# JanEGerken/HEAL-SWIN

Hardware: AMD Instinct MI355X
Metric: images/sec fwd+bwd, HEAL-SWIN nside=256 seg, batch=8 at 1/2/4/8 MI355X (higher is better)
Workload: dtype bf16

## Files before the change

heal_swin_amd/_lib.py:

```python
import ctypes
import os

import numpy as np

_PKG = os.path.dirname(os.path.abspath(__file__))
LIB_PATH = os.path.join(_PKG, "lib", "libhealswin.so")

HS_F32, HS_BF16 = 0, 1
HS_F64 = 3
HS_PRED_LABELS, HS_PRED_ROWS16 = 2, 4
HS_ATTN_COSINE = 1
HS_ATTN_FORCE_VALU = 2
HS_ATTN_RESIDUAL = 4
HS_ATTN_OVERWRITE_GRADS = 8
HS_EPI_BIAS, HS_EPI_GELU, HS_EPI_DGELU, HS_EPI_RESID = 0, 1, 2, 3
HS_ACC_DEFER = 2
HS_MLP_NORM_AFTER = 16
HS_U8, HS_I32, HS_I64 = 8, 9, 10
HS_FLAT_PATCH_ROWS, HS_FLAT_PIXEL_ROWS, HS_FLAT_IMAGE = 0, 1, 2
HS_DEPTH_L1, HS_DEPTH_L2, HS_DEPTH_HUBER, HS_DEPTH_LOGVAR = 0, 1, 2, 3
HS_DT_NONE, HS_DT_LOG, HS_DT_INV = 0, 1, 2
HS_DT_ZERO_BKG, HS_DT_1000_BKG, HS_DT_AFFINE, HS_DT_INVERSE = 1, 2, 4, 8
HS_DEPTH_STATS_WORDS = 15
HS_HISTOGRAM_MAX_BINS = 4096

c_i64 = ctypes.c_int64
c_int = ctypes.c_int
c_uint = ctypes.c_uint
c_ptr = ctypes.c_void_p
c_float = ctypes.c_float


class WgradProblem(ctypes.Structure):
    _fields_ = [("dy", c_ptr), ("x", c_ptr), ("dw", c_ptr), ("dbias", c_ptr), ("n_out", c_int), ("k_in", c_int), ("accumulate", c_int),
                ("gelu_x", c_int)]


def wgrad_problems(members):
    arr = (WgradProblem * len(members))()
    for q, (dy, x, dw, db, n_out, k_in, acc, gelu_x) in zip(arr, members):
        q.dy, q.x, q.dw, q.dbias = dy.data_ptr(), x.data_ptr(), dw.data_ptr(), (None if db is None else db.data_ptr())
        q.n_out, q.k_in, q.accumulate, q.gelu_x = int(n_out), int(k_in), int(acc), int(bool(gelu_x))
    return arr

class AdamGroup(ctypes.Structure):
    _fields_ = [("lr_dev", c_ptr), ("lr", c_float), ("beta1", c_float), ("beta2", c_float), ("eps", c_float), ("weight_decay", c_float),
                ("decoupled", ctypes.c_int32)]


def adam_groups(records):
    arr = (AdamGroup * len(records))()
    for q, (lr, b1, b2, eps, wd, decoupled) in zip(arr, records):
        on_device = hasattr(lr, "data_ptr")
        q.lr_dev, q.lr = (lr.data_ptr() if on_device else None), (0.0 if on_device else float(lr))
        q.beta1, q.beta2, q.eps, q.weight_decay, q.decoupled = float(b1), float(b2), float(eps), float(wd), int(bool(decoupled))
    return arr


class FisheyeCamera(ctypes.Structure):
    _fields_ = [("k", ctypes.c_double * 8), ("cx_offset", ctypes.c_double), ("cy_offset", ctypes.c_double), ("aspect_ratio", ctypes.c_double),
                ("poly_order", c_int), ("width", c_int), ("height", c_int)]


_SIGNATURES = {
    "hs_nest2ring": [c_int, c_ptr, c_ptr, c_i64],
    "hs_ring2nest": [c_int, c_ptr, c_ptr, c_i64],
    "hs_nest_win_idcs": [c_int, c_ptr],
    "hs_rel_pos_index": [c_int, c_ptr],
    "hs_build_nest_roll_shift": [c_i64, c_int, c_int, c_ptr, c_ptr, c_ptr],
    "hs_build_nest_grid_shift": [c_int, c_int, c_int, c_ptr, c_ptr, c_ptr],
    "hs_build_ring_shift": [c_int, c_int, c_int, c_int, c_ptr, c_ptr, c_ptr],
    "hs_attn_mask_from_labels": [c_ptr, c_i64, c_int, c_ptr],
    "hs_flat_zorder": [c_int, c_int, c_int, c_ptr, c_ptr],
    "hs_build_flat_shift": [c_int, c_int, c_int, c_int, c_int, c_ptr, c_ptr, c_ptr],
    "hs_flat_rel_pos_index": [c_int, c_ptr, c_ptr],
    "hs_flat_attn_mask": [c_int, c_int, c_int, c_int, c_ptr],
    "hs_flat_img_to_rows": [c_ptr, c_int, c_ptr, c_int, c_int, c_int, c_int, c_int, c_int, c_int, c_int, c_i64, c_ptr],
    "hs_flat_rows_to_img": [c_ptr, c_int, c_ptr, c_int, c_int, c_int, c_int, c_int, c_int, c_int, c_int, c_i64, c_ptr],
    "hs_flat_resize": [c_ptr, c_int, c_i64, c_int, c_int, c_int, c_int, c_ptr, c_ptr, c_ptr, c_ptr, c_ptr, c_int, c_int, c_int, c_int, c_int,
                       c_int, c_i64, c_int, c_int, c_int, c_int, c_int, c_int, c_float, c_float, c_ptr],
    "hs_rel_bias_gather": [c_ptr, c_ptr, c_ptr, c_int, c_int, c_int, c_ptr],
    "hs_rel_bias_scatter_grad_sorted_add": [c_ptr, c_ptr, c_ptr, c_ptr, c_int, c_int, c_int, c_ptr],
    "hs_cos_head_scale_fwd": [c_ptr, c_ptr, c_int, c_ptr],
    "hs_cos_head_scale_bwd": [c_ptr, c_ptr, c_ptr, c_int, c_int, c_ptr],
    "hs_rel_bias_gather_many": [c_ptr, c_ptr, c_int, c_ptr, c_ptr, c_int, c_int, c_ptr],
    "hs_rel_bias_scatter_grad_sorted_many": [c_ptr, c_ptr, c_ptr, c_ptr, c_int, c_ptr, c_ptr, c_int, c_int, c_ptr],
    "hs_cos_head_scale_many": [c_ptr, c_ptr, c_ptr, c_ptr, c_ptr, c_int, c_ptr],
    "hs_rel_bias_scatter_grad": [c_ptr, c_ptr, c_ptr, c_int, c_int, c_int, c_ptr],
    "hs_rel_bias_scatter_grad_sorted": [c_ptr, c_ptr, c_ptr, c_ptr, c_int, c_int, c_int, c_ptr],
    "hs_window_attn_fwd": [c_ptr, c_ptr, c_ptr, c_ptr, c_ptr, c_ptr, c_i64, c_ptr,
                           c_int, c_i64, c_int, c_int, c_int, c_uint, ctypes.c_float, ctypes.c_uint64, c_int, c_ptr],
    "hs_window_attn_bwd": [c_ptr, c_ptr, c_ptr, c_ptr, c_ptr, c_ptr, c_ptr, c_ptr, c_ptr, c_ptr, c_ptr, c_i64, c_ptr,
                           c_int, c_i64, c_int, c_int, c_int, c_uint, ctypes.c_float, ctypes.c_uint64, c_int, c_ptr],
    "hs_gather_rows": [c_ptr, c_ptr, c_ptr, c_i64, c_int, c_i64, c_i64, c_ptr],
    "hs_pix2ang_nest": [c_int, c_i64, c_i64, c_ptr, c_ptr],
    "hs_ln_head_supported": [c_int, c_int, c_int],
    "hs_expand_ln_head_supported": [c_int, c_int, c_int, c_int],
    "hs_expand_ln_head_fwd": [c_ptr, c_ptr, c_ptr, c_ptr, c_ptr, c_ptr, c_ptr, c_ptr, c_ptr, c_i64, c_int, c_int, c_int, c_ptr],
    "hs_expand_ln_head_ce_fwd": [c_ptr, c_ptr, c_ptr, c_ptr, c_ptr, c_ptr, c_ptr, c_int, c_ptr, c_ptr, c_ptr, c_ptr, c_ptr, c_i64, c_int, c_int,
                                 c_int, c_ptr],
    "hs_expand_ln_head_ce_step_fwd": [c_ptr, c_ptr, c_ptr, c_ptr, c_ptr, c_ptr, c_ptr, c_int, c_ptr, c_ptr, c_ptr, c_ptr, c_ptr, c_ptr, c_ptr,
                                      c_ptr, c_i64, c_int, c_int, c_int, c_ptr],
    "hs_ln_head_ce_bwd": [c_ptr, c_ptr, c_ptr, c_ptr, c_ptr, c_ptr, c_int, c_ptr, c_ptr, c_ptr, c_ptr, c_ptr, c_ptr, c_i64, c_int, c_int, c_ptr],
    "hs_expand_ln_head_depth_fwd": [c_ptr, c_ptr, c_ptr, c_ptr, c_ptr, c_ptr, c_int, c_float, c_int, c_ptr, c_ptr, c_ptr, c_ptr, c_ptr, c_i64,
                                    c_int, c_int, c_int, c_ptr],
    "hs_expand_ln_head_depth_step_fwd": [c_ptr, c_ptr, c_ptr, c_ptr, c_ptr, c_ptr, c_int, c_float, c_int, c_ptr, c_ptr, c_ptr, c_ptr, c_ptr,
                                         c_int, c_int, c_float, c_float, c_int, ctypes.c_double, c_ptr, c_int, c_ptr, c_ptr, c_ptr, c_ptr,
                                         c_i64, c_int, c_int, c_int, c_ptr],
    "hs_ln_head_depth_bwd": [c_ptr, c_ptr, c_ptr, c_ptr, c_int, c_float, c_ptr, c_int, c_ptr, c_ptr, c_ptr, c_ptr, c_ptr, c_ptr, c_i64, c_int,
                             c_int, c_ptr],
    "hs_ln_head_fwd": [c_ptr, c_ptr, c_ptr, c_ptr, c_ptr, c_ptr, c_i64, c_int, c_int, c_int, c_ptr],
    "hs_ln_head_bwd": [c_ptr, c_ptr, c_ptr, c_ptr, c_ptr, c_ptr, c_ptr, c_ptr, c_i64, c_int, c_int, c_int, c_ptr],
    "hs_sample_bilinear_u8": [c_ptr, c_int, c_int, c_int, c_int, c_ptr, c_ptr, c_i64, c_ptr, c_ptr],
    "hs_sample_mask_u8": [c_ptr, c_int, c_int, c_int, c_ptr, c_ptr, c_i64, c_int, c_ptr, c_ptr],
    "hs_hp_rotated_coords": [c_int, c_i64, c_i64, ctypes.POINTER(FisheyeCamera), c_ptr, c_int, c_ptr, c_ptr, c_ptr],
    "hs_sample_bilinear_u8_per_sample": [c_ptr, c_int, c_int, c_int, c_int, c_ptr, c_ptr, c_i64, c_ptr, c_ptr],
    "hs_sample_mask_u8_per_sample": [c_ptr, c_int, c_int, c_int, c_ptr, c_ptr, c_i64, c_int, c_ptr, c_ptr],
    "hs_hp_interp_weights_nest": [c_int, c_ptr, c_ptr, c_i64, c_ptr, c_ptr],
    "hs_backproject_labels": [c_ptr, c_int, c_i64, c_i64, c_int, c_i64, c_i64, c_i64, c_ptr, c_i64, c_int, c_ptr, c_ptr],
    "hs_backproject_image": [c_ptr, c_i64, c_i64, c_ptr, c_ptr, c_i64, c_ptr, c_ptr],
    "hs_seg_confusion": [c_ptr, c_int, c_i64, c_i64, c_int, c_i64, c_i64, c_i64, c_ptr, c_i64, c_ptr, c_int, c_ptr, c_ptr, c_ptr],
    "hs_depth_points": [c_ptr, c_int, c_i64, c_i64, c_i64, c_i64, c_i64, c_i64, c_ptr, c_i64, c_ptr, c_int, c_ptr, c_ptr, c_ptr, c_ptr,
                        c_ptr],
    "hs_chamfer_nn": [c_ptr, c_ptr, c_i64, c_i64, c_ptr, c_ptr, c_i64, c_i64, c_i64, c_int, c_ptr, c_ptr, c_ptr, c_ptr, c_ptr, c_ptr,
                      c_ptr],
    "hs_depth_metrics": [c_ptr, c_int, c_i64, c_i64, c_i64, c_i64, c_i64, c_i64, c_i64, c_ptr, c_int, c_i64, c_i64, c_i64, c_int,
                         ctypes.c_double, c_ptr, c_int, c_ptr, c_ptr, c_ptr],
    "hs_backproject_depth": [c_ptr, c_int, c_i64, c_i64, c_i64, c_i64, c_ptr, c_ptr, c_i64, c_ptr, c_ptr],
    "hs_flat_depth_to_hp": [c_ptr, c_int, c_i64, c_i64, c_i64, c_i64, c_ptr, c_ptr, c_ptr, c_i64, c_ptr, c_ptr],
    "hs_depth_metrics_gather": [c_ptr, c_int, c_i64, c_i64, c_i64, c_i64, c_i64, c_ptr, c_ptr, c_ptr, c_i64, c_ptr, c_int, c_i64, c_i64,
                                c_int, ctypes.c_double, c_ptr, c_int, c_ptr, c_ptr, c_ptr],
    "hs_sample_bilinear_u8_f32": [c_ptr, c_int, c_int, c_int, c_int, c_ptr, c_ptr, c_i64, c_ptr, c_ptr],
    "hs_sample_nearest_f32": [c_ptr, c_int, c_int, c_int, c_ptr, c_ptr, c_i64, c_float, c_ptr, c_ptr],
    "hs_sample_bilinear_u8_f32_per_sample": [c_ptr, c_int, c_int, c_int, c_int, c_ptr, c_ptr, c_i64, c_ptr, c_ptr],
    "hs_sample_nearest_f32_per_sample": [c_ptr, c_int, c_int, c_int, c_ptr, c_ptr, c_i64, c_float, c_ptr, c_ptr],
    "hs_depth_target": [c_ptr, c_i64, c_i64, c_ptr, c_i64, c_i64, c_i64, c_i64, c_int, c_int, c_float, c_float, c_ptr],
    "hs_depth_stats_update": [c_ptr, c_i64, c_int, c_int, c_ptr, c_ptr, c_ptr],
    "hs_depth_stats_merge": [c_ptr, c_int, c_ptr, c_ptr],
    "hs_histogram_update": [c_ptr, c_i64, c_int, c_int, c_ptr, c_int, c_ptr, c_ptr],
    "hs_select_rows": [c_ptr, c_int, c_i64, c_i64, c_i64, c_int, c_int, c_ptr, c_ptr, c_ptr],
    "hs_gelu_fwd": [c_ptr, c_ptr, c_i64, ctypes.c_float, ctypes.c_uint64, c_int, c_ptr],
    "hs_gelu_bwd": [c_ptr, c_ptr, c_ptr, c_i64, ctypes.c_float, ctypes.c_uint64, c_int, c_ptr],
    "hs_residual_drop": [c_ptr, c_ptr, c_ptr, c_ptr, c_i64, c_i64, ctypes.c_float, ctypes.c_uint64, c_int, c_ptr],
    "hs_linear_wgrad": [c_ptr, c_ptr, c_ptr, c_ptr, c_ptr, c_i64, c_int, c_int, c_int, c_int, c_ptr],
    "hs_reduce_flush": [c_ptr],
    "hs_set_seed_epoch": [c_ptr],
    "hs_linear_wgrad_gelu": [c_ptr, c_ptr, c_ptr, c_ptr, c_ptr, c_i64, c_int, c_int, c_int, c_int, c_ptr],
    "hs_linear_wgrad_gelu_supported": [c_i64, c_int, c_int, c_int],
    "hs_linear_wgrad_group_variant": [c_i64, c_int, c_int, c_int],
    "hs_linear_wgrad_group": [c_ptr, c_int, c_ptr, c_i64, c_int, c_ptr],
    "hs_mlp_fused_supported": [c_int, c_int, c_int],
    "hs_mlp_fused_fwd": [c_ptr, c_ptr, c_ptr, c_ptr, c_ptr, c_ptr, c_ptr, c_ptr, c_ptr, c_ptr, c_ptr, c_ptr, c_ptr, c_i64, c_int, c_int, c_uint,
                         c_int, c_ptr],
    "hs_mlp_fused_bwd": [c_ptr, c_ptr, c_ptr, c_ptr, c_ptr, c_ptr, c_ptr, c_i64, c_int, c_int, c_int, c_ptr],
    "hs_mlp_fused_drop_fwd": [c_ptr, c_ptr, c_ptr, c_ptr, c_ptr, c_ptr, c_ptr, c_ptr, c_ptr, c_ptr, c_ptr, c_ptr, c_ptr, c_ptr, c_i64, c_float,
                              ctypes.c_uint64, ctypes.c_uint64, c_i64, c_int, c_int, c_uint, c_int, c_ptr],
    "hs_mlp_fused_drop_bwd": [c_ptr, c_ptr, c_ptr, c_ptr, c_ptr, c_ptr, c_ptr, c_float, ctypes.c_uint64, c_i64, c_int, c_int, c_int, c_ptr],
    "hs_adam_step": [c_ptr, c_ptr, c_ptr, c_ptr, c_ptr, c_i64, c_float, c_ptr, c_float, c_float, c_float, c_float, c_int, c_ptr, c_ptr],
    "hs_adam_advance": [c_ptr, c_ptr],
    "hs_grad_stats": [c_ptr, c_i64, c_ptr, c_int, c_ptr, c_ptr],
    "hs_grad_guard_finalize": [c_ptr, c_i64, c_ptr, c_int, c_int, c_float, c_ptr, c_ptr, c_ptr, c_ptr],
    "hs_adam_step_guarded": [c_ptr, c_ptr, c_ptr, c_ptr, c_ptr, c_i64, c_float, c_ptr, c_float, c_float, c_float, c_float, c_int, c_ptr, c_float,
                             c_ptr, c_int, c_ptr],
    "hs_adam_advance_guarded": [c_ptr, c_ptr, c_int, c_ptr, c_ptr],
    "hs_adam_step_groups": [c_ptr, c_ptr, c_ptr, c_ptr, c_ptr, c_i64, c_ptr, c_int, c_ptr, c_int, c_ptr, c_int, c_i64, c_ptr, c_ptr],
    "hs_adam_step_groups_guarded": [c_ptr, c_ptr, c_ptr, c_ptr, c_ptr, c_i64, c_ptr, c_int, c_ptr, c_int, c_ptr, c_int, c_i64, c_ptr, c_float,
                                    c_ptr, c_int, c_ptr],
    "hs_grad_scale": [c_ptr, c_i64, c_float, c_ptr, c_ptr],
    "hs_weight_avg_update": [c_ptr, c_ptr, c_i64, c_int, c_float, c_ptr, c_ptr, c_int, c_ptr],
    "hs_weight_avg_advance": [c_ptr, c_ptr, c_int, c_ptr],
    "hs_weight_avg_swap": [c_ptr, c_ptr, c_ptr, c_i64, c_ptr],
    "hs_split_bf16x3": [c_ptr, c_ptr, c_i64, c_int, c_int, c_ptr],
    "hs_gelu_split3": [c_ptr, c_ptr, c_ptr, c_i64, c_int, ctypes.c_float, ctypes.c_uint64, c_ptr],
    "hs_linear_wgrad_ld": [c_ptr, c_i64, c_i64, c_ptr, c_i64, c_i64, c_ptr, c_ptr, c_ptr, c_i64, c_int, c_int, c_int, c_ptr],
    "hs_layernorm_fwd": [c_ptr, c_ptr, c_ptr, c_ptr, c_ptr, c_ptr, c_ptr, c_i64, c_int, c_int, c_ptr],
    "hs_add_layernorm_fwd": [c_ptr, c_ptr, c_ptr, c_ptr, c_ptr, c_ptr, c_ptr, c_ptr, c_i64, c_int, c_int, c_ptr],
    "hs_add_layernorm_bwd": [c_ptr, c_ptr, c_ptr, c_ptr, c_ptr, c_ptr, c_ptr, c_ptr, c_ptr, c_ptr, c_int, c_i64, c_int, c_int, c_ptr],
    "hs_layernorm_drop_fwd": [c_ptr, c_ptr, c_ptr, c_ptr, c_ptr, c_ptr, c_ptr, c_ptr, c_i64, ctypes.c_float, ctypes.c_uint64,
                              c_i64, c_int, c_int, c_ptr],
    "hs_layernorm_drop_bwd": [c_ptr, c_ptr, c_ptr, c_ptr, c_ptr, c_ptr, c_ptr, c_ptr, c_ptr, c_int, c_ptr, c_i64, ctypes.c_float,
                              ctypes.c_uint64, c_i64, c_int, c_int, c_ptr],
    "hs_add_layernorm_drop_fwd": [c_ptr, c_ptr, c_ptr, c_ptr, c_ptr, c_ptr, c_ptr, c_ptr, c_ptr, c_i64, ctypes.c_float,
                                  ctypes.c_uint64, c_i64, c_int, c_int, c_ptr],
    "hs_layernorm_fwd_ex": [c_ptr, c_ptr, c_ptr, c_ptr, c_ptr, c_ptr, c_ptr, c_ptr, c_ptr, c_ptr, c_ptr, c_ptr, c_i64, ctypes.c_float,
                            ctypes.c_uint64, c_i64, c_int, c_int, c_ptr],
    "hs_add_layernorm_drop_bwd": [c_ptr, c_ptr, c_ptr, c_ptr, c_ptr, c_ptr, c_ptr, c_ptr, c_ptr, c_ptr, c_ptr, c_int, c_ptr, c_i64,
                                  ctypes.c_float, ctypes.c_uint64, c_i64, c_int, c_int, c_ptr],
    "hs_seg_ce_fwd": [c_ptr, c_ptr, c_ptr, c_ptr, c_i64, c_i64, c_int, c_i64, c_i64, c_i64, c_int, c_i64, c_int, c_ptr],
    "hs_seg_ce_bwd": [c_ptr, c_ptr, c_ptr, c_ptr, c_ptr, c_i64, c_i64, c_int, c_i64, c_i64, c_i64, c_i64, c_i64, c_i64, c_int, c_i64,
                      c_int, c_ptr],
    "hs_depth_loss_fwd": [c_ptr, c_ptr, c_ptr, c_i64, c_i64, c_int, c_i64, c_i64, c_i64, c_int, c_float, c_int, c_ptr],
    "hs_depth_loss_bwd": [c_ptr, c_ptr, c_ptr, c_ptr, c_i64, c_i64, c_int, c_i64, c_i64, c_i64, c_i64, c_i64, c_i64, c_int, c_float, c_int, c_ptr],
    "hs_gemm_nt": [c_ptr, c_i64, c_ptr, c_i64, c_int, c_ptr, c_i64, c_ptr, c_i64, c_int, c_ptr, c_ptr, c_ptr, c_i64, c_int, c_int,
                   ctypes.c_float, ctypes.c_uint64, c_int, c_ptr],
    "hs_gemm_nt_set_tile": [c_int],
    "hs_gemm_nt_tile_variant": [c_i64, c_int, c_int, c_int, c_int],
    "hs_set_reserved_cus": [c_int],
    "hs_transpose_many_16": [c_ptr, c_int, c_int, c_ptr],
    "hs_debug_occupy_cus": [c_int, c_int, c_int, ctypes.c_double, c_ptr],
    "hs_debug_buffer_soffset_probe": [c_ptr, c_int, c_int, c_ptr, c_ptr],
    "hs_window_attn_module_supported": [c_int, c_int, c_int, c_int],
    "hs_window_attn_module_fwd": [c_ptr, c_ptr, c_ptr, c_ptr, c_ptr, c_ptr, c_ptr, c_ptr, c_ptr, c_ptr, c_ptr, c_i64, c_ptr, c_int, c_i64,
                                  c_int, c_int, c_int, c_uint, c_int, c_ptr],
    "hs_window_attn_module_fwd_train": [c_ptr] * 17 + [c_i64] + [c_ptr] * 6 + [c_int, c_i64, c_int, c_int, c_int, c_uint, c_int, c_ptr],
    "hs_window_attn_module_bwd_chain": [c_ptr] * 14 + [c_i64] + [c_ptr] * 11 + [c_int, c_int, c_i64, c_int, c_int, c_int, c_uint, c_int, c_ptr],
    "hs_layernorm_bwd": [c_ptr, c_ptr, c_ptr, c_ptr, c_ptr, c_ptr, c_ptr, c_ptr, c_ptr, c_int, c_i64, c_int, c_int, c_ptr],
    "hs_patch_merge_fwd": [c_ptr, c_ptr, c_ptr, c_ptr, c_ptr, c_ptr, c_ptr, c_ptr, c_i64, c_int, c_int, c_int, c_ptr],
    "hs_patch_merge_bwd": [c_ptr, c_ptr, c_ptr, c_ptr, c_ptr, c_ptr, c_ptr, c_ptr, c_ptr, c_ptr, c_ptr, c_ptr, c_ptr, c_int, c_i64,
                           c_int, c_int, c_int, c_ptr],
    "hs_patch_expand_fwd": [c_ptr, c_ptr, c_ptr, c_ptr, c_ptr, c_ptr, c_ptr, c_ptr, c_i64, c_int, c_int, c_int, c_int, c_ptr],
    "hs_patch_expand_bwd": [c_ptr, c_ptr, c_ptr, c_ptr, c_ptr, c_ptr, c_ptr, c_ptr, c_ptr, c_ptr, c_ptr, c_ptr, c_ptr, c_int, c_i64,
                            c_int, c_int, c_int, c_int, c_ptr],
}
_OTHER = {
    "hs_version": ([], ctypes.c_char_p),
    "hs_last_error": ([], ctypes.c_char_p),
    "hs_status_string": ([c_int], ctypes.c_char_p),
    "hs_device_count": ([], c_int),
    "hs_get_reserved_cus": ([], c_int),
    "hs_grad_guard_piece": ([], c_int),
    "hs_adam_max_groups": ([], c_int),
    "hs_get_seed_epoch": ([], c_ptr),
    "hs_reduce_pending": ([c_ptr], c_int),
    "hs_layernorm_bwd_workspace": ([c_i64, c_int], c_i64),
    "hs_seg_ce_partials": ([c_i64, c_i64], c_i64),
    "hs_depth_loss_partials": ([c_i64, c_i64], c_i64),
    "hs_depth_points_workspace": ([c_i64, c_i64], c_i64),
    "hs_depth_metrics_partials": ([c_i64], c_i64),
    "hs_depth_stats_partials": ([c_i64], c_i64),
    "hs_select_rows_workspace": ([c_int], c_i64),
    "hs_flat_resize_lds_bytes": ([c_int, c_int, c_int, c_int, c_int, c_int], c_i64),
    "hs_ln_head_partials": ([c_i64], c_i64),
    "hs_expand_ln_head_blocks": ([c_i64], c_i64),
    "hs_linear_wgrad_workspace": ([c_i64, c_int, c_int], c_i64),
    "hs_linear_wgrad_group_workspace": ([c_ptr, c_int, c_i64, c_int], c_i64),
    "hs_window_attn_bwd_workspace": ([c_int, c_i64, c_int, c_int, c_int, c_int], c_i64),
    "hs_patch_merge_bwd_workspace": ([c_i64, c_int, c_int], c_i64),
    "hs_window_attn_module_bwd_chain_workspace": ([c_int, c_i64, c_int, c_int, c_int], c_i64),
    "hs_patch_expand_bwd_workspace": ([c_i64, c_int, c_int, c_int], c_i64),
}
EXPORTED_SYMBOLS = sorted(list(_SIGNATURES) + list(_OTHER))


def _load():
    if not os.path.exists(LIB_PATH):
        raise RuntimeError(
            f"libhealswin.so not found at {LIB_PATH}: build it first (python heal_swin_amd/build.py, or "
            "__graft_entry__.build()).  heal_swin_amd has no CPU or PyTorch fallback."
        )
    lib = ctypes.CDLL(LIB_PATH)
    for name, argtypes in _SIGNATURES.items():
        fn = getattr(lib, name)
        fn.argtypes = argtypes
        fn.restype = c_int
    for name, (argtypes, restype) in _OTHER.items():
        fn = getattr(lib, name)
        fn.argtypes = argtypes
        fn.restype = restype
    return lib


lib = _load()


def check(status, what):
    if status != 0:
        msg = lib.hs_last_error().decode()
        kind = lib.hs_status_string(status).decode()
        if status == 1:
            raise AssertionError(f"{what}: {msg}")
        raise RuntimeError(f"{what} failed ({kind}): {msg}")


def version():
    return lib.hs_version().decode()


def device_count():
    return int(lib.hs_device_count())


def np_ptr(a):
    return None if a is None else a.ctypes.data_as(c_ptr)


def ptr(t):
    return None if t is None else ctypes.c_void_p(t.data_ptr())


def stream_ptr(device):
    import torch

    return ctypes.c_void_p(torch.cuda.current_stream(device).cuda_stream)


def dtype_code(dtype):
    import torch

    if dtype == torch.float32:
        return HS_F32
    if dtype == torch.bfloat16:
        return HS_BF16
    raise TypeError(f"heal_swin_amd kernels support float32 and bfloat16 activations, got {dtype}")


def nest2ring(nside, ipix):
    a = np.ascontiguousarray(ipix, dtype=np.int64)
    out = np.empty_like(a)
    check(lib.hs_nest2ring(int(nside), np_ptr(a), np_ptr(out), a.size), "hs_nest2ring")
    return out


def ring2nest(nside, ipix):
    a = np.ascontiguousarray(ipix, dtype=np.int64)
    out = np.empty_like(a)
    check(lib.hs_ring2nest(int(nside), np_ptr(a), np_ptr(out), a.size), "hs_ring2nest")
    return out


def nest_win_idcs(window_size):
    side = int(round(window_size ** 0.5))
    out = np.empty((max(side, 1), max(side, 1)), dtype=np.int64)
    check(lib.hs_nest_win_idcs(int(window_size), np_ptr(out)), "hs_nest_win_idcs")
    return out


def rel_pos_index(window_size):
    out = np.empty((window_size, window_size), dtype=np.int64)
    check(lib.hs_rel_pos_index(int(window_size), np_ptr(out)), "hs_rel_pos_index")
    return out


def _shift_out(n):
    return np.empty(n, np.int32), np.empty(n, np.int32), np.empty(n, np.uint8)


def build_nest_roll_shift(n_pix, window_size, shift_size):
    idx, inv, lab = _shift_out(n_pix)
    check(lib.hs_build_nest_roll_shift(int(n_pix), int(window_size), int(shift_size), np_ptr(idx), np_ptr(inv), np_ptr(lab)),
          "hs_build_nest_roll_shift")
    return idx, inv, lab


def build_nest_grid_shift(nside, base_pix, window_size):
    idx, inv, lab = _shift_out(max(base_pix, 0) * nside * nside)
    check(lib.hs_build_nest_grid_shift(int(nside), int(base_pix), int(window_size), np_ptr(idx), np_ptr(inv), np_ptr(lab)),
          "hs_build_nest_grid_shift")
    return idx, inv, lab


def build_ring_shift(nside, base_pix, window_size, shift_size):
    idx, inv, lab = _shift_out(max(base_pix, 0) * nside * nside)
    check(lib.hs_build_ring_shift(int(nside), int(base_pix), int(window_size), int(shift_size), np_ptr(idx), np_ptr(inv),
                                  np_ptr(lab)), "hs_build_ring_shift")
    return idx, inv, lab


def attn_mask_from_labels(labels, window_size):
    lab = np.ascontiguousarray(labels, dtype=np.uint8)
    out = np.empty((lab.size // window_size, window_size, window_size), dtype=np.float32)
    check(lib.hs_attn_mask_from_labels(np_ptr(lab), lab.size, int(window_size), np_ptr(out)), "hs_attn_mask_from_labels")
    return out


def flat_zorder(Ht, Wt, T):
    z = np.empty(Ht * Wt, np.int32)
    rm = np.empty(Ht * Wt, np.int32)
    check(lib.hs_flat_zorder(int(Ht), int(Wt), int(T), np_ptr(z), np_ptr(rm)), "hs_flat_zorder")
    return z, rm


def build_flat_shift(Ht, Wt, T, window, shift):
    idx, inv, lab = _shift_out(max(Ht * Wt, 0))
    check(lib.hs_build_flat_shift(int(Ht), int(Wt), int(T), int(window), int(shift), np_ptr(idx), np_ptr(inv), np_ptr(lab)),
          "hs_build_flat_shift")
    return idx, inv, lab


def flat_rel_pos_index(window):
    n = window * window
    rm = np.empty((n, n), np.int64)
    z = np.empty((n, n), np.int64)
    check(lib.hs_flat_rel_pos_index(int(window), np_ptr(rm), np_ptr(z)), "hs_flat_rel_pos_index")
    return rm, z


def flat_attn_mask(Ht, Wt, window, shift):
    out = np.empty(((Ht // window) * (Wt // window), window * window, window * window), np.float32)
    check(lib.hs_flat_attn_mask(int(Ht), int(Wt), int(window), int(shift), np_ptr(out)), "hs_flat_attn_mask")
    return out
```

heal_swin_amd/csrc/linear_wgrad.hip:

```cpp
#include <cstdlib>
#include <type_traits>
#include <utility>

#include "hs_gelu.h"

namespace hs {
namespace {

typedef __attribute__((ext_vector_type(4))) short s16x4;
typedef __attribute__((ext_vector_type(8))) short s16x8;
typedef __attribute__((address_space(3))) s16x4 lds_s16x4;

constexpr int kTileK = 128;
constexpr int kTok = 32;
constexpr int kMaxSlices = 2048;
constexpr int kReduceChunks = 32;
__host__ __device__ constexpr int row_stride(int cols) { return cols * 2 + 64; }

template <int LD>
__device__ __forceinline__ bf16x8 tr_frag(const unsigned char* tile, int tok0, int col0, int lane) {
    const int L = lane & 15, nblk = (lane >> 4) & 1;
    const unsigned char* a = tile + (tok0 + (L >> 2)) * LD + (col0 + nblk * 16 + (L & 3) * 4) * 2;
    const s16x4 lo = __builtin_amdgcn_ds_read_tr16_b64_v4i16((lds_s16x4*)a);
    const s16x4 hi = __builtin_amdgcn_ds_read_tr16_b64_v4i16((lds_s16x4*)(a + 4 * LD));
    const s16x8 v = {lo[0], lo[1], lo[2], lo[3], hi[0], hi[1], hi[2], hi[3]};
    return __builtin_bit_cast(bf16x8, v);
}

struct Geometry {
    int tile_n, tile_k, tiles_n, tiles_k, tiles, slices, chunks, per_xcd, dma, reads_first;
    int64_t rows_per_slice;
};

__host__ __device__ constexpr int64_t record_floats(int n_out, int k_in) { return (int64_t)n_out * k_in + n_out; }

inline void plan_slices(Geometry& g, int64_t rows, int wgs_per_cu) {
    int64_t want = ((int64_t)usable_cus() * wgs_per_cu) / g.tiles;
    const int64_t max_by_rows = (rows + 511) / 512;
    if (want > max_by_rows) want = max_by_rows;
    if (want > kMaxSlices) want = kMaxSlices;
    if (want < 1) want = 1;
    g.slices = (int)want;
    const int64_t rps = (rows + g.slices - 1) / g.slices;
    g.rows_per_slice = ((rps + kTok - 1) / kTok) * kTok;
    g.per_xcd = (g.slices * g.tiles + 7) / 8;
}

inline bool slice_fits_dma(const Geometry& g, int64_t width, int elt) { return g.rows_per_slice * width * elt < ((int64_t)1 << 31); }

inline Geometry geometry_for(int64_t rows, int n_out, int k_in, int tile_k, int wgs_per_cu, int tile_n = 0, int elt = 2) {
    Geometry g;
    g.tile_n = tile_n ? tile_n : ((n_out % 256 == 0 || n_out >= 512) ? 256 : 128);
    g.tile_k = tile_k;
    g.tiles_n = (n_out + g.tile_n - 1) / g.tile_n;
    g.tiles_k = (k_in + tile_k - 1) / tile_k;
    g.tiles = g.tiles_n * g.tiles_k;
    plan_slices(g, rows, wgs_per_cu);
    g.chunks = g.slices > 2 * kReduceChunks ? kReduceChunks : 1;
    g.dma = slice_fits_dma(g, n_out > k_in ? n_out : k_in, elt);
    g.reads_first = 3;
    return g;
}

inline Geometry make_geometry(int64_t rows, int n_out, int k_in) {
    static const int variant = getenv("HS_WGRAD_VARIANT") ? atoi(getenv("HS_WGRAD_VARIANT")) : 1;
    if (variant == 1 && k_in % 256 == 0 && (n_out % 256 == 0 || n_out >= 512)) {
        const Geometry g = geometry_for(rows, n_out, k_in, 256, 1);
        if (g.dma) return g;
    }
    Geometry g = geometry_for(rows, n_out, k_in, kTileK, 2);
    if (variant != 1) g.dma = 0;
    return g;
}

inline Geometry make_geometry_f32(int64_t rows, int n_out, int k_in) { return geometry_for(rows, n_out, k_in, kTileK, 3, 128, 4); }

__device__ __forceinline__ bool block_to_work(const Geometry& g, int b, int& slice, int& tile) {
    const int v = (b & 7) * g.per_xcd + (b >> 3);
    slice = v / g.tiles;
    tile = v % g.tiles;
    return (b >> 3) < g.per_xcd && v < g.slices * g.tiles;
}

struct SliceRows {
    int64_t m_begin;
    int m_len;
};
__device__ __forceinline__ SliceRows slice_rows(const Geometry& g, int slice, int64_t rows) {
    const int64_t m_begin = (int64_t)slice * g.rows_per_slice;
    int64_t m_end = m_begin + g.rows_per_slice;
    if (m_end > rows) m_end = rows;
    return {m_begin, m_end > m_begin ? (int)(m_end - m_begin) : 0};
}

template <int NB>
__device__ __forceinline__ void store_partial(const f32x16 (&acc)[NB][2], float* dst, int n_wave, int k_wave, int n_out, int k_in,
                                              int lane) {
#pragma unroll
    for (int i = 0; i < NB; ++i)
#pragma unroll
        for (int j = 0; j < 2; ++j) {
            const int kk = k_wave + j * 32 + (lane & 31);
#pragma unroll
            for (int r = 0; r < 16; ++r) {
                const int nn = n_wave + i * 32 + (r & 3) + 8 * (r >> 2) + 4 * (lane >> 5);
                if (nn < n_out && kk < k_in) dst[(int64_t)nn * k_in + kk] = acc[i][j][r];
            }
        }
}

template <int TN, int GROUPS, int PER_THREAD>
__device__ __forceinline__ void fold_bias(float* bred, const float (&bsum)[PER_THREAD], int tid, int n0, int n_out, float* dst) {
    constexpr int CH = TN / PER_THREAD;
#pragma unroll
    for (int i = 0; i < PER_THREAD; ++i) bred[(tid / CH) * TN + (tid % CH) * PER_THREAD + i] = bsum[i];
    __syncthreads();
    if (tid < TN) {
        float t = 0.f;
#pragma unroll
        for (int rg = 0; rg < GROUPS; ++rg) t += bred[rg * TN + tid];
        if (n0 + tid < n_out) dst[n0 + tid] = t;
    }
}

__device__ __forceinline__ void add_bf16x8(float (&bsum)[8], uint32_t w0, uint32_t w1, uint32_t w2, uint32_t w3) {
    const uint32_t w[4] = {w0, w1, w2, w3};
#pragma unroll
    for (int i = 0; i < 4; ++i) {
        bsum[2 * i] += bf_lo(w[i]);
        bsum[2 * i + 1] += bf_hi(w[i]);
    }
}

template <int NB>
__global__ void __launch_bounds__(256, 2) wgrad_kernel(const uint16_t* __restrict__ dy, const uint16_t* __restrict__ x,
                                                       float* __restrict__ part_w, float* __restrict__ part_b, int64_t rows,
                                                       int n_out, int k_in, Geometry g) {
    constexpr int TN = 64 * NB;
    constexpr int LDY = row_stride(TN), LDX = row_stride(kTileK);
    constexpr int YB = kTok * LDY, XB = kTok * LDX;
    constexpr int YCH = TN / 8;
    constexpr int YPASS = (kTok * YCH) / 256;
    __shared__ __attribute__((aligned(16))) unsigned char smem[2 * (YB + XB)];
    auto ytile = [&](int b) { return smem + b * (YB + XB); };
    auto xtile = [&](int b) { return smem + b * (YB + XB) + YB; };
    float* bred = (float*)smem;

    const int tid = threadIdx.x, lane = tid & 63, wave = tid >> 6, half = lane >> 5;
    const int wn = wave >> 1, wk = wave & 1;

    int slice, tile;
    if (!block_to_work(g, blockIdx.x, slice, tile)) return;
    const int tn = tile / g.tiles_k, tk = tile % g.tiles_k;
    const int n0 = tn * TN, k0 = tk * kTileK;
    const SliceRows sr = slice_rows(g, slice, rows);
    const int64_t m_begin = sr.m_begin, m_end = sr.m_begin + sr.m_len;

    const int xr = tid >> 4, xc = tid & 15;
    const int yr = tid / YCH, yc = tid % YCH;
    const bool ycol_ok = n0 + yc * 8 < n_out, xcol_ok = k0 + xc * 8 < k_in;
    const uint16_t* yptr = dy + n0 + yc * 8;
    const uint16_t* xptr = x + k0 + xc * 8;
    const bool do_bias = part_b != nullptr && tk == 0;
    float bsum[8] = {0.f, 0.f, 0.f, 0.f, 0.f, 0.f, 0.f, 0.f};

    f32x16 acc[NB][2];
    zero(acc);

    uint4 ry[YPASS], rx[2];
    auto load_regs = [&](int64_t m0) {
#pragma unroll
        for (int ps = 0; ps < YPASS; ++ps) {
            const int64_t m = m0 + yr + (256 / YCH) * ps;
            ry[ps] = (m < m_end && ycol_ok) ? *(const uint4*)(yptr + m * n_out) : make_uint4(0, 0, 0, 0);
        }
#pragma unroll
        for (int ps = 0; ps < 2; ++ps) {
            const int64_t m = m0 + xr + 16 * ps;
            rx[ps] = (m < m_end && xcol_ok) ? *(const uint4*)(xptr + m * k_in) : make_uint4(0, 0, 0, 0);
        }
    };
    auto store_lds = [&](int buf) {
#pragma unroll
        for (int ps = 0; ps < YPASS; ++ps) {
            *(uint4*)(ytile(buf) + (yr + (256 / YCH) * ps) * LDY + yc * 16) = ry[ps];
            if (do_bias) add_bf16x8(bsum, ry[ps].x, ry[ps].y, ry[ps].z, ry[ps].w);
        }
#pragma unroll
        for (int ps = 0; ps < 2; ++ps) *(uint4*)(xtile(buf) + (xr + 16 * ps) * LDX + xc * 16) = rx[ps];
    };

    if (m_begin < m_end) {
        load_regs(m_begin);
        store_lds(0);
    }
    __syncthreads();
    int buf = 0;
    for (int64_t m0 = m_begin; m0 < m_end; m0 += kTok) {
        const bool more = m0 + kTok < m_end;
        if (more) load_regs(m0 + kTok);
        bf16x8 af[2][NB], bf[2][2];
#pragma unroll
        for (int ks = 0; ks < 2; ++ks) {
            const int tok0 = ks * 16 + 8 * half;
#pragma unroll
            for (int j = 0; j < 2; ++j) bf[ks][j] = tr_frag<LDX>(xtile(buf), tok0, wk * 64 + j * 32, lane);
#pragma unroll
            for (int i = 0; i < NB; ++i) af[ks][i] = tr_frag<LDY>(ytile(buf), tok0, wn * 32 * NB + i * 32, lane);
        }
#pragma unroll
        for (int ks = 0; ks < 2; ++ks)
#pragma unroll
            for (int i = 0; i < NB; ++i)
#pragma unroll
                for (int j = 0; j < 2; ++j)
                    acc[i][j] = __builtin_amdgcn_mfma_f32_32x32x16_bf16(af[ks][i], bf[ks][j], acc[i][j], 0, 0, 0);
        if (more) store_lds(buf ^ 1);
        __syncthreads();
        buf ^= 1;
    }

    const int64_t rec = slice * record_floats(n_out, k_in);
    store_partial(acc, part_w + rec, n0 + wn * 32 * NB, k0 + wk * 64, n_out, k_in, lane);
    if (do_bias) fold_bias<TN, 256 / YCH>(bred, bsum, tid, n0, n_out, part_b + rec);
}

#if defined(__HIP_DEVICE_COMPILE__)
template <int YI, int XI>
__device__ __forceinline__ void issue_stage(__amdgpu_buffer_rsrc_t rs_y, __amdgpu_buffer_rsrc_t rs_x, unsigned char* ylds,
                                            unsigned char* xlds, int (&voff_y)[YI], int (&voff_x)[XI], int ystep, int xstep) {
#pragma unroll
    for (int j = 0; j < YI; ++j) {
        __builtin_amdgcn_raw_ptr_buffer_load_lds(rs_y, (lds_void*)(ylds + j * 1024), 16, voff_y[j], 0, 0, 0);
        voff_y[j] += ystep;
    }
#pragma unroll
    for (int j = 0; j < XI; ++j) {
        __builtin_amdgcn_raw_ptr_buffer_load_lds(rs_x, (lds_void*)(xlds + j * 1024), 16, voff_x[j], 0, 0, 0);
        voff_x[j] += xstep;
    }
}

template <int PIECES, int AH>
__device__ __forceinline__ void wait_stage(int younger) {
    if (AH - 1 >= 2 && younger >= 2)
        asm volatile("s_waitcnt vmcnt(%0)" ::"n"(2 * PIECES) : "memory");
    else if (younger >= 1)
        asm volatile("s_waitcnt vmcnt(%0)" ::"n"(PIECES) : "memory");
    else
        asm volatile("s_waitcnt vmcnt(0)" ::: "memory");
}
#endif

template <int NSTAGE, typename Issue, typename Stage>
__device__ __forceinline__ void run_stages(int nst, Issue&& issue, Stage&& stage) {
    static_for<NSTAGE - 1>([&](auto bc) {
        constexpr int b = decltype(bc)::value;
        if (nst > b) issue(b);
    });
    for (int t = 0; t < nst; t += NSTAGE)
        static_for<NSTAGE>([&](auto bc) {
            constexpr int b = decltype(bc)::value;
            if (t + b < nst) stage(t + b, bc, std::integral_constant<int, (b + NSTAGE - 1) % NSTAGE>{});
        });
}

template <int RB>
__device__ __forceinline__ s16x8 tr_frag_asm(uint32_t a, int ks) {
    s16x4 lo, hi;
    if (ks == 0) {
        asm volatile("ds_read_b64_tr_b16 %0, %1" : "=v"(lo) : "v"(a));
        asm volatile("ds_read_b64_tr_b16 %0, %1 offset:%2" : "=v"(hi) : "v"(a), "n"(4 * RB));
    } else {
        asm volatile("ds_read_b64_tr_b16 %0, %1 offset:%2" : "=v"(lo) : "v"(a), "n"(16 * RB));
        asm volatile("ds_read_b64_tr_b16 %0, %1 offset:%2" : "=v"(hi) : "v"(a), "n"(20 * RB));
    }
    return s16x8{lo[0], lo[1], lo[2], lo[3], hi[0], hi[1], hi[2], hi[3]};
}

constexpr int kMaxGroup = 4;
struct Member {
    const uint16_t* dy;
    const uint16_t* x;
    float* part_w;
    float* part_b;
    int n_out, k_in, ldy, ldx, yc0, xc0, tiles_k, first_tile, gelu;
};
struct MemberTable {
    int count;
    Member m[kMaxGroup];
};

template <int NB, int TK, bool GX = false>
__global__ void __launch_bounds__(TK * 2, 2) wgrad_dma_kernel(const MemberTable tb, int64_t rows, Geometry g) {
#if defined(__HIP_DEVICE_COMPILE__)
    constexpr int TN = 64 * NB;
    constexpr int WK = TK / 64, NW = 2 * WK, NT = 64 * NW;
    constexpr int YRB = TN * 2, XRB = TK * 2;
    constexpr int YB = kTok * YRB, XB = kTok * XRB;
    constexpr int STAGE = YB + XB, NSTAGE = TK == 256 ? 4 : 3, AH = NSTAGE - 1;
    constexpr int YI = YB / 1024 / NW, XI = XB / 1024 / NW;
    constexpr int YCH = YRB / 16, XCH = XRB / 16;
    __shared__ __attribute__((aligned(16))) unsigned char smem[NSTAGE * STAGE];
    float* bred = (float*)smem;

    const int tid = threadIdx.x, lane = tid & 63, wave = tid >> 6, half = lane >> 5;
    const int wn = wave / WK, wk = wave % WK;
    int slice, tile;
    if (!block_to_work(g, blockIdx.x, slice, tile)) return;
    int mi = 0;
#pragma unroll
    for (int i = 1; i < kMaxGroup; ++i)
        if (i < tb.count && tile >= tb.m[i].first_tile) mi = i;
    const Member& mb = tb.m[__builtin_amdgcn_readfirstlane(mi)];
    const uint16_t* __restrict__ dy = mb.dy;
    const uint16_t* __restrict__ x = mb.x;
    float* __restrict__ part_w = mb.part_w;
    float* __restrict__ part_b = mb.part_b;
    const int n_out = mb.n_out, k_in = mb.k_in, ldy = mb.ldy, ldx = mb.ldx, yc0 = mb.yc0, xc0 = mb.xc0;
    [[maybe_unused]] const bool gelu = mb.gelu != 0;
    tile -= mb.first_tile;
    const int tn = tile / mb.tiles_k, tk = tile % mb.tiles_k;
    const int n0 = tn * TN, k0 = tk * TK;
    const SliceRows sr = slice_rows(g, slice, rows);
    const int64_t m_begin = sr.m_begin;
    const int m_len = sr.m_len, nst = (m_len + kTok - 1) / kTok;
    const bool do_bias = part_b != nullptr && tk == 0;

    const __amdgpu_buffer_rsrc_t rs_y = __builtin_amdgcn_make_buffer_rsrc((void*)(dy + m_begin * ldy), 0, m_len * ldy * 2, 0x00020000);
    const __amdgpu_buffer_rsrc_t rs_x = __builtin_amdgcn_make_buffer_rsrc((void*)(x + m_begin * ldx), 0, m_len * ldx * 2, 0x00020000);
    int voff_y[YI], voff_x[XI];
#pragma unroll
    for (int j = 0; j < YI; ++j) {
        const int p = (wave * YI + j) * 64 + lane, row = p / YCH, pc = p % YCH;
        voff_y[j] = row * ldy * 2 + (yc0 + n0) * 2 + ((pc ^ ((row & 3) << 2)) << 4);
    }
#pragma unroll
    for (int j = 0; j < XI; ++j) {
        const int p = (wave * XI + j) * 64 + lane, row = p / XCH, pc = p % XCH;
        voff_x[j] = row * ldx * 2 + (xc0 + k0) * 2 + ((pc ^ ((row & 3) << 2)) << 4);
    }
    const int ystep = kTok * ldy * 2, xstep = kTok * ldx * 2;
    auto issue = [&](int b) {
        unsigned char* base = smem + b * STAGE;
        issue_stage(rs_y, rs_x, base + wave * YI * 1024, base + YB + wave * XI * 1024, voff_y, voff_x, ystep, xstep);
    };

    const int L = lane & 15, nblk = (lane >> 4) & 1, row_in = L >> 2;
    const int lane_lo = (nblk * 2 + ((L & 3) >> 1)) * 16 + (L & 1) * 8;
    int yoff[NB], xoff[2];
#pragma unroll
    for (int i = 0; i < NB; ++i) yoff[i] = (8 * half + row_in) * YRB + ((((wn * NB + i) ^ row_in) << 2) << 4) + lane_lo;
#pragma unroll
    for (int j = 0; j < 2; ++j) xoff[j] = YB + (8 * half + row_in) * XRB + ((((wk * 2 + j) ^ row_in) << 2) << 4) + lane_lo;
    const uint32_t lds0 = (uint32_t)(uintptr_t)(__attribute__((address_space(3))) unsigned char*)smem;
    const int yr = tid / YCH, yc = tid % YCH;
    const int boff = yr * YRB + ((yc ^ ((yr & 3) << 2)) << 4);
    float bsum[8] = {0.f, 0.f, 0.f, 0.f, 0.f, 0.f, 0.f, 0.f};

    f32x16 acc[NB][2];
    zero(acc);

    s16x8 af[2][NB], bf[2][2];
    auto read_frags = [&](auto buf_c) {
        constexpr int buf = decltype(buf_c)::value;
#pragma unroll
        for (int ks = 0; ks < 2; ++ks) {
#pragma unroll
            for (int j = 0; j < 2; ++j) bf[ks][j] = tr_frag_asm<XRB>(lds0 + buf * STAGE + xoff[j], ks);
#pragma unroll
            for (int i = 0; i < NB; ++i) af[ks][i] = tr_frag_asm<YRB>(lds0 + buf * STAGE + yoff[i], ks);
        }
    };
    auto wait_half = [&](int ks) {
        if constexpr (NB == 4) {
            if (ks == 0) asm volatile("s_waitcnt lgkmcnt(12)" : "+v"(bf[0][0]), "+v"(bf[0][1]), "+v"(af[0][0]), "+v"(af[0][1]), "+v"(af[0][2]), "+v"(af[0][3]));
            else asm volatile("s_waitcnt lgkmcnt(0)" : "+v"(bf[1][0]), "+v"(bf[1][1]), "+v"(af[1][0]), "+v"(af[1][1]), "+v"(af[1][2]), "+v"(af[1][3]));
        } else {
            if (ks == 0) asm volatile("s_waitcnt lgkmcnt(8)" : "+v"(bf[0][0]), "+v"(bf[0][1]), "+v"(af[0][0]), "+v"(af[0][1]));
            else asm volatile("s_waitcnt lgkmcnt(0)" : "+v"(bf[1][0]), "+v"(bf[1][1]), "+v"(af[1][0]), "+v"(af[1][1]));
        }
    };
    auto mma_half = [&](int ks) {
        if constexpr (GX) {
            if (gelu) {
#pragma unroll
                for (int j = 0; j < 2; ++j) {
                    u32x4 w = __builtin_bit_cast(u32x4, bf[ks][j]);
#pragma unroll
                    for (int e = 0; e < 4; ++e) {
                        const f32x2 v = gelu2(f32x2{bf_lo(w[e]), bf_hi(w[e])});
                        w[e] = pack_bf16x2(v.x, v.y);
                    }
                    bf[ks][j] = __builtin_bit_cast(s16x8, w);
                }
            }
        }
#pragma unroll
        for (int i = 0; i < NB; ++i)
#pragma unroll
            for (int j = 0; j < 2; ++j)
                acc[i][j] = __builtin_amdgcn_mfma_f32_32x32x16_bf16(__builtin_bit_cast(bf16x8, af[ks][i]), __builtin_bit_cast(bf16x8, bf[ks][j]), acc[i][j], 0, 0, 0);
    };
    auto bias_sums = [&](auto buf_c) {
        constexpr int buf = decltype(buf_c)::value;
        constexpr int PS = kTok / (NT / YCH);
        u32x4 v[PS];
        const uint32_t ba = lds0 + buf * STAGE + boff;
        asm volatile("ds_read_b128 %0, %1" : "=v"(v[0]) : "v"(ba));
        asm volatile("ds_read_b128 %0, %1 offset:%2" : "=v"(v[1]) : "v"(ba), "n"((NT / YCH) * YRB));
        if constexpr (PS == 4) {
            asm volatile("ds_read_b128 %0, %1 offset:%2" : "=v"(v[2]) : "v"(ba), "n"(2 * (NT / YCH) * YRB));
            asm volatile("ds_read_b128 %0, %1 offset:%2" : "=v"(v[3]) : "v"(ba), "n"(3 * (NT / YCH) * YRB));
            asm volatile("s_waitcnt lgkmcnt(0)" : "+v"(v[0]), "+v"(v[1]), "+v"(v[2]), "+v"(v[3]));
        } else {
            asm volatile("s_waitcnt lgkmcnt(0)" : "+v"(v[0]), "+v"(v[1]));
        }
#pragma unroll
        for (int ps = 0; ps < PS; ++ps) add_bf16x8(bsum, v[ps][0], v[ps][1], v[ps][2], v[ps][3]);
    };
    const bool late_group = NW == 8 && g.reads_first == 3 && wave >= NW / 2;
    auto stage = [&](int t, auto buf_c, auto nbuf_c) {
        constexpr int nbuf = decltype(nbuf_c)::value;
        wait_stage<YI + XI, AH>(nst - 1 - t);
        __builtin_amdgcn_s_barrier();
        if (late_group) {
            if (t > 0) {
                mma_half(0);
                mma_half(1);
            }
            __builtin_amdgcn_sched_barrier(0);
            if (t + AH < nst) issue(nbuf);
            read_frags(buf_c);
            if (do_bias) bias_sums(buf_c);
            wait_half(0);
            wait_half(1);
            return;
        }
        if (g.reads_first == 0 && t + AH < nst) issue(nbuf);
        read_frags(buf_c);
        if (g.reads_first != 0 && g.reads_first != 2 && t + AH < nst) issue(nbuf);
        wait_half(0);
        mma_half(0);
        __builtin_amdgcn_sched_barrier(0);
        if (g.reads_first == 2 && t + AH < nst) issue(nbuf);
        wait_half(1);
        mma_half(1);
        if (do_bias) bias_sums(buf_c);
    };
    run_stages<NSTAGE>(nst, issue, stage);

    if (late_group && nst > 0) {
        mma_half(0);
        mma_half(1);
    }

    const int64_t rec = slice * record_floats(n_out, k_in);
    store_partial(acc, part_w + rec, n0 + wn * 32 * NB, k0 + wk * 64, n_out, k_in, lane);
    if (do_bias) {
        __syncthreads();
        fold_bias<TN, NT / YCH>(bred, bsum, tid, n0, n_out, part_b + rec);
    }
#endif
}

constexpr int kTokF = 16;

template <int OFF>
__device__ __forceinline__ float lds_b32(uint32_t a) {
    float v;
    asm volatile("ds_read_b32 %0, %1 offset:%2" : "=v"(v) : "v"(a), "n"(OFF));
    return v;
}
template <int OFF>
__device__ __forceinline__ u32x4 lds_b128(uint32_t a) {
    u32x4 v;
    asm volatile("ds_read_b128 %0, %1 offset:%2" : "=v"(v) : "v"(a), "n"(OFF));
    return v;
}

__global__ void __launch_bounds__(256, 3) wgrad_dma_f32_kernel(const float* __restrict__ dy, const float* __restrict__ x,
                                                               float* __restrict__ part_w, float* __restrict__ part_b, int64_t rows,
                                                               int n_out, int k_in, Geometry g) {
#if defined(__HIP_DEVICE_COMPILE__)
    constexpr int TN = 128, TK = 128;
    constexpr int RB = TN * 4;
    constexpr int YB = kTokF * RB, XB = kTokF * RB;
    constexpr int STAGE = YB + XB, NSTAGE = 3, AH = NSTAGE - 1;
    constexpr int YI = YB / 1024 / 4, XI = XB / 1024 / 4;
    __shared__ __attribute__((aligned(16))) unsigned char smem[NSTAGE * STAGE];
    float* bred = (float*)smem;
    const int tid = threadIdx.x, lane = tid & 63, wave = tid >> 6, half = lane >> 5, l31 = lane & 31;
    const int wn = wave >> 1, wk = wave & 1;
    int slice, tile;
    if (!block_to_work(g, blockIdx.x, slice, tile)) return;
    const int tn = tile / g.tiles_k, tk = tile % g.tiles_k;
    const int n0 = tn * TN, k0 = tk * TK;
    const SliceRows sr = slice_rows(g, slice, rows);
    const int64_t m_begin = sr.m_begin;
    const int m_len = sr.m_len, nst = (m_len + kTokF - 1) / kTokF;
    const bool do_bias = part_b != nullptr && tk == 0;

    const __amdgpu_buffer_rsrc_t rs_y = __builtin_amdgcn_make_buffer_rsrc((void*)(dy + m_begin * n_out), 0, m_len * n_out * 4, 0x00020000);
    const __amdgpu_buffer_rsrc_t rs_x = __builtin_amdgcn_make_buffer_rsrc((void*)(x + m_begin * k_in), 0, m_len * k_in * 4, 0x00020000);
    int voff_y[YI], voff_x[XI];
#pragma unroll
    for (int j = 0; j < YI; ++j) {
        const int p = (wave * YI + j) * 64 + lane, row = p >> 5, ch = p & 31;
        voff_y[j] = row * n_out * 4 + n0 * 4 + (ch << 4);
    }
#pragma unroll
    for (int j = 0; j < XI; ++j) {
        const int p = (wave * XI + j) * 64 + lane, row = p >> 5, ch = p & 31;
        voff_x[j] = row * k_in * 4 + k0 * 4 + (ch << 4);
    }
    const int ystep = kTokF * n_out * 4, xstep = kTokF * k_in * 4;
    auto issue = [&](int b) {
        unsigned char* base = smem + b * STAGE;
        issue_stage(rs_y, rs_x, base + wave * YI * 1024, base + YB + wave * XI * 1024, voff_y, voff_x, ystep, xstep);
    };
    const uint32_t lds0 = (uint32_t)(uintptr_t)(__attribute__((address_space(3))) unsigned char*)smem;
    const uint32_t ya = lds0 + half * RB + (wn * 64 + l31) * 4;
    const uint32_t xa = lds0 + YB + half * RB + (wk * 64 + l31) * 4;
    const uint32_t ba = lds0 + (tid >> 5) * RB + (tid & 31) * 16;
    float bsum[4] = {0.f, 0.f, 0.f, 0.f};

    f32x16 acc[2][2];
    zero(acc);

    auto stage = [&](int t, auto buf_c, auto nbuf_c) {
        constexpr int buf = decltype(buf_c)::value, nbuf = decltype(nbuf_c)::value;
        wait_stage<YI + XI, AH>(nst - 1 - t);
        __builtin_amdgcn_s_barrier();
        if (t + AH < nst) issue(nbuf);
        const uint32_t yb = ya + buf * STAGE, xb = xa + buf * STAGE;
        float fa[8][2], fb[8][2];
        static_for<8>([&](auto jc) {
            constexpr int j = decltype(jc)::value;
            fa[j][0] = lds_b32<2 * j * RB>(yb);
            fa[j][1] = lds_b32<2 * j * RB + 128>(yb);
            fb[j][0] = lds_b32<2 * j * RB>(xb);
            fb[j][1] = lds_b32<2 * j * RB + 128>(xb);
        });
        asm volatile("s_waitcnt lgkmcnt(15)"
                     : "+v"(fa[0][0]), "+v"(fa[0][1]), "+v"(fb[0][0]), "+v"(fb[0][1]), "+v"(fa[1][0]), "+v"(fa[1][1]), "+v"(fb[1][0]),
                       "+v"(fb[1][1]), "+v"(fa[2][0]), "+v"(fa[2][1]), "+v"(fb[2][0]), "+v"(fb[2][1]), "+v"(fa[3][0]), "+v"(fa[3][1]),
                       "+v"(fb[3][0]), "+v"(fb[3][1]));
#pragma unroll
        for (int j = 0; j < 4; ++j)
#pragma unroll
            for (int a = 0; a < 2; ++a)
#pragma unroll
                for (int b2 = 0; b2 < 2; ++b2)
                    acc[a][b2] = __builtin_amdgcn_mfma_f32_32x32x2f32(fa[j][a], fb[j][b2], acc[a][b2], 0, 0, 0);
        __builtin_amdgcn_sched_barrier(0);
        asm volatile("s_waitcnt lgkmcnt(0)"
                     : "+v"(fa[4][0]), "+v"(fa[4][1]), "+v"(fb[4][0]), "+v"(fb[4][1]), "+v"(fa[5][0]), "+v"(fa[5][1]), "+v"(fb[5][0]),
                       "+v"(fb[5][1]), "+v"(fa[6][0]), "+v"(fa[6][1]), "+v"(fb[6][0]), "+v"(fb[6][1]), "+v"(fa[7][0]), "+v"(fa[7][1]),
                       "+v"(fb[7][0]), "+v"(fb[7][1]));
#pragma unroll
        for (int j = 4; j < 8; ++j)
#pragma unroll
            for (int a = 0; a < 2; ++a)
#pragma unroll
                for (int b2 = 0; b2 < 2; ++b2)
                    acc[a][b2] = __builtin_amdgcn_mfma_f32_32x32x2f32(fa[j][a], fb[j][b2], acc[a][b2], 0, 0, 0);
        if (do_bias) {
            u32x4 v0 = lds_b128<0>(ba + buf * STAGE), v1 = lds_b128<8 * RB>(ba + buf * STAGE);
            asm volatile("s_waitcnt lgkmcnt(0)" : "+v"(v0), "+v"(v1));
#pragma unroll
            for (int i = 0; i < 4; ++i) bsum[i] += __uint_as_float(v0[i]) + __uint_as_float(v1[i]);
        }
    };
    run_stages<NSTAGE>(nst, issue, stage);

    const int64_t rec = slice * record_floats(n_out, k_in);
    store_partial(acc, part_w + rec, n0 + wn * 64, k0 + wk * 64, n_out, k_in, lane);
    if (do_bias) {
        __syncthreads();
        fold_bias<TN, 8>(bred, bsum, tid, n0, n_out, part_b + rec);
    }
#endif
}

inline int dma_variant(const Geometry& g) { return !g.dma ? 0 : (g.tile_k == 256 ? 1 : (g.tile_n == 256 ? 2 : 3)); }
inline bool on_gelu_tile(const Geometry& g) { return dma_variant(g) == 3; }
inline bool bf16_shape_ok(int64_t rows, int n_out, int k_in) {
    return rows > 0 && n_out > 0 && k_in > 0 && n_out % 4 == 0 && k_in % 8 == 0;
}

inline void launch_dma(int variant, bool any_gelu, dim3 grid, hipStream_t s, const MemberTable& tb, int64_t rows, const Geometry& g) {
    if (variant == 1)
        hipLaunchKernelGGL((wgrad_dma_kernel<4, 256>), grid, dim3(512), 0, s, tb, rows, g);
    else if (variant == 2)
        hipLaunchKernelGGL((wgrad_dma_kernel<4, 128>), grid, dim3(256), 0, s, tb, rows, g);
    else if (any_gelu)
        hipLaunchKernelGGL((wgrad_dma_kernel<2, 128, true>), grid, dim3(256), 0, s, tb, rows, g);
    else
        hipLaunchKernelGGL((wgrad_dma_kernel<2, 128>), grid, dim3(256), 0, s, tb, rows, g);
}

inline int sum_slices(const float* part_w, int slices, int n_out, int k_in, float* dw, float* dbias, int accumulate, hipStream_t s) {
    const int64_t n = (int64_t)n_out * k_in, rec = record_floats(n_out, k_in), count = dbias ? rec : n;
    if (accumulate & HS_ACC_DEFER) return reduce_defer(part_w, rec, slices, n, count, dw, dbias, accumulate & 1, s);
    return reduce_now(part_w, rec, slices, n, count, dw, dbias, accumulate & 1, s);
}

struct GroupPlan {
    bool grouped;
    int variant, any_gelu;
    Geometry g;
    int first_tile[kMaxGroup], tiles_k[kMaxGroup];
    int64_t offset[kMaxGroup], total;
};

inline GroupPlan plan_group(const hs_wgrad_problem* p, int count, int64_t rows, int dtype) {
    GroupPlan pl{};
    pl.grouped = dtype == HS_BF16 && count > 1;
    int tiles = 0;
    for (int i = 0; i < count && pl.grouped; ++i) {
        if (!bf16_shape_ok(rows, p[i].n_out, p[i].k_in)) pl.grouped = false;
        if (!pl.grouped) break;
        const Geometry gi = make_geometry(rows, p[i].n_out, p[i].k_in);
        const int v = dma_variant(gi);
        if (i == 0) {
            pl.variant = v;
            pl.g = gi;
        }
        if (v == 0 || v != pl.variant || (p[i].gelu_x && !on_gelu_tile(gi))) pl.grouped = false;
        pl.first_tile[i] = tiles;
        pl.tiles_k[i] = gi.tiles_k;
        pl.any_gelu |= p[i].gelu_x ? 1 : 0;
        tiles += gi.tiles;
    }
    if (pl.grouped) {
        pl.g.tiles = tiles;
        plan_slices(pl.g, rows, pl.variant == 1 ? 1 : 2);
        for (int i = 0; i < count; ++i)
            if (!slice_fits_dma(pl.g, p[i].n_out > p[i].k_in ? p[i].n_out : p[i].k_in, 2)) pl.grouped = false;
    }
    int64_t off = 0;
    for (int i = 0; i < count; ++i) {
        pl.offset[i] = off;
        off += pl.grouped ? pl.g.slices * record_floats(p[i].n_out, p[i].k_in) : hs_linear_wgrad_workspace(rows, p[i].n_out, p[i].k_in);
    }
    pl.total = off;
    return pl;
}

struct ColumnBlock {
    int ld, col0;
};

int linear_wgrad_impl(const void* dy, const void* x, float* dw, float* dbias, float* workspace, int64_t rows, int n_out, int k_in,
                      int accumulate, int dtype, void* stream, ColumnBlock yb, ColumnBlock xb, bool gelu_x) {
    HS_CHECK_ARG(dy && x && dw && workspace, "null pointer");
    HS_CHECK_ALIGNED("hs_linear_wgrad", 16, dy, x, dw, dbias, workspace);
    if (int st = linear_wgrad_check_shape("hs_linear_wgrad", rows, n_out, k_in, dtype)) return st;
    const Geometry g = dtype == HS_F32 ? make_geometry_f32(rows, n_out, k_in) : make_geometry(rows, n_out, k_in);
    if (gelu_x && !(dtype == HS_BF16 && on_gelu_tile(g)))
        return fail(HS_ERR_UNSUPPORTED, "hs_linear_wgrad_gelu: bf16 and the 128 x 128 LDS-DMA tile only (n_out <= 128-class shapes)");
    const bool strided = yb.ld != n_out || xb.ld != k_in || yb.col0 || xb.col0;
    if (strided) {
        if (!g.dma || !slice_fits_dma(g, yb.ld > xb.ld ? yb.ld : xb.ld, 2))
            return fail(HS_ERR_UNSUPPORTED, "hs_linear_wgrad_ld: a token slice exceeds the 2 GiB buffer-offset range");
    }
    float* part_w = workspace;
    float* part_b = dbias ? workspace + (int64_t)n_out * k_in : nullptr;
    hipStream_t s = (hipStream_t)stream;
    const dim3 grid((unsigned)(8 * g.per_xcd));
    const uint16_t* dyp = (const uint16_t*)dy;
    const uint16_t* xp = (const uint16_t*)x;
    if (dtype == HS_F32)
        hipLaunchKernelGGL(wgrad_dma_f32_kernel, grid, dim3(256), 0, s, (const float*)dy, (const float*)x, part_w, part_b, rows, n_out,
                           k_in, g);
    else if (g.dma) {
        MemberTable tb{};
        tb.count = 1;
        tb.m[0] = Member{dyp, xp, part_w, part_b, n_out, k_in, yb.ld, xb.ld, yb.col0, xb.col0, g.tiles_k, 0, gelu_x ? 1 : 0};
        launch_dma(dma_variant(g), gelu_x, grid, s, tb, rows, g);
    } else if (g.tile_n == 256)
        hipLaunchKernelGGL(wgrad_kernel<4>, grid, dim3(256), 0, s, dyp, xp, part_w, part_b, rows, n_out, k_in, g);
    else
        hipLaunchKernelGGL(wgrad_kernel<2>, grid, dim3(256), 0, s, dyp, xp, part_w, part_b, rows, n_out, k_in, g);
    HS_LAUNCH_CHECK("linear_wgrad");
    return sum_slices(part_w, g.slices, n_out, k_in, dw, dbias, accumulate, s);
}

}

int linear_wgrad_check_shape(const char* who, int64_t rows, int n_out, int k_in, int dtype) {
    HS_CHECK_ARG(rows > 0 && n_out > 0 && k_in > 0, "%s: bad shape", who);
    HS_CHECK_ARG(dtype == HS_BF16 || dtype == HS_F32, "%s: dtype must be HS_F32 or HS_BF16", who);
    if (dtype == HS_BF16 && (n_out % 4 || k_in % 8))
        return fail(HS_ERR_UNSUPPORTED, "%s: bf16: n_out must be a multiple of 4 and k_in a multiple of 8", who);
    if (dtype == HS_F32 && (n_out % 4 || k_in % 4)) return fail(HS_ERR_UNSUPPORTED, "%s: fp32: n_out and k_in must be multiples of 4", who);
    const Geometry g = dtype == HS_F32 ? make_geometry_f32(rows, n_out, k_in) : make_geometry(rows, n_out, k_in);
    if (dtype == HS_BF16 && n_out % 8 && !g.dma)
        return fail(HS_ERR_UNSUPPORTED, "%s: n_out must be a multiple of 8 for slices beyond 2 GiB", who);
    if (dtype == HS_F32 && !g.dma) return fail(HS_ERR_UNSUPPORTED, "%s: fp32: a token slice exceeds the 2 GiB buffer-offset range", who);
    return HS_OK;
}

}

extern "C" {

int64_t hs_linear_wgrad_workspace(int64_t rows, int n_out, int k_in) {
    if (rows <= 0 || n_out <= 0 || k_in <= 0) return 0;
    const hs::Geometry g = hs::make_geometry(rows, n_out, k_in), f = hs::make_geometry_f32(rows, n_out, k_in);
    const int64_t a = g.slices + (g.chunks > 1 ? g.chunks : 0), b = f.slices + (f.chunks > 1 ? f.chunks : 0);
    return (a > b ? a : b) * hs::record_floats(n_out, k_in);
}

int hs_linear_wgrad(const void* dy, const void* x, float* dw, float* dbias, float* workspace, int64_t rows, int n_out,
                    int k_in, int accumulate, int dtype, void* stream) {
    return hs::linear_wgrad_impl(dy, x, dw, dbias, workspace, rows, n_out, k_in, accumulate, dtype, stream, {n_out, 0}, {k_in, 0}, false);
}

int hs_linear_wgrad_gelu_supported(int64_t rows, int n_out, int k_in, int dtype) {
    if (dtype != HS_BF16 || !hs::bf16_shape_ok(rows, n_out, k_in)) return 0;
    return hs::on_gelu_tile(hs::make_geometry(rows, n_out, k_in));
}

int hs_linear_wgrad_gelu(const void* dy, const void* h, float* dw, float* dbias, float* workspace, int64_t rows, int n_out, int k_in,
                         int accumulate, int dtype, void* stream) {
    return hs::linear_wgrad_impl(dy, h, dw, dbias, workspace, rows, n_out, k_in, accumulate, dtype, stream, {n_out, 0}, {k_in, 0}, true);
}

int hs_linear_wgrad_ld(const void* dy, int64_t ldy, int64_t ycol0, const void* x, int64_t ldx, int64_t xcol0, float* dw, float* dbias,
                       float* workspace, int64_t rows, int n_out, int k_in, int accumulate, void* stream) {
    HS_CHECK_ARG(ycol0 >= 0 && xcol0 >= 0 && ycol0 + n_out <= ldy && xcol0 + k_in <= ldx && ldy % 8 == 0 && ldx % 8 == 0 &&
                 ycol0 % 8 == 0 && xcol0 % 8 == 0 && ldy < (1 << 20) && ldx < (1 << 20),
                 "hs_linear_wgrad_ld: column blocks must lie inside the rows; strides and offsets are multiples of 8 elements");
    return hs::linear_wgrad_impl(dy, x, dw, dbias, workspace, rows, n_out, k_in, accumulate, HS_BF16, stream, {(int)ldy, (int)ycol0},
                                 {(int)ldx, (int)xcol0}, false);
}

int hs_linear_wgrad_group_variant(int64_t rows, int n_out, int k_in, int dtype) {
    if (dtype != HS_BF16 || !hs::bf16_shape_ok(rows, n_out, k_in)) return 0;
    return hs::dma_variant(hs::make_geometry(rows, n_out, k_in));
}

int64_t hs_linear_wgrad_group_workspace(const hs_wgrad_problem* problems, int count, int64_t rows, int dtype) {
    if (!problems || count < 1 || count > hs::kMaxGroup || rows <= 0) return 0;
    return hs::plan_group(problems, count, rows, dtype).total;
}

int hs_linear_wgrad_group(const hs_wgrad_problem* problems, int count, float* workspace, int64_t rows, int dtype, void* stream) {
    using namespace hs;
    HS_CHECK_ARG(problems && workspace, "null pointer");
    HS_CHECK_ARG(count >= 1 && count <= kMaxGroup, "hs_linear_wgrad_group: 1 to 4 problems");
    HS_CHECK_ARG(rows > 0, "bad shape");
    HS_CHECK_ARG(dtype == HS_BF16 || dtype == HS_F32, "dtype must be HS_F32 or HS_BF16");
    HS_CHECK_ALIGNED("hs_linear_wgrad_group", 16, workspace);
    for (int i = 0; i < count; ++i)
        HS_CHECK_ALIGNED("hs_linear_wgrad_group", 16, problems[i].dy, problems[i].x, problems[i].dw, problems[i].dbias);
    const GroupPlan pl = plan_group(problems, count, rows, dtype);
    if (!pl.grouped) {
        for (int i = 0; i < count; ++i) {
            const hs_wgrad_problem& p = problems[i];
            if (int st = linear_wgrad_impl(p.dy, p.x, p.dw, p.dbias, workspace + pl.offset[i], rows, p.n_out, p.k_in, p.accumulate, dtype,
                                           stream, {p.n_out, 0}, {p.k_in, 0}, p.gelu_x != 0))
                return st;
        }
        return HS_OK;
    }
    MemberTable tb{};
    tb.count = count;
    for (int i = 0; i < count; ++i) {
        const hs_wgrad_problem& p = problems[i];
        HS_CHECK_ARG(p.dy && p.x && p.dw, "null pointer");
        float* part = workspace + pl.offset[i];
        tb.m[i] = Member{(const uint16_t*)p.dy, (const uint16_t*)p.x, part, p.dbias ? part + (int64_t)p.n_out * p.k_in : nullptr,
                         p.n_out, p.k_in, p.n_out, p.k_in, 0, 0, pl.tiles_k[i], pl.first_tile[i], p.gelu_x ? 1 : 0};
    }
    hipStream_t s = (hipStream_t)stream;
    launch_dma(pl.variant, pl.any_gelu != 0, dim3((unsigned)(8 * pl.g.per_xcd)), s, tb, rows, pl.g);
    HS_LAUNCH_CHECK("linear_wgrad_group");
    for (int i = 0; i < count; ++i) {
        const hs_wgrad_problem& p = problems[i];
        if (int st = sum_slices(tb.m[i].part_w, pl.g.slices, p.n_out, p.k_in, p.dw, p.dbias, p.accumulate, s)) return st;
    }
    return HS_OK;
}

}
```

heal_swin_amd/csrc/mlp_fused.hip:

```cpp
#include <algorithm>

#include "hs_gelu.h"

namespace hs {
HS_DEFINE_SEED_EPOCH_SETTER(set_seed_epoch_mlp_fused)
namespace {

typedef __attribute__((ext_vector_type(4))) float f32x4;
typedef unsigned int u32x2v __attribute__((__vector_size__(8)));

constexpr int kT = 32;
constexpr float kLnEps = 1e-5f;

struct MlpParams {
    const uint16_t* x;
    const uint16_t* wa;
    const uint16_t* wb;
    const float* ba;
    const float* bb;
    const float* ln_g;
    const float* ln_b;
    const uint16_t* hin;
    uint16_t* n_out;
    float* mean_out;
    float* rstd_out;
    uint16_t* h_out;
    uint16_t* act_out;
    uint16_t* out;
    int64_t tiles;
    int residual;
    int ln_after;
    uint16_t* m_out;
    const uint16_t* res_in;
    float drop_p;
    uint64_t seed_h, seed_o;
    const float* row_scale;
    int tiles_per_sample;
    int64_t row0;
};

__device__ __forceinline__ u32x4 ld128(uint32_t addr) {
    u32x4 v;
    asm volatile("ds_read_b128 %0, %1" : "=v"(v) : "v"(addr));
    return v;
}
__device__ __forceinline__ u32x2v ld64(uint32_t addr) {
    u32x2v v;
    asm volatile("ds_read_b64 %0, %1" : "=v"(v) : "v"(addr));
    return v;
}
__device__ __forceinline__ u32x4 ld128_now(uint32_t addr) {
    u32x4 v;
    asm volatile("ds_read_b128 %0, %1\n\ts_waitcnt lgkmcnt(0)" : "=&v"(v) : "v"(addr) : "memory");
    return v;
}
__device__ __forceinline__ void ld128x2_now(uint32_t a0, uint32_t a1, u32x4& v0, u32x4& v1) {
    asm volatile("ds_read_b128 %0, %2\n\tds_read_b128 %1, %3\n\ts_waitcnt lgkmcnt(0)" : "=&v"(v0), "=&v"(v1) : "v"(a0), "v"(a1) : "memory");
}
__device__ __forceinline__ void ld128x4_now(uint32_t a0, uint32_t a1, uint32_t a2, uint32_t a3, u32x4& v0, u32x4& v1, u32x4& v2, u32x4& v3) {
    asm volatile("ds_read_b128 %0, %4\n\tds_read_b128 %1, %5\n\tds_read_b128 %2, %6\n\tds_read_b128 %3, %7\n\ts_waitcnt lgkmcnt(0)"
                 : "=&v"(v0), "=&v"(v1), "=&v"(v2), "=&v"(v3)
                 : "v"(a0), "v"(a1), "v"(a2), "v"(a3)
                 : "memory");
}
__device__ __forceinline__ void ld64x4_now(uint32_t a0, uint32_t a1, uint32_t a2, uint32_t a3, u32x2v& v0, u32x2v& v1, u32x2v& v2, u32x2v& v3) {
    asm volatile("ds_read_b64 %0, %4\n\tds_read_b64 %1, %5\n\tds_read_b64 %2, %6\n\tds_read_b64 %3, %7\n\ts_waitcnt lgkmcnt(0)"
                 : "=&v"(v0), "=&v"(v1), "=&v"(v2), "=&v"(v3)
                 : "v"(a0), "v"(a1), "v"(a2), "v"(a3)
                 : "memory");
}
__device__ __forceinline__ void st64(uint32_t addr, uint32_t a, uint32_t b) {
    const u32x2v v = {a, b};
    asm volatile("ds_write_b64 %0, %1" ::"v"(addr), "v"(v) : "memory");
}
__device__ __forceinline__ void st128(uint32_t addr, const u32x4& v) { asm volatile("ds_write_b128 %0, %1" ::"v"(addr), "v"(v) : "memory"); }
__device__ __forceinline__ bf16x8 as_frag(const u32x4& v) { return __builtin_bit_cast(bf16x8, v); }
__device__ __forceinline__ float row16_sum(float v) {
    v += __builtin_bit_cast(float, __builtin_amdgcn_mov_dpp(__builtin_bit_cast(int, v), 0xB1, 0xF, 0xF, true));
    v += __builtin_bit_cast(float, __builtin_amdgcn_mov_dpp(__builtin_bit_cast(int, v), 0x4E, 0xF, 0xF, true));
    v += __builtin_bit_cast(float, __builtin_amdgcn_mov_dpp(__builtin_bit_cast(int, v), 0x141, 0xF, 0xF, true));
    v += __builtin_bit_cast(float, __builtin_amdgcn_mov_dpp(__builtin_bit_cast(int, v), 0x140, 0xF, 0xF, true));
    return v;
}

template <int C, bool BWD, bool DROP>
__global__ void __launch_bounds__(C * 4, 1) mlp_fused_kernel(MlpParams p) {
#if defined(__HIP_DEVICE_COMPILE__)
    constexpr int H = 4 * C, NW = C / 16, KS1 = C / 16, KS2 = H / 32, NCH = C / 8, HCH = H / 8;
    constexpr int XP = (8 + NW - 1) / NW;
    constexpr int HPIECES = kT * HCH / 64;
    constexpr int HP = (HPIECES + NW - 1) / NW;
    constexpr int XPITCH = 256, APITCH = H * 2, YPITCH = 512;
    constexpr int X_OFF = 0, A_OFF = 2 * kT * XPITCH, Y_OFF = A_OFF + kT * APITCH, P_OFF = Y_OFF + kT * YPITCH;
    constexpr int P_BA = 0, P_BB = H, P_LNG = H + 128, P_LNB = H + 256;
    constexpr int HB_OFF = P_OFF + (H + 384) * 4;
    constexpr int SMEM = BWD ? HB_OFF + 2 * kT * APITCH : HB_OFF + kT * APITCH;
    __shared__ __attribute__((aligned(16))) unsigned char smem[SMEM];
    const uint32_t lds0 = (uint32_t)(uintptr_t)(__attribute__((address_space(3))) unsigned char*)smem;

    const int tid = threadIdx.x, lane = tid & 63, half = lane >> 5, l31 = lane & 31, l15 = lane & 15, q4 = lane >> 4;
    const int wave = __builtin_amdgcn_readfirstlane(tid >> 6);
    if ((int64_t)blockIdx.x >= p.tiles) return;
    const bool has_ln = !BWD && p.ln_g != nullptr && !p.ln_after;
    const bool ln_post = !BWD && p.ln_g != nullptr && p.ln_after;
    const bool keep_raw = !BWD && p.residual;
    const bool add_res = BWD && p.res_in != nullptr;
    const ElemRng rng_h(DROP ? p.drop_p : 0.f, p.seed_h), rng_o(DROP ? p.drop_p : 0.f, p.seed_o);
    const bool dropping = DROP && p.drop_p > 0.f;

    auto aoff = [](int row, int chunk) { return (uint32_t)(row * APITCH + ((chunk ^ (row & 15)) << 4)); };
    auto yoff = [](int row, int c4) { return (uint32_t)(row * YPITCH + ((c4 ^ (row & 15)) << 4)); };

    const int64_t x_bytes = p.tiles * kT * (int64_t)(C * 2), h_bytes = p.tiles * kT * (int64_t)(H * 2);
    const __amdgpu_buffer_rsrc_t rx = __builtin_amdgcn_make_buffer_rsrc((void*)p.x, 0, (int)std::min<int64_t>(x_bytes, 0x7FFFFE00ll), 0x00020000);
    const __amdgpu_buffer_rsrc_t rh =
        __builtin_amdgcn_make_buffer_rsrc((void*)(BWD ? p.hin : p.x), 0, BWD ? (int)std::min<int64_t>(h_bytes, 0x7FFFFE00ll) : 0, 0x00020000);
    int lane_o = lane;
    auto issue_x = [&](int64_t ti, int buf) {
        const int l15 = lane_o & 15, q4 = lane_o >> 4;
#pragma unroll
        for (int j = 0; j < XP; ++j) {
            const int pc = wave + NW * j;
            if (pc < 8) {
                const int row = 4 * pc + q4, lc = l15 ^ (row & 15);
                const uint32_t voff = lc < NCH ? (uint32_t)(((uint32_t)ti * kT + row) * (C * 2) + lc * 16) : kOob;
                __builtin_amdgcn_raw_ptr_buffer_load_lds(rx, (lds_void*)(smem + X_OFF + buf * (kT * XPITCH) + pc * 1024), 16, voff, 0, 0, 0);
            }
        }
    };
    auto issue_h = [&](int64_t ti, int buf) {
        if constexpr (BWD) {
#pragma unroll
            for (int j = 0; j < HP; ++j) {
                const int pc = wave + NW * j;
                if (pc < HPIECES) {
                    const int slot = pc * 64 + lane_o, row = slot / HCH, lc = (slot % HCH) ^ (row & 15);
                    const uint32_t voff = (uint32_t)(((uint32_t)ti * kT + row) * (H * 2) + lc * 16);
                    __builtin_amdgcn_raw_ptr_buffer_load_lds(rh, (lds_void*)(smem + HB_OFF + buf * (kT * APITCH) + pc * 1024), 16, voff, 0, 0, 0);
                }
            }
        }
    };
    int64_t ti = blockIdx.x;
    issue_x(ti, 0);
    issue_h(ti, 0);
    {
        float* ps = (float*)(smem + P_OFF);
        for (int i = tid; i < H; i += NW * 64) ps[P_BA + i] = p.ba ? p.ba[i] : 0.f;
        for (int i = tid; i < C; i += NW * 64) {
            ps[P_BB + i] = p.bb ? p.bb[i] : 0.f;
            ps[P_LNG + i] = (has_ln || ln_post) ? p.ln_g[i] : 1.f;
            ps[P_LNB + i] = (has_ln || ln_post) ? p.ln_b[i] : 0.f;
        }
    }
    bf16x8 wa[2][KS1], wb[KS2];
#pragma unroll
    for (int i = 0; i < 2; ++i)
#pragma unroll
        for (int ks = 0; ks < KS1; ++ks) wa[i][ks] = *(const bf16x8*)(p.wa + (int64_t)(64 * wave + 32 * i + l31) * C + 16 * ks + 8 * half);
#pragma unroll
    for (int ks = 0; ks < KS2; ++ks) wb[ks] = *(const bf16x8*)(p.wb + (int64_t)(16 * wave + l15) * H + 32 * ks + 8 * q4);
    asm volatile("s_waitcnt vmcnt(0)" ::: "memory");
    __syncthreads();

    const uint32_t pbase = lds0 + P_OFF, abase = lds0 + A_OFF, ybase = lds0 + Y_OFF;
    u32x4 raw[XP], raw_prev[XP];
#pragma unroll
    for (int j = 0; j < XP; ++j) raw[j] = raw_prev[j] = u32x4{0u, 0u, 0u, 0u};
    int64_t ti_prev = -1;
    int buf = 0;

    auto epilogue = [&](int64_t tp, const u32x4 (&res)[XP]) {
        const int l15 = lane_o & 15, q4 = lane_o >> 4;
#pragma unroll
        for (int j = 0; j < XP; ++j) {
            const int pc = wave + NW * j;
            if (pc < 8) {
                const int row = 4 * pc + q4, lc = l15 ^ (row & 15);
                const int lcc = lc < NCH ? lc : 0;
                u32x4 y0, y1;
                ld128x2_now(ybase + yoff(row, 2 * lcc), ybase + yoff(row, 2 * lcc + 1), y0, y1);
                float f[8];
#pragma unroll
                for (int e = 0; e < 4; ++e) {
                    f[e] = __uint_as_float(y0[e]);
                    f[4 + e] = __uint_as_float(y1[e]);
                }
                const bool valid = lc < NCH;
                const int64_t grow = tp * kT + row;
                if (ln_post) {
                    const u32x4 mw = {pack_bf16x2(f[0], f[1]), pack_bf16x2(f[2], f[3]), pack_bf16x2(f[4], f[5]), pack_bf16x2(f[6], f[7])};
                    if (valid && p.m_out) *(u32x4*)(p.m_out + grow * C + lc * 8) = mw;
                    const uint32_t ga = pbase + (P_LNG + lcc * 8) * 4, ba = pbase + (P_LNB + lcc * 8) * 4;
                    u32x4 g0, g1, b0, b1;
                    ld128x4_now(ga, ga + 16, ba, ba + 16, g0, g1, b0, b1);
                    float s1 = 0.f, s2 = 0.f;
#pragma unroll
                    for (int e = 0; e < 4; ++e) {
                        f[2 * e] = valid ? bf_lo(mw[e]) : 0.f;
                        f[2 * e + 1] = valid ? bf_hi(mw[e]) : 0.f;
                    }
                    if constexpr (DROP) {
                        if (dropping) {
                            const int64_t e0 = ((p.row0 + grow) * C) + lcc * 8;
                            uint32_t hp = 0;
                            const uint32_t ck = rng_o.template run_key<8>(e0);
#pragma unroll
                            for (int e = 0; e < 8; ++e) f[e] *= rng_o.template run_mult<8>(e0, e, ck, hp);
                        }
                    }
#pragma unroll
                    for (int e = 0; e < 8; ++e) s1 += f[e];
                    const float mean = row16_sum(s1) * (1.f / C);
#pragma unroll
                    for (int e = 0; e < 8; ++e) {
                        f[e] = valid ? f[e] - mean : 0.f;
                        s2 = fmaf(f[e], f[e], s2);
                    }
                    const float rstd = rsqrtf(row16_sum(s2) * (1.f / C) + kLnEps);
#pragma unroll
                    for (int e = 0; e < 4; ++e) {
                        f[e] = fmaf(f[e] * rstd, __uint_as_float(g0[e]), __uint_as_float(b0[e]));
                        f[4 + e] = fmaf(f[4 + e] * rstd, __uint_as_float(g1[e]), __uint_as_float(b1[e]));
                    }
                    if ((lane_o & 15) == 0 && p.mean_out) {
                        p.mean_out[grow] = mean;
                        p.rstd_out[grow] = rstd;
                    }
                    if constexpr (DROP) {
                        if (p.row_scale) {
                            const float rs = p.row_scale[(uint32_t)((p.row0 >> 5) + tp) / (uint32_t)p.tiles_per_sample];
#pragma unroll
                            for (int e = 0; e < 8; ++e) f[e] *= rs;
                        }
                    }
                }
                if (keep_raw || add_res) {
#pragma unroll
                    for (int e = 0; e < 4; ++e) {
                        f[2 * e] += bf_lo(res[j][e]);
                        f[2 * e + 1] += bf_hi(res[j][e]);
                    }
                }
                const u32x4 o = {pack_bf16x2(f[0], f[1]), pack_bf16x2(f[2], f[3]), pack_bf16x2(f[4], f[5]), pack_bf16x2(f[6], f[7])};
                if (valid) *(u32x4*)(p.out + grow * C + lc * 8) = o;
            }
        }
    };

    for (; ti < p.tiles; ti += gridDim.x) {
        asm volatile("" : "+v"(lane_o));
        const uint32_t xbase = lds0 + X_OFF + buf * (kT * XPITCH);
        const uint32_t hbase = lds0 + HB_OFF + buf * (kT * APITCH);
        const int64_t ti_next = ti + gridDim.x;
        const bool more = ti_next < p.tiles;
#pragma unroll
        for (int j = 0; j < XP; ++j) raw_prev[j] = raw[j];
        if constexpr (!BWD) {
            if (has_ln || keep_raw) {
#pragma unroll
                for (int j = 0; j < XP; ++j) {
                    const int pc = wave + NW * j;
                    if (pc < 8) {
                        const int l15 = lane_o & 15, q4 = lane_o >> 4;
                        const int row = 4 * pc + q4, lc = l15 ^ (row & 15);
                        const bool valid = lc < NCH;
                        const uint32_t addr = xbase + pc * 1024 + lane_o * 16;
                        const u32x4 v = ld128_now(addr);
                        raw[j] = v;
                        if (!has_ln) continue;
                        const int lcc = valid ? lc : 0;
                        const uint32_t ga = pbase + (P_LNG + lcc * 8) * 4, ba = pbase + (P_LNB + lcc * 8) * 4;
                        u32x4 g0, g1, b0, b1;
                        ld128x4_now(ga, ga + 16, ba, ba + 16, g0, g1, b0, b1);
                        float f[8], s1 = 0.f, s2 = 0.f;
#pragma unroll
                        for (int e = 0; e < 4; ++e) {
                            f[2 * e] = valid ? bf_lo(v[e]) : 0.f;
                            f[2 * e + 1] = valid ? bf_hi(v[e]) : 0.f;
                            s1 += f[2 * e] + f[2 * e + 1];
                        }
                        const float mean = row16_sum(s1) * (1.f / C);
#pragma unroll
                        for (int e = 0; e < 8; ++e) {
                            f[e] = valid ? f[e] - mean : 0.f;
                            s2 = fmaf(f[e], f[e], s2);
                        }
                        const float rstd = rsqrtf(row16_sum(s2) * (1.f / C) + kLnEps);
                        u32x4 o;
#pragma unroll
                        for (int e = 0; e < 4; ++e) {
                            const float ga0 = __uint_as_float(e < 2 ? g0[2 * e] : g1[2 * e - 4]), ga1 = __uint_as_float(e < 2 ? g0[2 * e + 1] : g1[2 * e - 3]);
                            const float be0 = __uint_as_float(e < 2 ? b0[2 * e] : b1[2 * e - 4]), be1 = __uint_as_float(e < 2 ? b0[2 * e + 1] : b1[2 * e - 3]);
                            o[e] = pack_bf16x2(fmaf(f[2 * e] * rstd, ga0, be0), fmaf(f[2 * e + 1] * rstd, ga1, be1));
                        }
                        st128(addr, o);
                        const int64_t grow = ti * kT + row;
                        if (valid && p.n_out) *(u32x4*)(p.n_out + grow * C + lc * 8) = o;
                        if (l15 == 0 && p.mean_out) {
                            p.mean_out[grow] = mean;
                            p.rstd_out[grow] = rstd;
                        }
                    }
                }
            }
        }
        asm volatile("s_waitcnt lgkmcnt(0)" ::: "memory");
        __builtin_amdgcn_s_barrier();
        if (more) {
            issue_x(ti_next, buf ^ 1);
            issue_h(ti_next, buf ^ 1);
        }
        if (ti_prev >= 0) epilogue(ti_prev, raw_prev);
        if constexpr (BWD) {
            if (add_res) {
                const int l15o = lane_o & 15, q4o = lane_o >> 4;
#pragma unroll
                for (int j = 0; j < XP; ++j) {
                    const int pc = wave + NW * j;
                    const int row = 4 * (pc < 8 ? pc : 0) + q4o, lc = l15o ^ (row & 15);
                    const uint16_t* src = p.res_in + (ti * kT + row) * C + (lc < NCH ? lc : 0) * 8;
                    asm volatile("global_load_dwordx4 %0, %1, off" : "=v"(raw[j]) : "v"(src) : "memory");
                }
            }
        }

        f32x16 acc[2];
        if constexpr (!BWD) {
#pragma unroll
            for (int i = 0; i < 2; ++i) {
                u32x4 bv[4];
                const uint32_t a = pbase + (P_BA + 64 * wave + 32 * i + 4 * half) * 4;
                ld128x4_now(a, a + 32, a + 64, a + 96, bv[0], bv[1], bv[2], bv[3]);
#pragma unroll
                for (int r = 0; r < 16; ++r) acc[i][r] = __uint_as_float(bv[r >> 2][r & 3]);
            }
        } else {
#pragma unroll
            for (int i = 0; i < 2; ++i)
#pragma unroll
                for (int r = 0; r < 16; ++r) acc[i][r] = 0.f;
        }
        {
            const uint32_t xa = xbase + l31 * XPITCH;
            const int sx = l31 & 15;
            u32x4 fx[2];
            fx[0] = ld128(xa + (uint32_t)(((0 + half) ^ sx) << 4));
#pragma unroll
            for (int ks = 0; ks < KS1; ++ks) {
                const int set = ks & 1;
                if (ks + 1 < KS1) {
                    fx[set ^ 1] = ld128(xa + (uint32_t)(((2 * (ks + 1) + half) ^ sx) << 4));
                    asm volatile("s_waitcnt lgkmcnt(1)" : "+v"(fx[set]));
                } else {
                    asm volatile("s_waitcnt lgkmcnt(0)" : "+v"(fx[set]));
                }
                acc[0] = __builtin_amdgcn_mfma_f32_32x32x16_bf16(wa[0][ks], as_frag(fx[set]), acc[0], 0, 0, 0);
                acc[1] = __builtin_amdgcn_mfma_f32_32x32x16_bf16(wa[1][ks], as_frag(fx[set]), acc[1], 0, 0, 0);
            }
        }
        u32x2v hw[2][4];
        const uint32_t h2base = lds0 + HB_OFF;
        const uint64_t cbase = DROP ? (uint64_t)(p.row0 + ti * kT + l31) * (uint64_t)(H / 8) + (uint64_t)(8 * wave) : 0ull;
        if constexpr (BWD) {
#pragma unroll
            for (int i = 0; i < 2; ++i)
                ld64x4_now(hbase + aoff(l31, 8 * wave + 4 * i + 0) + 8 * half, hbase + aoff(l31, 8 * wave + 4 * i + 1) + 8 * half,
                           hbase + aoff(l31, 8 * wave + 4 * i + 2) + 8 * half, hbase + aoff(l31, 8 * wave + 4 * i + 3) + 8 * half, hw[i][0],
                           hw[i][1], hw[i][2], hw[i][3]);
        }
#pragma unroll
        for (int i = 0; i < 2; ++i)
#pragma unroll
            for (int g = 0; g < 4; ++g) {
                f32x2 v[2] = {f32x2{acc[i][4 * g], acc[i][4 * g + 1]}, f32x2{acc[i][4 * g + 2], acc[i][4 * g + 3]}};
                const uint32_t off = aoff(l31, 8 * wave + 4 * i + g) + 8 * half, dst = abase + off;
                uint32_t ck = 0;
                if constexpr (DROP) {
                    if (dropping) ck = rng_h.chunk_key(cbase + (uint32_t)(4 * i + g));
                }
                auto drop2 = [&](int t) {
                    const uint32_t hh = ElemRng::pair_bits(ck, ElemRng::half_mult(half, t));
                    return f32x2{rng_h.keep_lo(hh), rng_h.keep_hi(hh)};
                };
                if constexpr (!BWD) {
                    st64(h2base + off, pack_bf16x2(v[0].x, v[0].y), pack_bf16x2(v[1].x, v[1].y));
// ... 208 lines not shown
```

heal_swin_amd/csrc/module_ops.cpp:

```cpp
#include "hs_common.h"

namespace {
inline int64_t max64(int64_t a, int64_t b) { return a > b ? a : b; }
inline int64_t round4(int64_t v) { return (v + 3) & ~(int64_t)3; }
}

extern "C" {

int64_t hs_window_attn_module_bwd_chain_workspace(int batch, int64_t n_tokens, int channels, int num_heads, int window_size) {
    const int64_t rows = (int64_t)batch * n_tokens;
    int64_t ws = hs_window_attn_bwd_workspace(batch, n_tokens, channels, num_heads, window_size, HS_BF16);
    ws = max64(ws, hs_linear_wgrad_workspace(rows, 3 * channels, channels));
    ws = max64(ws, hs_linear_wgrad_workspace(rows, channels, channels));
    ws = max64(ws, hs_layernorm_bwd_workspace(rows, channels));
    return round4(rows * channels * 5 / 2 + 4) + ws;
}

int hs_window_attn_module_bwd_chain(const void* dout, const void* x, const void* xn, const float* mean, const float* rstd, const void* qkv,
                              const void* attn_out, const float* lse, const void* qkv_w_t, const void* proj_w_t, const float* ln_gamma,
                              const float* bias, const float* head_scale, const int32_t* idx, int64_t roll, const uint8_t* labels,
                              void* dx, float* dqkv_w, float* dqkv_b, float* dproj_w, float* dproj_b, float* dln_gamma, float* dln_beta,
                              float* dbias, float* dhead_scale, float* workspace, int accumulate, int batch, int64_t n_tokens, int channels,
                              int num_heads, int window_size, unsigned flags, int dtype, void* stream) {
    using namespace hs;
    HS_CHECK_ARG(dout && qkv && attn_out && lse && qkv_w_t && proj_w_t && head_scale && dx && dqkv_w && dproj_w && dhead_scale && workspace,
                 "hs_window_attn_module_bwd_chain: null operand");
    HS_CHECK_ARG((ln_gamma != nullptr) == (x && xn && mean && rstd && dln_gamma && dln_beta),
                 "hs_window_attn_module_bwd_chain: with a LayerNorm in front pass x, xn, mean, rstd, dln_gamma, dln_beta; without it none of them");
    HS_CHECK_ARG((bias == nullptr) == (dbias == nullptr), "hs_window_attn_module_bwd_chain: bias and dbias go together");
    HS_CHECK_ARG(ln_gamma || x, "hs_window_attn_module_bwd_chain: x (the qkv Linear's input) is needed for its weight gradient");
    HS_CHECK_ARG(accumulate == 0 || accumulate == 1,
                 "hs_window_attn_module_bwd_chain: accumulate must be 0 (overwrite) or 1 (add); HS_ACC_DEFER is not taken here: the chained "
                 "kernels share one workspace");
    if (!hs_window_attn_module_supported(channels, num_heads, window_size, dtype))
        return fail(HS_ERR_UNSUPPORTED, "hs_window_attn_module_bwd_chain: bf16, window 64, head_dim 32 and C = 96 or 128 only");
    {
        const char* who = "hs_window_attn_module_bwd_chain";
        if (int st = window_attn_check_shape(who, batch, n_tokens, channels, num_heads, window_size, roll, dtype)) return st;
        const int64_t m = (int64_t)batch * n_tokens;
        const int c = channels;
        if (int st = linear_wgrad_check_shape(who, m, c, c, dtype)) return st;
        if (int st = gemm_nt_check_shape(who, c, c, c, 0, 0, 0, m, c)) return st;
        if (int st = linear_wgrad_check_shape(who, m, 3 * c, c, dtype)) return st;
        if (int st = gemm_nt_check_shape(who, 3 * c, 3 * c, 3 * c, 0, 0, 0, m, c)) return st;
        if (int st = layernorm_check_shape(who, m, c, dtype)) return st;
    }
    HS_CHECK_ALIGNED("hs_window_attn_module_bwd_chain", 16, dout, x, xn, qkv, attn_out, qkv_w_t, proj_w_t, ln_gamma, dx, dqkv_w, dqkv_b, dproj_w,
                     dproj_b, dln_gamma, dln_beta, workspace);
    const int C = channels;
    const int64_t rows = (int64_t)batch * n_tokens;
    uint16_t* d_o = (uint16_t*)workspace;
    uint16_t* dqkv = d_o + rows * C;
    uint16_t* dxn = dqkv + rows * 3 * C;
    float* ws = workspace + round4(rows * C * 5 / 2 + 4);
    const bool v1 = ln_gamma != nullptr;
    if (int st = hs_linear_wgrad(dout, attn_out, dproj_w, dproj_b, ws, rows, C, C, accumulate, dtype, stream)) return st;
    if (int st = hs_gemm_nt(dout, C, proj_w_t, C, C, nullptr, 0, nullptr, 0, 0, nullptr, d_o, nullptr, rows, C, HS_EPI_BIAS, 0.f, 0, dtype, stream))
        return st;
    const unsigned cflags = (flags & HS_ATTN_COSINE) | (accumulate ? 0u : HS_ATTN_OVERWRITE_GRADS);
    if (int st = hs_window_attn_bwd(qkv, attn_out, d_o, lse, dqkv, dbias, dhead_scale, ws, bias, head_scale, idx, roll, labels, batch, n_tokens, C,
                                    num_heads, window_size, cflags, 0.f, 0, dtype, stream))
        return st;
    const void* qkv_in = v1 ? xn : x;
    if (int st = hs_linear_wgrad(dqkv, qkv_in, dqkv_w, dqkv_b, ws, rows, 3 * C, C, accumulate, dtype, stream)) return st;
    if (!v1)
        return hs_gemm_nt(dqkv, 3 * C, qkv_w_t, 3 * C, 3 * C, nullptr, 0, nullptr, 0, 0, nullptr, dx, nullptr, rows, C, HS_EPI_BIAS, 0.f, 0, dtype,
                          stream);
    if (int st = hs_gemm_nt(dqkv, 3 * C, qkv_w_t, 3 * C, 3 * C, nullptr, 0, nullptr, 0, 0, nullptr, dxn, nullptr, rows, C, HS_EPI_BIAS, 0.f, 0, dtype,
                            stream))
        return st;
    const void* dres = (flags & HS_ATTN_RESIDUAL) ? dout : nullptr;
    if (dres) return hs_add_layernorm_bwd(dxn, dres, x, ln_gamma, mean, rstd, dx, dln_gamma, dln_beta, ws, accumulate, rows, C, dtype, stream);
    return hs_layernorm_bwd(dxn, x, ln_gamma, mean, rstd, dx, dln_gamma, dln_beta, ws, accumulate, rows, C, dtype, stream);
}

}
```

heal_swin_amd/ops/attention.py:

```python
import ctypes
import os

import torch

from .. import _lib
from .._lib import check, lib, ptr, stream_ptr
from .runtime import RT, _cast_param, _f32, _require_gpu, _sink_buffer, _timed
from .norm import LayerNormFn
from .gemm import LinearFn


class RelPosBiasFn(torch.autograd.Function):

    @staticmethod
    def forward(ctx, table, rel_idx, window_size):
        _require_gpu(table, rel_idx)
        assert rel_idx.dtype == torch.int32 and rel_idx.is_contiguous()
        t = _f32(table)
        rows, nh = t.shape
        bias = torch.empty((nh, window_size, window_size), dtype=torch.float32, device=t.device)
        check(lib.hs_rel_bias_gather(ptr(t), ptr(rel_idx), ptr(bias), rows, nh, window_size, stream_ptr(t.device)),
              "hs_rel_bias_gather")
        ctx.save_for_backward(rel_idx)
        ctx.shape = (rows, nh, window_size)
# ... 12 lines not shown
            check(lib.hs_rel_bias_scatter_grad_sorted_add(ptr(dbias), ptr(order), ptr(offsets), ptr(buf), rows, nh, ws,
                                                          stream_ptr(dbias.device)), "hs_rel_bias_scatter_grad_sorted_add")
            RT.grad_sink.deposited(ctx.table)
            return None, None, None
        dtable = torch.empty((rows, nh), dtype=torch.float32, device=dbias.device)
        check(lib.hs_rel_bias_scatter_grad_sorted(ptr(dbias), ptr(order), ptr(offsets), ptr(dtable), rows, nh, ws,
                                                  stream_ptr(dbias.device)), "hs_rel_bias_scatter_grad_sorted")
        return dtable.to(ctx.table_dtype), None, None


class CosHeadScaleFn(torch.autograd.Function):

    @staticmethod
    def forward(ctx, logit_scale):
        _require_gpu(logit_scale)
        ls = logit_scale.detach().reshape(-1)
        out = torch.empty_like(ls)
        check(lib.hs_cos_head_scale_fwd(ptr(ls), ptr(out), ls.numel(), stream_ptr(ls.device)), "hs_cos_head_scale_fwd")
        ctx.param = logit_scale
        return out

    @staticmethod
    def backward(ctx, dscale):
        p = ctx.param
        ls = p.detach().reshape(-1)
        dscale = dscale.to(torch.float32).contiguous()
        buf = _sink_buffer(p, vector=False)
        if buf is not None:
            check(lib.hs_cos_head_scale_bwd(ptr(ls), ptr(dscale), ptr(buf.view(-1)), ls.numel(), 1, stream_ptr(ls.device)), "hs_cos_head_scale_bwd")
            RT.grad_sink.deposited(p)
            return None
        d = torch.empty_like(ls)
        check(lib.hs_cos_head_scale_bwd(ptr(ls), ptr(dscale), ptr(d), ls.numel(), 0, stream_ptr(ls.device)), "hs_cos_head_scale_bwd")
        return d.view(p.shape)


def cos_head_scale(logit_scale):
    return CosHeadScaleFn.apply(logit_scale)


BATCH_ATTN_PARAMS = True


def _ptr_array(tensors):
    return (ctypes.c_void_p * len(tensors))(*[t.data_ptr() for t in tensors])


def _int_array(values):
    return (ctypes.c_int * len(values))(*[int(v) for v in values])


class RelPosBiasManyFn(torch.autograd.Function):

    @staticmethod
    def forward(ctx, rel_idx, window_size, *tables):
        _require_gpu(rel_idx, *tables)
        assert rel_idx.dtype == torch.int32 and rel_idx.is_contiguous()
        assert all(t.dtype == torch.float32 and t.is_contiguous() and t.shape[0] == tables[0].shape[0] for t in tables)
        rows, heads = tables[0].shape[0], [t.shape[1] for t in tables]
        flat = torch.empty((sum(heads), window_size, window_size), dtype=torch.float32, device=rel_idx.device)
        check(lib.hs_rel_bias_gather_many(_ptr_array([t.detach() for t in tables]), _int_array(heads), len(tables), ptr(rel_idx), ptr(flat), rows,
                                          window_size, stream_ptr(rel_idx.device)), "hs_rel_bias_gather_many")
        ctx.save_for_backward(rel_idx)
        ctx.tables, ctx.meta = tables, (rows, heads, window_size)
        ctx.set_materialize_grads(False)
        return tuple(flat.split(heads, 0))

    @staticmethod
    def backward(ctx, *dbiases):
        (rel_idx,) = ctx.saved_tensors
        rows, heads, ws = ctx.meta
        order, offsets = _rel_idx_groups(rel_idx, rows)
        grads = [None] * len(heads)
        src, dst, nh, acc, sunk = [], [], [], [], []
        for j, db in enumerate(dbiases):
            if db is None:
                continue
            db = db.to(torch.float32).contiguous()
            buf = _sink_buffer(ctx.tables[j], vector=False)
            if buf is not None:
                sunk.append(ctx.tables[j])
                out, a = buf, 1
            else:
                out, a = torch.empty((rows, heads[j]), dtype=torch.float32, device=db.device), 0
                grads[j] = out
            src.append(db), dst.append(out), nh.append(heads[j]), acc.append(a)
        if src:
            check(lib.hs_rel_bias_scatter_grad_sorted_many(_ptr_array(src), _ptr_array(dst), _int_array(nh), _int_array(acc), len(src), ptr(order),
                                                           ptr(offsets), rows, ws, stream_ptr(src[0].device)), "hs_rel_bias_scatter_grad_sorted_many")
        for t in sunk:
            RT.grad_sink.deposited(t)
        return (None, None, *grads)


def rel_pos_bias_many(rel_idx, window_size, tables):
    return RelPosBiasManyFn.apply(rel_idx, int(window_size), *tables)


class CosHeadScaleManyFn(torch.autograd.Function):

    @staticmethod
    def forward(ctx, *logit_scales):
        _require_gpu(*logit_scales)
        ls = [p.detach().reshape(-1) for p in logit_scales]
        heads = [t.numel() for t in ls]
        flat = torch.empty(sum(heads), dtype=torch.float32, device=ls[0].device)
        outs = list(flat.split(heads))
        check(lib.hs_cos_head_scale_many(_ptr_array(ls), None, _ptr_array(outs), _int_array(heads), None, len(ls), stream_ptr(flat.device)),
              "hs_cos_head_scale_many")
        ctx.params, ctx.heads = logit_scales, heads
        ctx.set_materialize_grads(False)
        return tuple(outs)

    @staticmethod
    def backward(ctx, *dscales):
        grads = [None] * len(ctx.heads)
        ls, ds, dst, nh, acc, sunk = [], [], [], [], [], []
        for j, d in enumerate(dscales):
            if d is None:
                continue
            p = ctx.params[j]
            buf = _sink_buffer(p, vector=False)
            if buf is not None:
                sunk.append(p)
                out, a = buf.view(-1), 1
            else:
                out, a = torch.empty(ctx.heads[j], dtype=torch.float32, device=d.device), 0
                grads[j] = out.view(p.shape)
            ls.append(p.detach().reshape(-1)), ds.append(d.to(torch.float32).contiguous()), dst.append(out), nh.append(ctx.heads[j]), acc.append(a)
        if ls:
            check(lib.hs_cos_head_scale_many(_ptr_array(ls), _ptr_array(ds), _ptr_array(dst), _int_array(nh), _int_array(acc), len(ls),
                                             stream_ptr(ls[0].device)), "hs_cos_head_scale_many (backward)")
        for p in sunk:
            RT.grad_sink.deposited(p)
        return tuple(grads)


def cos_head_scale_many(logit_scales):
    return CosHeadScaleManyFn.apply(*logit_scales)


_REL_IDX_GROUPS = {}


def _rel_idx_groups(rel_idx, rows):
    key = (rel_idx.data_ptr(), rel_idx.numel(), rows, rel_idx.device)
    hit = _REL_IDX_GROUPS.get(key)
    if hit is None:
        flat = rel_idx.flatten().long()
        order = torch.argsort(flat, stable=True).to(torch.int32)
        counts = torch.bincount(flat, minlength=rows)[:rows]
        offsets = torch.zeros(rows + 1, dtype=torch.int32, device=rel_idx.device)
        offsets[1:] = torch.cumsum(counts, 0).to(torch.int32)
        hit = _REL_IDX_GROUPS[key] = (order.contiguous(), offsets, rel_idx)
    return hit[0], hit[1]


FORCE_VALU_ATTENTION = False


class WindowAttnCoreFn(torch.autograd.Function):

    @staticmethod
    def forward(ctx, qkv, bias, head_scale, idx, roll, labels, num_heads, window_size, cosine, attn_drop=0.0, seed=0, pre=None):
        _require_gpu(qkv, bias, head_scale, idx, labels)
        B, N, C3 = qkv.shape
        C = C3 // 3
        qkv = qkv.contiguous()
        dt = _lib.dtype_code(qkv.dtype)
        hs = _f32(head_scale).reshape(-1)
        assert hs.numel() == num_heads
        bias_c = _f32(bias)
        flags = (_lib.HS_ATTN_COSINE if cosine else 0) | (_lib.HS_ATTN_FORCE_VALU if FORCE_VALU_ATTENTION else 0)
        if pre is not None:
            out, lse = pre
        else:
            out = torch.empty((B, N, C), dtype=qkv.dtype, device=qkv.device)
            need_grad = any(ctx.needs_input_grad[:3])
            lse = torch.empty((B, num_heads, N), dtype=torch.float32, device=qkv.device) if need_grad else None
            with _timed("window_attn_fwd", qkv.device, 4 * B * N * C * qkv.element_size(), 4 * B * N * C * window_size):
                check(lib.hs_window_attn_fwd(ptr(qkv), ptr(out), ptr(lse), ptr(bias_c), ptr(hs), ptr(idx), int(roll), ptr(labels),
                                             B, N, C, num_heads, window_size, flags, float(attn_drop), int(seed), dt,
                                             stream_ptr(qkv.device)),
                      "hs_window_attn_fwd")
        ctx.save_for_backward(qkv, out, lse, bias_c, hs, idx, labels)
        ctx.args = (B, N, C, num_heads, window_size, flags, dt, int(roll))
        ctx.drop = (float(attn_drop), int(seed))
        ctx.bias_dtype = None if bias is None else bias.dtype
        ctx.scale_meta = (head_scale.dtype, head_scale.shape)
        return out

    @staticmethod
    def backward(ctx, dout):
        qkv, out, lse, bias_c, hs, idx, labels = ctx.saved_tensors
        B, N, C, nh, ws, flags, dt, roll = ctx.args
        dout = dout.contiguous()
        dqkv = torch.empty_like(qkv)
        nb = bias_c.numel() if bias_c is not None else 0
        mfma_bf16 = qkv.dtype == torch.bfloat16 and ws == 64 and C == 32 * nh and not (flags & _lib.HS_ATTN_FORCE_VALU)
        if mfma_bf16:
            flags |= _lib.HS_ATTN_OVERWRITE_GRADS
            zeros = torch.empty(nb + hs.numel(), dtype=torch.float32, device=qkv.device)
        else:
            zeros = torch.zeros(nb + hs.numel(), dtype=torch.float32, device=qkv.device)
        dbias = zeros[:nb].view(bias_c.shape) if bias_c is not None else None
        dscale = zeros[nb:].view(hs.shape)
        nws = int(lib.hs_window_attn_bwd_workspace(B, N, C, nh, ws, dt))
        wsp = torch.empty(nws, dtype=torch.float32, device=qkv.device) if nws else None
        streams = 7 if qkv.dtype == torch.bfloat16 else 8
        with _timed("window_attn_bwd", qkv.device, streams * B * N * C * qkv.element_size(), 10 * B * N * C * ws):
            check(lib.hs_window_attn_bwd(ptr(qkv), ptr(out), ptr(dout), ptr(lse), ptr(dqkv), ptr(dbias), ptr(dscale), ptr(wsp),
                                         ptr(bias_c), ptr(hs), ptr(idx), roll, ptr(labels),
                                         B, N, C, nh, ws, flags, ctx.drop[0], ctx.drop[1], dt, stream_ptr(qkv.device)),
                  "hs_window_attn_bwd")
        dbias_out = None if dbias is None else dbias.to(ctx.bias_dtype)
        sdt, sshape = ctx.scale_meta
        dscale_out = dscale.to(sdt).reshape(sshape) if (flags & _lib.HS_ATTN_COSINE) else None
        return dqkv, dbias_out, dscale_out, None, None, None, None, None, None, None, None, None


def window_attn_core(qkv, bias, head_scale, idx, roll, labels, num_heads, window_size, cosine, attn_drop=0.0, seed=None):
    if attn_drop > 0.0 and seed is None:
        seed = int(torch.randint(0, 2 ** 62, (1,)).item())
    return WindowAttnCoreFn.apply(qkv, bias, head_scale, idx, roll, labels, num_heads, window_size, cosine,
                                  float(attn_drop), int(seed or 0))


COMP_RESIDUAL = os.environ.get("HS_COMP_RESIDUAL", "0") == "1"
COMP_RESIDUAL_LAST_STAGE = False


FUSED_ATTN_MODULE = True


def window_attn_module_ok(x, num_heads, window_size):
    return (FUSED_ATTN_MODULE and x.is_cuda and x.dtype == torch.bfloat16 and not torch.is_grad_enabled() and
            bool(lib.hs_window_attn_module_supported(x.shape[-1], num_heads, window_size, _lib.HS_BF16)))


def window_attn_module(x, qkv_w, qkv_b, proj_w, proj_b, bias, head_scale, idx, roll, labels, num_heads, window_size, cosine,
                       ln_weight=None, ln_bias=None, residual=False):
    _require_gpu(x, qkv_w, proj_w, bias, head_scale, idx, labels)
    B, N, C = x.shape
    x = x.contiguous()
    out = torch.empty_like(x)
    wq, wp = _cast_param(qkv_w, torch.bfloat16).contiguous(), _cast_param(proj_w, torch.bfloat16).contiguous()
    hs = _f32(head_scale).reshape(-1)
    flags = (_lib.HS_ATTN_COSINE if cosine else 0) | (_lib.HS_ATTN_RESIDUAL if residual else 0)
    nbytes = (3 if residual else 2) * B * N * C * 2
    flops = B * N * (8 * C * C + 4 * window_size * C)
    with _timed("window_attn_module_fwd", x.device, nbytes, flops):
        check(lib.hs_window_attn_module_fwd(ptr(x), ptr(out), ptr(wq), ptr(_f32(qkv_b)), ptr(wp), ptr(_f32(proj_b)), ptr(_f32(ln_weight)),
                                            ptr(_f32(ln_bias)), ptr(_f32(bias)), ptr(hs), ptr(idx), int(roll), ptr(labels), B, N, C,
                                            num_heads, window_size, flags, _lib.HS_BF16, stream_ptr(x.device)),
              "hs_window_attn_module_fwd")
    return out


FUSED_ATTN_MODULE_TRAIN = os.environ.get("HS_FUSED_ATTN_TRAIN", "1") != "0"
FUSED_NORM2 = False


def window_attn_module_train_ok(x, num_heads, window_size):
    return (FUSED_ATTN_MODULE_TRAIN and x.is_cuda and x.dtype == torch.bfloat16 and torch.is_grad_enabled() and
            not FORCE_VALU_ATTENTION and bool(lib.hs_window_attn_module_supported(x.shape[-1], num_heads, window_size, _lib.HS_BF16)))


def window_attn_module_train(x, ln_weight, ln_bias, qkv_w, qkv_b, proj_w, proj_b, bias, head_scale, idx, roll, labels, num_heads,
                             window_size, cosine, residual_alias=False, norm2=None):
    _require_gpu(x, qkv_w, proj_w, bias, head_scale, idx, labels)
    B, N, C = x.shape
    x = x.contiguous()
    dev = x.device
    has_ln = ln_weight is not None
    out, o = torch.empty_like(x), torch.empty_like(x)
    xn = torch.empty_like(x) if has_ln else None
    qkv = torch.empty((B, N, 3 * C), dtype=x.dtype, device=dev)
    mean = torch.empty(B * N, dtype=torch.float32, device=dev) if has_ln else None
    rstd = torch.empty(B * N, dtype=torch.float32, device=dev) if has_ln else None
    lse = torch.empty((B, num_heads, N), dtype=torch.float32, device=dev)
    n2 = mean2 = rstd2 = None
    if norm2 is not None:
        assert has_ln and not residual_alias
        n2 = torch.empty_like(x)
        mean2 = torch.empty(B * N, dtype=torch.float32, device=dev)
        rstd2 = torch.empty(B * N, dtype=torch.float32, device=dev)
    wq, wp = _cast_param(qkv_w, torch.bfloat16).contiguous(), _cast_param(proj_w, torch.bfloat16).contiguous()
    hs = _f32(head_scale).reshape(-1)
    flags = (_lib.HS_ATTN_COSINE if cosine else 0) | (_lib.HS_ATTN_RESIDUAL if has_ln else 0)
    with _timed("window_attn_module_fwd_train", dev, ((9 if has_ln else 6) + (1 if n2 is not None else 0)) * B * N * C * 2,
                B * N * (8 * C * C + 4 * window_size * C)):
        check(lib.hs_window_attn_module_fwd_train(ptr(x), ptr(out), ptr(xn), ptr(mean), ptr(rstd), ptr(qkv), ptr(o), ptr(lse), ptr(wq),
                                                  ptr(_f32(qkv_b)), ptr(wp), ptr(_f32(proj_b)), ptr(_f32(ln_weight)), ptr(_f32(ln_bias)),
                                                  ptr(_f32(bias)), ptr(hs), ptr(idx), int(roll), ptr(labels),
                                                  ptr(None if n2 is None else _f32(norm2[0])), ptr(None if n2 is None else _f32(norm2[1])),
                                                  ptr(n2), ptr(mean2), ptr(rstd2), B, N, C, num_heads,
                                                  window_size, flags, _lib.HS_BF16, stream_ptr(dev)),
              "hs_window_attn_module_fwd_train")
    if not has_ln:
        x_res = None
        if residual_alias:
            qkv_t, x_res = LinearFn.apply(x, qkv_w, qkv_b, True, None, (qkv,))
        else:
            qkv_t = LinearFn.apply(x, qkv_w, qkv_b, False, None, (qkv,))
        o_t = WindowAttnCoreFn.apply(qkv_t, bias, head_scale, idx, roll, labels, num_heads, window_size, cosine, 0.0, 0, (o, lse))
        y = LinearFn.apply(o_t, proj_w, proj_b, False, None, (out,))
        return (y, x_res) if residual_alias else y
    assert not residual_alias
    n1, xs = LayerNormFn.apply(x, ln_weight, ln_bias, None, None, True, None, False, (xn, mean, rstd))
    qkv_t = LinearFn.apply(n1, qkv_w, qkv_b, False, None, (qkv,))
    o_t = WindowAttnCoreFn.apply(qkv_t, bias, head_scale, idx, roll, labels, num_heads, window_size, cosine, 0.0, 0, (o, lse))
    x1 = LinearFn.apply(o_t, proj_w, proj_b, False, xs, (out,))
    if n2 is None:
        return x1
    return LayerNormFn.apply(x1, norm2[0], norm2[1], None, None, True, None, False, (n2, mean2, rstd2))
```

heal_swin_amd/ops/gemm.py:

```python
import math
import os

import torch

from .. import _lib
from .._lib import check, lib, ptr, stream_ptr
from . import runtime
from .runtime import RT, _aligned, _cast_param, _defer_flag, _defer_keep, _require_gpu, _sink_buffer, _timed


OWN_GEMM = os.environ.get("HS_OWN_GEMM", "auto")


OWN_GELU_MAX_K = 4096
OWN_DGELU_MAX_K = 1024
OWN_BIAS_MAX_K = 0


class GemmTuner:
    MIN_FLOP = 1 << 33

    def __init__(self):
        self.picks = {}
        self.trials = {}
# ... 25 lines not shown
            for rep in range(4):
                for own in (True, False):
                    a, w = sets[rep & 1]
                    e0, e1 = torch.cuda.Event(enable_timing=True), torch.cuda.Event(enable_timing=True)
                    e0.record()
                    if own:
                        gemm_nt(a, w, bias32)
                    else:
                        torch.nn.functional.linear(a, w, bias16)
                    e1.record()
                    e1.synchronize()
                    if rep:
                        best[own] = min(best[own], e0.elapsed_time(e1))
            del sets
        self.trials[key] = (round(1e3 * best[True], 1), round(1e3 * best[False], 1))
        self.picks[key] = best[True] <= best[False]
        return self.picks[key]


GEMM_TUNE = True
GEMM_TUNER = GemmTuner()


def own_gemm_ok(epi, n, k, dtype, k2=0, m=None):
    if dtype != torch.bfloat16 or OWN_GEMM == "0" or k % 8 or k2 % 8 or n % 8 or n < 16:
        return False
    if OWN_GEMM == "1" or RT.prefer_own_gemm:
        return True
    kk = k + k2
    if epi == _lib.HS_EPI_DGELU:
        return kk <= OWN_DGELU_MAX_K
    if epi == _lib.HS_EPI_GELU:
        return kk <= OWN_GELU_MAX_K
    if OWN_BIAS_MAX_K > 0:
        return kk <= OWN_BIAS_MAX_K
    if GEMM_TUNE and m is not None and k2 == 0 and torch.cuda.is_available():
        pick = GEMM_TUNER.pick(int(m), n, kk, torch.device("cuda", torch.cuda.current_device()))
        if pick is not None:
            return pick
    return kk <= 128 or n <= 128 or (n <= 256 and kk <= 256)


RESID_DGRAD_OWN = True


def own_gemm_legal(n, k, dtype):
    return dtype == torch.bfloat16 and OWN_GEMM != "0" and k % 8 == 0 and n % 8 == 0 and n >= 16


RESID_EPILOGUE = True


def gemm_nt(a2d, w, bias=None, epi=0, aux=None, a2=None, w2=None, want_c=True, drop_p=0.0, seed=0):
    w, w2, bias = _aligned(w), _aligned(w2), _aligned(bias)
    if epi != _lib.HS_EPI_GELU:
        aux = _aligned(aux)
    m, k = a2d.shape
    n = w.shape[0]
    assert a2d.stride(1) == 1 and w.stride(1) == 1 and a2d.dtype == torch.bfloat16 and w.dtype == torch.bfloat16
    c = torch.empty((m, n), dtype=torch.bfloat16, device=a2d.device) if want_c else None
    if epi == _lib.HS_EPI_GELU:
        aux = torch.empty((m, n), dtype=torch.bfloat16, device=a2d.device)
    k2 = 0 if a2 is None else a2.shape[1]
    if bias is not None and bias.dtype != torch.float32:
        bias = bias.float()
    with _timed(f"hs_gemm_nt epi={epi} m={m} n={n} k={k + k2}", a2d.device, 2 * (m * (k + k2) + n * (k + k2) + m * n * (2 if (epi and want_c) else 1)), 2 * m * n * (k + k2)):
        check(lib.hs_gemm_nt(ptr(a2d), a2d.stride(0), ptr(w), w.stride(0), k, ptr(a2), 0 if a2 is None else a2.stride(0), ptr(w2),
                             0 if w2 is None else w2.stride(0), k2, ptr(bias), ptr(c), ptr(aux), m, n, epi, float(drop_p), int(seed),
                             _lib.HS_BF16, stream_ptr(a2d.device)), "hs_gemm_nt")
    return c, aux


def _lib_tag(kind, m, n, k):
    return f"lib {kind} m={m} n={n} k={k}"


FP32_GEMM = os.environ.get("HS_FP32_GEMM", "bf16x3")
_BF16X3_MIN = 160
_SPLIT_MEMO = []
_MM_OUT_DTYPE = [None]


def _bf16x3_ok(x, n=None, k=None):
    ok = FP32_GEMM == "bf16x3" and x.dtype == torch.float32 and x.is_cuda and x.shape[-1] % 8 == 0
    ok = ok and (n is None or n * k >= _BF16X3_MIN * (n + k))
    if ok and _MM_OUT_DTYPE[0] is None:
        _probe_mm_out_dtype(x.device)
    return ok and _MM_OUT_DTYPE[0] is not False


def _probe_mm_out_dtype(device):
    try:
        a = torch.zeros((8, 8), dtype=torch.bfloat16, device=device)
        torch.mm(a, a, out_dtype=torch.float32)
        _MM_OUT_DTYPE[0] = True
    except Exception:
        _MM_OUT_DTYPE[0] = False
        import warnings
        warnings.warn("heal_swin_amd: torch.mm(..., out_dtype=) is unavailable in this PyTorch build; fp32 Linear products run as "
                      "exact fp32 GEMMs (HS_FP32_GEMM=strict behaviour) instead of bf16x3")


def split3(x2d, mode):
    x2d = _aligned(x2d.contiguous())
    key = (x2d.data_ptr(), tuple(x2d.shape), x2d._version, mode)
    for kk, _, t in _SPLIT_MEMO:
        if kk == key:
            return t
    rows, k = x2d.shape
    out = torch.empty((rows, 3 * k), dtype=torch.bfloat16, device=x2d.device)
    check(lib.hs_split_bf16x3(ptr(x2d), ptr(out), rows, k, mode, stream_ptr(x2d.device)), "hs_split_bf16x3")
    if mode == 0:
        _SPLIT_MEMO.append((key, x2d, out))
        del _SPLIT_MEMO[:-2]
    return out


class _Split:

    def __init__(self, t3, k):
        self.t3, self.shape, self.dtype, self.device = t3, (t3.shape[0], k), torch.float32, t3.device

    def is_contiguous(self):
        return True

    def record_stream(self, stream):
        self.t3.record_stream(stream)

    def dim(self):
        return 2


def _split_of(x2d):
    if isinstance(x2d, _Split):
        return x2d.t3
    if x2d is None or x2d.dtype != torch.float32:
        return None
    key = (x2d.data_ptr(), tuple(x2d.shape), x2d._version, 0)
    for kk, _, t in _SPLIT_MEMO:
        if kk == key:
            return t
    return None


_WSPLIT = {}
_WSPLIT_CAPACITY = 1024


def _weight_split(w2d, transposed):
    key = (w2d.untyped_storage().data_ptr(), w2d.storage_offset(), tuple(w2d.shape), tuple(w2d.stride()), bool(transposed))
    hit = _WSPLIT.get(key)
    if hit is not None and hit[0] == w2d._version and hit[1] == RT.weight_epoch:
        return hit[3]
    src = _aligned(w2d.t().contiguous() if transposed else w2d.contiguous())
    rows, k = src.shape
    out = torch.empty((rows, 3 * k), dtype=torch.bfloat16, device=src.device)
    check(lib.hs_split_bf16x3(ptr(src), ptr(out), rows, k, 1, stream_ptr(src.device)), "hs_split_bf16x3")
    if len(_WSPLIT) >= _WSPLIT_CAPACITY:
        for old in list(_WSPLIT)[:_WSPLIT_CAPACITY // 2]:
            del _WSPLIT[old]
    _WSPLIT[key] = (w2d._version, RT.weight_epoch, w2d.detach(), out)
    return out


def _mm_f32(a3, b3t, bias=None):
    if _MM_OUT_DTYPE[0] is None:
        _probe_mm_out_dtype(a3.device)
    if not _MM_OUT_DTYPE[0]:
        raise RuntimeError("HS_FP32_GEMM=bf16x3 needs torch.mm(..., out_dtype=torch.float32); set HS_FP32_GEMM=strict")
    if bias is None:
        return torch.mm(a3, b3t, out_dtype=torch.float32)
    if _MM_OUT_DTYPE[0] is True:
        try:
            y = torch.addmm(bias, a3, b3t, out_dtype=torch.float32)
            _MM_OUT_DTYPE[0] = "addmm"
            return y
        except Exception:
            _MM_OUT_DTYPE[0] = "mm"
    if _MM_OUT_DTYPE[0] == "addmm":
        return torch.addmm(bias, a3, b3t, out_dtype=torch.float32)
    return torch.mm(a3, b3t, out_dtype=torch.float32).add_(bias)


def _lib_linear(x2, w, b):
    if isinstance(x2, _Split):
        m, k = x2.shape
        with _timed(_lib_tag("fwd bf16x3", m, w.shape[0], 3 * k), x2.device, 4 * (m * k + m * w.shape[0]), 6 * m * k * w.shape[0]):
            return _mm_f32(x2.t3, _weight_split(w.reshape(w.shape[0], k), False).t(), b)
    m, k = x2.shape[0] if x2.dim() == 2 else x2.numel() // x2.shape[-1], x2.shape[-1]
    if _bf16x3_ok(x2, w.shape[0], k) and w.dtype == torch.float32 and w.shape[0] % 8 == 0:
        with _timed(_lib_tag("fwd bf16x3", m, w.shape[0], 3 * k), x2.device, 4 * (m * k + m * w.shape[0]), 6 * m * k * w.shape[0]):
            y = _mm_f32(split3(x2.reshape(m, k), 0), _weight_split(w.reshape(w.shape[0], k), False).t(), b)
        return y.view(x2.shape[:-1] + (w.shape[0],))
    with _timed(_lib_tag("fwd", m, w.shape[0], k), x2.device, 2 * (m * k + m * w.shape[0]), 2 * m * k * w.shape[0]):
        return torch.nn.functional.linear(x2, w, b)


def _lib_matmul(dy2, w, res=None):
    m, n = dy2.shape
    if isinstance(dy2, _Split):
        with _timed(_lib_tag("dgrad bf16x3", m, w.shape[1], 3 * n), dy2.device, 4 * (m * n + m * w.shape[1]), 6 * m * n * w.shape[1]):
            return _mm_f32(dy2.t3, _weight_split(w, True).t(), res)
    if _bf16x3_ok(dy2, w.shape[1], n) and w.dtype == torch.float32 and w.shape[1] % 8 == 0:
        with _timed(_lib_tag("dgrad bf16x3", m, w.shape[1], 3 * n), dy2.device, 4 * (m * n + m * w.shape[1]), 6 * m * n * w.shape[1]):
            dx = _mm_f32(split3(dy2, 0), _weight_split(w, True).t(), res)
        return dx
    with _timed(_lib_tag("dgrad", m, w.shape[1], n), dy2.device, 2 * (m * n + m * w.shape[1]), 2 * m * n * w.shape[1]):
        return dy2 @ w if res is None else torch.addmm(res, dy2, w)


def _cast_param_t(p, dtype, cache=None):
    if cache is None:
        cache = RT.cast_cache if RT.cast_cache is not None else RT.last_cast_cache
    c = cache.get_t(p, dtype) if (cache is not None and p.dim() == 2 and cache.current(p)) else None
    if c is None:
        n_out = p.shape[0]
        c = p.detach().to(dtype).view(n_out, -1).t().contiguous()
    return c


def _wgrad_group_ok(dy2, x2, n_out, k_in, want_b, bbuf, x3):
    return bool(runtime.WGRAD_GROUP and x3 is None and x2 is not None and x2.dtype == torch.bfloat16 and dy2.dtype == torch.bfloat16 and
                (bbuf is not None or not want_b) and _defer_flag(dy2.device) and
                lib.hs_linear_wgrad_group_variant(dy2.shape[0], n_out, k_in, _lib.HS_BF16) == 1)


def _wgrad_issue(members, dev):
    rows = members[0][0].shape[0]
    arr = _lib.wgrad_problems(members)
    ws = torch.empty(int(lib.hs_linear_wgrad_group_workspace(arr, len(members), rows, _lib.HS_BF16)), dtype=torch.float32, device=dev)
    with _timed("linear_wgrad" if len(members) == 1 else "linear_wgrad group", dev, sum(2 * rows * (m[4] + m[5]) for m in members),
                sum(2 * rows * m[4] * m[5] for m in members)):
        check(lib.hs_linear_wgrad_group(arr, len(members), ptr(ws), rows, _lib.HS_BF16, stream_ptr(dev)), "hs_linear_wgrad_group")
    _defer_keep(dev, ws)


def _wgrad_grouped(member):
    dev = member[0].device
    s = torch.cuda.current_stream(dev).cuda_stream
    parked = runtime._PARKED.pop(s, None)
    if parked is not None and parked[0].shape[0] == member[0].shape[0]:
        _wgrad_issue([parked, member], dev)
        return
    if parked is not None:
        _wgrad_issue([parked], dev)
    runtime._PARKED[s] = member


def _wgrad_flush_parked(s, device=None):
    parked = runtime._PARKED.pop(s, None)
    if parked is not None:
        _wgrad_issue([parked], parked[0].device)


runtime._PARK_FLUSH[:] = [_wgrad_flush_parked]


def _param_grads(dy2, x2, weight, bias, want_w, want_b, x3=None, gelu_x=False):
    n_out = weight.shape[0]
    k_in = weight.numel() // n_out
    if not (want_w or want_b):
        return None, None
    if x2 is None:
        assert x3 is not None and dy2.dtype == torch.float32
        hip_ok = dy2.is_contiguous() and n_out % 8 == 0
        assert hip_ok
    else:
        hip_ok = (x2.is_contiguous() and dy2.is_contiguous() and n_out % 4 == 0 and
                  ((x2.dtype == torch.bfloat16 and k_in % 8 == 0) or (x2.dtype == torch.float32 and k_in % 4 == 0)))
    wbuf = _sink_buffer(weight) if (hip_ok and want_w) else None
    bbuf = _sink_buffer(bias) if (wbuf is not None and want_b) else None
    if wbuf is not None and (not want_b or bbuf is not None):
        aw = RT.async_wgrad
        wbuf = wbuf.view(n_out, k_in)
        if aw is not None:
            cur = torch.cuda.current_stream(dy2.device)
            aw.stream.wait_stream(cur)
            dy2.record_stream(aw.stream)
            (x2 if x2 is not None else x3).record_stream(aw.stream)
            with torch.cuda.stream(aw.stream):
                LinearFn._wgrad_hip(dy2, x2, n_out, k_in, want_b, wbuf, bbuf, x3, gelu_x)
        elif _wgrad_group_ok(dy2, x2, n_out, k_in, want_b, bbuf, x3):
            _wgrad_grouped((dy2, x2, wbuf, bbuf if want_b else None, n_out, k_in, 1 | _lib.HS_ACC_DEFER, gelu_x))
        else:
            LinearFn._wgrad_hip(dy2, x2, n_out, k_in, want_b, wbuf, bbuf, x3, gelu_x)
        RT.grad_sink.deposited(weight)
        if want_b:
            RT.grad_sink.deposited(bias)
        return None, None
    dw = db = None
    if hip_ok:
        dw32, db32 = LinearFn._wgrad_hip(dy2, x2, n_out, k_in, want_b, x3=x3, gelu_x=gelu_x)
        dw = dw32.to(weight.dtype).view(weight.shape) if want_w else None
        db = db32.to(bias.dtype) if want_b else None
    else:
        assert not gelu_x
        if want_w:
            dw = (dy2.t() @ x2).to(weight.dtype).view(weight.shape)
        if want_b:
            db = dy2.sum(0).to(bias.dtype)
    return dw, db


class LinearFn(torch.autograd.Function):

    @staticmethod
    def forward(ctx, x, weight, bias, passthrough=False, residual=None, pre=None):
        _require_gpu(x, weight, bias, residual)
        n_out = weight.shape[0]
        k_in = weight.numel() // n_out
        w = _cast_param(weight, x.dtype).view(n_out, k_in)
        ctx.x_shape = x.shape
        ctx.bias_param = bias
        ctx.w_cast = w if w.dtype != weight.dtype else None
        ctx.cast_cache = RT.cast_cache
        ctx.passthrough = passthrough
        ctx.has_residual = residual is not None
        ctx.x3 = None
        if pre is not None:
            y = pre[0]
        elif residual is not None:
            assert not passthrough
            if own_gemm_legal(n_out, k_in, x.dtype) and x.is_contiguous():
                res2 = residual.reshape(-1, n_out)
                res2 = res2 if res2.is_contiguous() else res2.contiguous()
                y = gemm_nt(x.reshape(-1, k_in), w, bias, _lib.HS_EPI_RESID, aux=res2)[0].view(x.shape[:-1] + (n_out,))
            else:
                y = _lib_linear(x, w, None if bias is None else _cast_param(bias, x.dtype)) + residual
                ctx.x3 = _split_of(x.reshape(-1, k_in)) if x.is_contiguous() else None
        elif own_gemm_ok(_lib.HS_EPI_BIAS, n_out, k_in, x.dtype, m=x.numel() // k_in) and x.is_contiguous():
            y = gemm_nt(x.reshape(-1, k_in), w, bias)[0].view(x.shape[:-1] + (n_out,))
        else:
            y = _lib_linear(x, w, None if bias is None else _cast_param(bias, x.dtype))
            ctx.x3 = _split_of(x.reshape(-1, k_in)) if x.is_contiguous() else None
        ctx.save_for_backward(None if ctx.x3 is not None else x, weight)
        return (y, x.view_as(x)) if passthrough else y

    @staticmethod
    def _wgrad_hip(dy2, x2, n_out, k_in, want_b, dw_out=None, db_out=None, x3=None, gelu_x=False):
        rows = dy2.shape[0]
        dev = dy2.device
        accumulate = 1 if dw_out is not None else 0
        defer = _defer_flag(dev) if (dw_out is not None and (db_out is not None or not want_b)) else 0
        dw32 = dw_out if dw_out is not None else torch.empty((n_out, k_in), dtype=torch.float32, device=dev)
        db32 = None
        if want_b:
            db32 = db_out if db_out is not None else torch.empty(n_out, dtype=torch.float32, device=dev)
        nws = int(lib.hs_linear_wgrad_workspace(rows, n_out, k_in))
        ws = torch.empty(nws, dtype=torch.float32, device=dev)
        if x3 is not None or (_bf16x3_ok(x2, n_out, k_in) and n_out % 8 == 0 and x2.dtype == dy2.dtype):
            dy3 = dy2.t3 if isinstance(dy2, _Split) else split3(dy2, 0)
            x3 = x3 if x3 is not None else split3(x2, 0)
            aw = RT.async_wgrad
            if aw is not None and torch.cuda.current_stream(dev) == aw.stream:
                dy3.record_stream(aw.stream)
                x3.record_stream(aw.stream)
            with _timed("linear_wgrad bf16x3", dev, 3 * 2 * rows * (n_out + k_in), 6 * rows * n_out * k_in):
                for i, (yo, xo, dbp) in enumerate(((0, 0, db32), (0, 2 * k_in, None), (2 * n_out, 0, db32))):
                    d = defer if i == 2 else 0
                    check(lib.hs_linear_wgrad_ld(ptr(dy3), 3 * n_out, yo, ptr(x3), 3 * k_in, xo, ptr(dw32), ptr(dbp), ptr(ws), rows,
                                                 n_out, k_in, (1 if (accumulate or i) else 0) | d, stream_ptr(dev)), "hs_linear_wgrad_ld")
                if defer:
                    _defer_keep(dev, ws)
            return dw32, db32
        with _timed("linear_wgrad", dev, x2.element_size() * rows * (n_out + k_in), 2 * rows * n_out * k_in):
            if gelu_x:
                check(lib.hs_linear_wgrad_gelu(ptr(dy2), ptr(x2), ptr(dw32), ptr(db32), ptr(ws), rows, n_out, k_in, accumulate | defer,
                                               _lib.dtype_code(x2.dtype), stream_ptr(dev)), "hs_linear_wgrad_gelu")
            else:
                check(lib.hs_linear_wgrad(ptr(dy2), ptr(x2), ptr(dw32), ptr(db32), ptr(ws), rows, n_out, k_in, accumulate | defer,
                                          _lib.dtype_code(x2.dtype), stream_ptr(dev)), "hs_linear_wgrad")
        if defer:
            _defer_keep(dev, ws)
        return dw32, db32

    @staticmethod
    def backward(ctx, dy, dx_res=None):
        x, weight = ctx.saved_tensors
        bias = ctx.bias_param
        n_out = weight.shape[0]
        k_in = weight.numel() // n_out
        if dy is None:
            return dx_res, None, None, None, None, None
        dy2 = dy.reshape(-1, n_out)
        x2 = None if x is None else x.reshape(-1, k_in)
        if not dy2.is_contiguous():
            dy2 = dy2.contiguous()
        dx = None
        if ctx.needs_input_grad[0]:
            dx = _input_grad(dy2, weight, ctx.w_cast, None if dx_res is None else dx_res.reshape(-1, k_in), ctx.cast_cache).reshape(ctx.x_shape)
        ctx.w_cast = ctx.cast_cache = None
        x3, ctx.x3 = ctx.x3, None
        dw, db = _param_grads(dy2, x2, weight, bias, ctx.needs_input_grad[1], bias is not None and ctx.needs_input_grad[2], x3)
        return dx, dw, db, None, (dy if ctx.has_residual else None), None


def _input_grad(dy2, weight, w_cast, dx_res2=None, cache=None):
    n_out = weight.shape[0]
    k_in = weight.numel() // n_out
    epi = _lib.HS_EPI_BIAS if dx_res2 is None else _lib.HS_EPI_RESID
    if own_gemm_ok(epi, k_in, n_out, dy2.dtype, m=dy2.shape[0]) or (dx_res2 is not None and RESID_DGRAD_OWN and own_gemm_legal(k_in, n_out, dy2.dtype)):
        res = None if dx_res2 is None else dx_res2.to(dy2.dtype).contiguous()
        return gemm_nt(dy2, _cast_param_t(weight, dy2.dtype, cache), None, epi, aux=res)[0]
    w = w_cast if (w_cast is not None and w_cast.dtype == dy2.dtype) else (
        weight if weight.dtype == dy2.dtype else weight.to(dy2.dtype)).view(n_out, k_in)
    if dx_res2 is not None:
        return _lib_matmul(dy2, w, dx_res2.to(dy2.dtype))
    return _lib_matmul(dy2, w)


def linear(x, weight, bias=None):
    return LinearFn.apply(x, weight, bias)


def linear_residual(x, weight, bias, residual):
    return LinearFn.apply(x, weight, bias, False, residual)


def linear_passthrough(x, weight, bias=None):
    return LinearFn.apply(x, weight, bias, True)




class PadSliceFn(torch.autograd.Function):

    @staticmethod
    def forward(ctx, x, n):
        ctx.shape, ctx.n = x.shape, n
        return x[..., :n]

    @staticmethod
    def backward(ctx, g):
        full = RT.zero_padded_grads.pop(g.data_ptr(), None)
        if (full is not None and g._base is full and full.numel() == math.prod(ctx.shape) and full.dtype == g.dtype and
                g.shape == ctx.shape[:-1] + (ctx.n,) and g.stride() == full.view(ctx.shape)[..., :ctx.n].stride()):
            return full.view(ctx.shape), None
        out = g.new_zeros(ctx.shape)
        out[..., :ctx.n] = g
        return out, None


def pad_slice(x, n):
    return PadSliceFn.apply(x, n)
```

include/healswin.h:

```cpp
#ifndef HEALSWIN_H
#define HEALSWIN_H

#include <stdint.h>

#ifdef __cplusplus
extern "C" {
#endif

typedef enum {
    HS_OK = 0,
    HS_ERR_INVALID_ARG = 1,
    HS_ERR_UNSUPPORTED = 2,
    HS_ERR_HIP = 3,
    HS_ERR_NOT_PERMUTATION = 4,
    HS_ERR_MISALIGNED = 5
} hs_status;

typedef enum { HS_F32 = 0, HS_BF16 = 1 } hs_dtype;

#define HS_ATTN_COSINE 1u
#define HS_ATTN_FORCE_VALU 2u
#define HS_ATTN_RESIDUAL 4u
#define HS_ATTN_OVERWRITE_GRADS 8u

const char* hs_version(void);
const char* hs_last_error(void);
const char* hs_status_string(int status);
int hs_device_count(void);

int hs_transpose_many_16(const void* jobs, int count, int blocks_per_job, void* stream);

int hs_set_reserved_cus(int n);
int hs_get_reserved_cus(void);
int hs_set_seed_epoch(const void* counter);
const void* hs_get_seed_epoch(void);
int hs_debug_occupy_cus(int n_workgroups, int threads, int lds_bytes, double microseconds, void* stream);
int hs_debug_buffer_soffset_probe(const void* src, int bytes, int soffset, void* out128, void* stream);


int hs_nest2ring(int nside, const int64_t* in, int64_t* out, int64_t n);
int hs_ring2nest(int nside, const int64_t* in, int64_t* out, int64_t n);

int hs_nest_win_idcs(int window_size, int64_t* out);

int hs_rel_pos_index(int window_size, int64_t* out);


int hs_build_nest_roll_shift(int64_t n_pix, int window_size, int shift_size,
                             int32_t* idx, int32_t* inv, uint8_t* labels);
int hs_build_nest_grid_shift(int nside, int base_pix, int window_size,
                             int32_t* idx, int32_t* inv, uint8_t* labels);
int hs_build_ring_shift(int nside, int base_pix, int window_size, int shift_size,
                        int32_t* idx, int32_t* inv, uint8_t* labels);

int hs_attn_mask_from_labels(const uint8_t* labels, int64_t n, int window_size, float* out);

int hs_rel_bias_gather(const float* table, const int32_t* rel_idx, float* bias,
                       int table_rows, int num_heads, int window_size, void* stream);
int hs_rel_bias_scatter_grad(const float* dbias, const int32_t* rel_idx, float* dtable,
                             int table_rows, int num_heads, int window_size, void* stream);
int hs_rel_bias_scatter_grad_sorted(const float* dbias, const int32_t* order, const int32_t* offsets, float* dtable,
                                    int table_rows, int num_heads, int window_size, void* stream);
int hs_rel_bias_scatter_grad_sorted_add(const float* dbias, const int32_t* order, const int32_t* offsets, float* dtable,
                                        int table_rows, int num_heads, int window_size, void* stream);
int hs_cos_head_scale_fwd(const float* logit_scale, float* scale, int num_heads, void* stream);
int hs_cos_head_scale_bwd(const float* logit_scale, const float* dscale, float* dlogit_scale, int num_heads, int accumulate, void* stream);
int hs_rel_bias_gather_many(const void* const* tables, const int* heads, int count, const int32_t* rel_idx, float* bias_base,
                            int table_rows, int window_size, void* stream);
int hs_rel_bias_scatter_grad_sorted_many(const void* const* dbias, void* const* dtables, const int* heads, const int* accumulate, int count,
                                         const int32_t* order, const int32_t* offsets, int table_rows, int window_size, void* stream);
int hs_cos_head_scale_many(const void* const* logit_scale, const void* const* dscale, void* const* out, const int* heads, const int* accumulate,
                           int count, void* stream);

int hs_window_attn_fwd(const void* qkv, void* out, float* lse,
                       const float* bias, const float* head_scale,
                       const int32_t* idx, int64_t roll, const uint8_t* labels,
                       int batch, int64_t n_tokens, int channels, int num_heads, int window_size,
                       unsigned flags, float attn_drop, uint64_t seed, int dtype, void* stream);

int64_t hs_window_attn_bwd_workspace(int batch, int64_t n_tokens, int channels, int num_heads, int window_size, int dtype);
int hs_window_attn_bwd(const void* qkv, const void* out, const void* dout, const float* lse,
                       void* dqkv, float* dbias, float* dhead_scale, float* workspace,
                       const float* bias, const float* head_scale,
                       const int32_t* idx, int64_t roll, const uint8_t* labels,
                       int batch, int64_t n_tokens, int channels, int num_heads, int window_size,
                       unsigned flags, float attn_drop, uint64_t seed, int dtype, void* stream);

int hs_gather_rows(const void* x, void* out, const int32_t* idx, int64_t roll,
                   int batch, int64_t n_tokens, int64_t row_bytes, void* stream);

int hs_layernorm_fwd(const void* x, const void* residual, const float* gamma, const float* beta,
                     void* y, float* mean, float* rstd,
                     int64_t rows, int width, int dtype, void* stream);
int64_t hs_layernorm_bwd_workspace(int64_t rows, int width);
int hs_layernorm_bwd(const void* dy, const void* x, const float* gamma, const float* mean, const float* rstd,
                     void* dx, float* dgamma, float* dbeta, float* workspace, int accumulate,
                     int64_t rows, int width, int dtype, void* stream);

int hs_add_layernorm_fwd(const void* a, const void* b, const float* gamma, const float* beta,
                         void* sum_out, void* y, float* mean, float* rstd,
                         int64_t rows, int width, int dtype, void* stream);
int hs_add_layernorm_bwd(const void* dy, const void* dsum, const void* sum, const float* gamma,
                         const float* mean, const float* rstd, void* dx, float* dgamma, float* dbeta, float* workspace,
                         int accumulate, int64_t rows, int width, int dtype, void* stream);

int hs_layernorm_drop_fwd(const void* x, const void* residual, const float* gamma, const float* beta, void* y,
                          float* mean, float* rstd, const float* row_scale, int64_t rows_per_sample, float drop_p,
                          uint64_t seed, int64_t rows, int width, int dtype, void* stream);
int hs_layernorm_drop_bwd(const void* dy, const void* x, const float* gamma, const float* mean, const float* rstd,
                          void* dx, float* dgamma, float* dbeta, float* workspace, int accumulate, const float* row_scale,
                          int64_t rows_per_sample, float drop_p, uint64_t seed, int64_t rows, int width, int dtype,
                          void* stream);
int hs_add_layernorm_drop_fwd(const void* a, const void* b, const float* gamma, const float* beta, void* sum_out, void* y,
                              float* mean, float* rstd, const float* row_scale, int64_t rows_per_sample, float drop_p,
                              uint64_t seed, int64_t rows, int width, int dtype, void* stream);
int hs_layernorm_fwd_ex(const void* x, const void* residual, const void* add_in, const void* lo_in, const float* gamma,
                        const float* beta, void* y, void* sum_out, void* lo_out, float* mean, float* rstd,
                        const float* row_scale, int64_t rows_per_sample, float drop_p, uint64_t seed, int64_t rows, int width,
                        int dtype, void* stream);
int hs_add_layernorm_drop_bwd(const void* dy, const void* dsum, const void* sum, const float* gamma, const float* mean,
                              const float* rstd, void* da, void* db, float* dgamma, float* dbeta, float* workspace, int accumulate,
                              const float* row_scale, int64_t rows_per_sample, float drop_p, uint64_t seed,
                              int64_t rows, int width, int dtype, void* stream);

int hs_gelu_fwd(const void* x, void* y, int64_t n, float drop_p, uint64_t seed, int dtype, void* stream);
int hs_gelu_bwd(const void* dy, const void* x, void* dx, int64_t n, float drop_p, uint64_t seed, int dtype, void* stream);

int hs_residual_drop(const void* x, const void* t, void* out, const float* row_scale, int64_t elems_per_sample, int64_t n,
                     float drop_p, uint64_t seed, int dtype, void* stream);

int64_t hs_seg_ce_partials(int64_t batch, int64_t npix);
int hs_seg_ce_fwd(const void* logits, const void* labels, const float* class_weights, float* partials,
                  int64_t batch, int64_t npix, int n_classes, int64_t stride_b, int64_t stride_k, int64_t stride_p,
                  int label_bytes, int64_t ignore_index, int dtype, void* stream);
int hs_seg_ce_bwd(const void* logits, const void* labels, const float* class_weights, const float* scale, void* dlogits,
                  int64_t batch, int64_t npix, int n_classes, int64_t stride_b, int64_t stride_k, int64_t stride_p,
                  int64_t dstride_b, int64_t dstride_k, int64_t dstride_p, int label_bytes, int64_t ignore_index,
                  int dtype, void* stream);

#define HS_DEPTH_L1 0
#define HS_DEPTH_L2 1
#define HS_DEPTH_HUBER 2
#define HS_DEPTH_LOGVAR 3
int64_t hs_depth_loss_partials(int64_t batch, int64_t npix);
int hs_depth_loss_fwd(const void* pred, const float* target, float* partials, int64_t batch, int64_t npix, int channels,
                      int64_t stride_b, int64_t stride_c, int64_t stride_p, int kind, float huber_delta, int dtype, void* stream);
int hs_depth_loss_bwd(const void* pred, const float* target, const float* scale, void* dpred, int64_t batch, int64_t npix, int channels,
                      int64_t stride_b, int64_t stride_c, int64_t stride_p, int64_t dstride_b, int64_t dstride_c, int64_t dstride_p,
                      int kind, float huber_delta, int dtype, void* stream);

int64_t hs_linear_wgrad_workspace(int64_t rows, int n_out, int k_in);
int hs_linear_wgrad(const void* dy, const void* x, float* dw, float* dbias, float* workspace,
                    int64_t rows, int n_out, int k_in, int accumulate, int dtype, void* stream);
int hs_linear_wgrad_gelu_supported(int64_t rows, int n_out, int k_in, int dtype);
int hs_linear_wgrad_gelu(const void* dy, const void* h, float* dw, float* dbias, float* workspace, int64_t rows, int n_out, int k_in,
                         int accumulate, int dtype, void* stream);
typedef struct hs_wgrad_problem {
    const void* dy;
    const void* x;
    float* dw;
    float* dbias;
    int n_out, k_in, accumulate, gelu_x;
} hs_wgrad_problem;
int hs_linear_wgrad_group_variant(int64_t rows, int n_out, int k_in, int dtype);
int64_t hs_linear_wgrad_group_workspace(const hs_wgrad_problem* problems, int count, int64_t rows, int dtype);
int hs_linear_wgrad_group(const hs_wgrad_problem* problems, int count, float* workspace, int64_t rows, int dtype, void* stream);

#define HS_ACC_DEFER 2
int hs_reduce_pending(void* stream);
int hs_reduce_flush(void* stream);

#define HS_MLP_NORM_AFTER 16u
int hs_mlp_fused_supported(int channels, int hidden, int dtype);
int hs_mlp_fused_fwd(const void* x, const float* ln_gamma, const float* ln_beta, const void* w1, const float* b1, const void* w2,
                     const float* b2, void* n_out, float* mean_out, float* rstd_out, void* h_out, void* act_out, void* out, int64_t rows,
                     int channels, int hidden, unsigned flags, int dtype, void* stream);
int hs_mlp_fused_bwd(const void* dy, const void* h, const void* w2_t, const void* w1_t, const void* dres, void* dh, void* dn, int64_t rows,
                     int channels, int hidden, int dtype, void* stream);
int hs_mlp_fused_drop_fwd(const void* x, const float* ln_gamma, const float* ln_beta, const void* w1, const float* b1, const void* w2,
                          const float* b2, void* m_out, float* mean_out, float* rstd_out, void* h_out, void* act_out, void* out,
                          const float* row_scale, int64_t rows_per_sample, float drop_p, uint64_t seed_hidden, uint64_t seed_out,
                          int64_t rows, int channels, int hidden, unsigned flags, int dtype, void* stream);
int hs_mlp_fused_drop_bwd(const void* dy, const void* h, const void* w2_t, const void* w1_t, const void* dres, void* dh, void* dn,
                          float drop_p, uint64_t seed_hidden, int64_t rows, int channels, int hidden, int dtype, void* stream);

int hs_adam_step(float* p, const float* g, float* m, float* v, void* p_bf16, int64_t n, float lr, const float* lr_dev, float beta1,
                 float beta2, float eps, float weight_decay, int decoupled, const int64_t* step, void* stream);
int hs_adam_advance(int64_t* step, void* stream);

#define HS_ADAM_MAX_GROUPS 32
typedef struct {
    const float* lr_dev;
    float lr;
    float beta1, beta2, eps, weight_decay;
    int32_t decoupled;
} hs_adam_group;
int hs_adam_max_groups(void);
int hs_adam_step_groups(float* p, const float* g, float* m, float* v, void* p_bf16, int64_t n, const hs_adam_group* groups, int n_groups,
                        const int32_t* runs, int n_runs, const int32_t* block_first, int n_blocks, int64_t covered, const int64_t* step,
                        void* stream);

typedef struct {
    float total_norm;
    float clip_coef;
    int32_t finite;
    int32_t reserved;
} hs_grad_guard;
int hs_grad_guard_piece(void);
int hs_grad_stats(const float* g, int64_t n, const int64_t* items, int n_items, double* partials, void* stream);
int hs_grad_guard_finalize(const double* partials, int64_t n_items, const int32_t* params, int n_params, int norm_inf, float max_norm,
                           float* param_norm, double* work, hs_grad_guard* guard, void* stream);
int hs_adam_step_guarded(float* p, const float* g, float* m, float* v, void* p_bf16, int64_t n, float lr, const float* lr_dev, float beta1,
                         float beta2, float eps, float weight_decay, int decoupled, const int64_t* step, float clip_value,
                         const hs_grad_guard* guard, int skip_nonfinite, void* stream);
int hs_adam_step_groups_guarded(float* p, const float* g, float* m, float* v, void* p_bf16, int64_t n, const hs_adam_group* groups,
                                int n_groups, const int32_t* runs, int n_runs, const int32_t* block_first, int n_blocks, int64_t covered,
                                const int64_t* step, float clip_value, const hs_grad_guard* guard, int skip_nonfinite, void* stream);
int hs_adam_advance_guarded(int64_t* step, const hs_grad_guard* guard, int skip_nonfinite, int64_t* skipped, void* stream);
int hs_grad_scale(float* g, int64_t n, float clip_value, const hs_grad_guard* guard, void* stream);

int hs_weight_avg_update(float* avg, const float* p, int64_t n, int kind, float decay, const int64_t* n_averaged, const hs_grad_guard* guard,
                         int skip_nonfinite, void* stream);
int hs_weight_avg_advance(int64_t* n_averaged, const hs_grad_guard* guard, int skip_nonfinite, void* stream);
int hs_weight_avg_swap(float* p, float* avg, void* p_bf16, int64_t n, void* stream);

int hs_window_attn_module_supported(int channels, int num_heads, int window_size, int dtype);
int hs_window_attn_module_fwd(const void* x, void* out, const void* qkv_w, const float* qkv_b, const void* proj_w,
                              const float* proj_b, const float* ln_gamma, const float* ln_beta, const float* bias,
                              const float* head_scale, const int32_t* idx, int64_t roll, const uint8_t* labels, int batch,
                              int64_t n_tokens, int channels, int num_heads, int window_size, unsigned flags, int dtype,
                              void* stream);

int hs_window_attn_module_fwd_train(const void* x, void* out, void* xn_out, float* mean_out, float* rstd_out, void* qkv_out,
                                    void* attn_out, float* lse_out, const void* qkv_w, const float* qkv_b, const void* proj_w,
                                    const float* proj_b, const float* ln_gamma, const float* ln_beta, const float* bias,
                                    const float* head_scale, const int32_t* idx, int64_t roll, const uint8_t* labels,
                                    const float* norm2_gamma, const float* norm2_beta, void* n2_out, float* mean2_out, float* rstd2_out,
                                    int batch, int64_t n_tokens, int channels, int num_heads, int window_size, unsigned flags, int dtype,
                                    void* stream);

int64_t hs_window_attn_module_bwd_chain_workspace(int batch, int64_t n_tokens, int channels, int num_heads, int window_size);
int hs_window_attn_module_bwd_chain(const void* dout, const void* x, const void* xn, const float* mean, const float* rstd, const void* qkv,
                              const void* attn_out, const float* lse, const void* qkv_w_t, const void* proj_w_t, const float* ln_gamma,
                              const float* bias, const float* head_scale, const int32_t* idx, int64_t roll, const uint8_t* labels,
                              void* dx, float* dqkv_w, float* dqkv_b, float* dproj_w, float* dproj_b, float* dln_gamma, float* dln_beta,
                              float* dbias, float* dhead_scale, float* workspace, int accumulate, int batch, int64_t n_tokens, int channels,
                              int num_heads, int window_size, unsigned flags, int dtype, void* stream);

#define HS_EPI_BIAS 0
#define HS_EPI_GELU 1
#define HS_EPI_DGELU 2
#define HS_EPI_RESID 3
int hs_gemm_nt(const void* a, int64_t lda, const void* b, int64_t ldb, int k, const void* a2, int64_t lda2, const void* b2,
               int64_t ldb2, int k2, const float* bias, void* c, void* aux, int64_t m, int n, int epilogue, float drop_p,
               uint64_t seed, int dtype, void* stream);
int hs_gemm_nt_set_tile(int variant);
int hs_gemm_nt_tile_variant(int64_t m, int n, int k, int k2, int epilogue);

int hs_pix2ang_nest(int nside, int64_t first, int64_t count, double* theta, double* phi);
int hs_sample_bilinear_u8(const void* img, int batch, int channels, int height, int width, const double* rx, const double* ry,
                          int64_t n, void* out, void* stream);
int hs_sample_mask_u8(const void* mask, int batch, int height, int width, const double* rx, const double* ry, int64_t n,
                      int background, void* out, void* stream);

typedef struct hs_fisheye_camera {
    double k[8];
    double cx_offset, cy_offset, aspect_ratio;
    int poly_order, width, height;
} hs_fisheye_camera;
int hs_hp_rotated_coords(int nside, int64_t first_pix, int64_t count, const hs_fisheye_camera* cam, const double* rot, int batch,
                         double* u, double* v, void* stream);
int hs_sample_bilinear_u8_per_sample(const void* img, int batch, int channels, int height, int width, const double* rx,
                                     const double* ry, int64_t n, void* out, void* stream);
int hs_sample_mask_u8_per_sample(const void* mask, int batch, int height, int width, const double* rx, const double* ry, int64_t n,
                                 int background, void* out, void* stream);

#define HS_PRED_LABELS 2
#define HS_PRED_ROWS16 4
int hs_hp_interp_weights_nest(int nside, const double* theta, const double* phi, int64_t n, int64_t* pix, double* wgt);
int hs_backproject_labels(const void* pred, int pred_kind, int64_t batch, int64_t npix, int n_classes, int64_t stride_b,
                          int64_t stride_k, int64_t stride_p, const int32_t* nearest, int64_t n_out, int background, uint8_t* out,
                          void* stream);
int hs_backproject_image(const uint8_t* hp_img, int64_t planes, int64_t npix, const int32_t* idx, const double* wgt, int64_t n_out,
                         double* out, void* stream);
int hs_seg_confusion(const void* pred, int pred_kind, int64_t batch, int64_t npix, int n_classes, int64_t stride_b, int64_t stride_k,
                     int64_t stride_p, const int32_t* nearest, int64_t n_out, const uint8_t* target, int uncovered, int64_t* conf,
                     int64_t* bad, void* stream);

#define HS_F64 3
#define HS_DS_N 0
#define HS_DS_SE 1
#define HS_DS_AE 2
#define HS_DS_MEAN_SE 3
#define HS_DS_MEAN_AE 4
#define HS_DS_PRED 5
#define HS_DS_SIL_N 6
#define HS_DS_SIL_D 7
#define HS_DS_SIL_D2 8
#define HS_DS_INV_N 9
#define HS_DS_INV_SE 10
#define HS_DS_STD_N 11
#define HS_DS_STD 12
#define HS_DS_RANGE 13
#define HS_DEPTH_NSUMS 29
int64_t hs_depth_points_workspace(int64_t batch, int64_t n);
int hs_depth_points(const void* depth, int kind, int64_t batch, int64_t n, int64_t width, int64_t stride_b, int64_t stride_h,
                    int64_t stride_w, const uint8_t* foreground, int64_t fg_stride_b, const float* background, int n_background,
                    const double* dir, void* workspace, float* points, int64_t* offsets, void* stream);
int hs_chamfer_nn(const float* a, const int64_t* a_off, int64_t a_rows, int64_t a_max, const float* b, const int64_t* b_off,
                  int64_t b_rows, int64_t b_max, int64_t batch, int splits, void* workspace, float* dist_a, float* dist_b,
                  int64_t* idx_a, int64_t* idx_b, double* term, void* stream);
int64_t hs_depth_metrics_partials(int64_t total);
int hs_depth_metrics(const void* pred, int pred_kind, int64_t batch, int64_t n, int64_t width, int64_t stride_b, int64_t stride_c,
                     int64_t stride_h, int64_t stride_w, const void* target, int target_kind, int64_t t_stride_b, int64_t t_stride_h,
                     int64_t t_stride_w, int use_logvar, double total_mean, const float* ranges, int n_ranges, double* partial,
                     double* state, void* stream);
int hs_backproject_depth(const void* pred, int kind, int64_t batch, int64_t npix, int64_t stride_b, int64_t stride_p, const int32_t* idx,
                         const double* wgt, int64_t n_out, double* out, void* stream);

int hs_flat_depth_to_hp(const void* pred, int kind, int64_t batch, int64_t n_src, int64_t stride_b, int64_t stride_p, const int32_t* nearest,
                        const int32_t* idx, const float* wgt, int64_t n, float* out, void* stream);
int hs_depth_metrics_gather(const void* pred, int pred_kind, int64_t batch, int64_t n_src, int64_t stride_b, int64_t stride_c, int64_t stride_p,
                            const int32_t* nearest, const int32_t* idx, const float* wgt, int64_t n, const void* target, int target_kind,
                            int64_t t_stride_b, int64_t t_stride_p, int use_logvar, double total_mean, const float* ranges, int n_ranges,
                            double* partial, double* state, void* stream);

#define HS_HISTOGRAM_MAX_BINS 4096
#define HS_DT_NONE 0
#define HS_DT_LOG 1
#define HS_DT_INV 2
#define HS_DT_ZERO_BKG 1
#define HS_DT_1000_BKG 2
#define HS_DT_AFFINE 4
#define HS_DT_INVERSE 8
#define HS_DSTAT_TOTAL 0
#define HS_DSTAT_BACKGROUND 1
#define HS_DSTAT_VALUES 2
#define HS_DSTAT_FINITE 3
#define HS_DSTAT_POSINF 4
#define HS_DSTAT_NEGINF 5
#define HS_DSTAT_NAN 6
#define HS_DSTAT_FG_VALUES 7
#define HS_DSTAT_FG_POSINF 8
#define HS_DSTAT_FG_NAN 9
#define HS_DSTAT_NCOUNTS 10
#define HS_DEPTH_STATS_WORDS 15
int hs_sample_bilinear_u8_f32(const void* img, int batch, int channels, int height, int width, const double* rx, const double* ry,
                              int64_t n, float* out, void* stream);
int hs_sample_nearest_f32(const float* src, int batch, int height, int width, const double* rx, const double* ry, int64_t n,
                          float background, float* out, void* stream);
int hs_sample_bilinear_u8_f32_per_sample(const void* img, int batch, int channels, int height, int width, const double* rx,
                                         const double* ry, int64_t n, float* out, void* stream);
int hs_sample_nearest_f32_per_sample(const float* src, int batch, int height, int width, const double* rx, const double* ry, int64_t n,
                                     float background, float* out, void* stream);
int hs_depth_target(const float* in, int64_t in_stride_b, int64_t in_stride_p, float* out, int64_t out_stride_b, int64_t out_stride_p,
                    int64_t batch, int64_t n, int flags, int transform, float shift, float scale, void* stream);
int64_t hs_depth_stats_partials(int64_t n);
int hs_depth_stats_update(const float* depth, int64_t n, int transform, int use_masking, int64_t* partial, int64_t* state, void* stream);
int hs_depth_stats_merge(const int64_t* states, int count, int64_t* state, void* stream);
int hs_histogram_update(const float* depth, int64_t n, int transform, int use_masking, const double* edges, int bins, int64_t* counts,
                        void* stream);

int64_t hs_select_rows_workspace(int rows);
int hs_select_rows(const float* x, int rows, int64_t n, int64_t row_stride, int64_t k, int nan_propagates, int splits, void* workspace,
                   float* out, void* stream);

int hs_ln_head_supported(int width, int n_classes, int dtype);
int64_t hs_ln_head_partials(int64_t rows);
int hs_ln_head_fwd(const void* y, const void* wfold, const float* bvec, void* logits, float* mean, float* rstd, int64_t rows,
                   int width, int dtype, int logits_dtype, void* stream);
int hs_ln_head_bwd(const void* y, const float* mean, const float* rstd, const void* dlogits, const void* afold, void* dy,
                   void* dprime, float* partials, int64_t rows, int width, int dtype, int logits_dtype, void* stream);

int hs_split_bf16x3(const float* x, void* out, int64_t rows, int k, int mode, void* stream);
int hs_gelu_split3(const float* dy, const float* x, void* out3, int64_t rows, int k, float drop_p, uint64_t seed, void* stream);
int hs_linear_wgrad_ld(const void* dy, int64_t ldy, int64_t ycol0, const void* x, int64_t ldx, int64_t xcol0, float* dw, float* dbias,
                       float* workspace, int64_t rows, int n_out, int k_in, int accumulate, void* stream);

int hs_expand_ln_head_supported(int width, int children, int n_classes, int dtype);
int hs_expand_ln_head_fwd(const void* xn, const void* xn_lo, const void* wexp, const void* wfold, const float* bvec, void* y, float* logits,
                          float* mean, float* rstd, int64_t tokens, int width, int children, int dtype, void* stream);

int64_t hs_expand_ln_head_blocks(int64_t tokens);
int hs_expand_ln_head_ce_fwd(const void* xn, const void* xn_lo, const void* wexp, const void* wfold, const float* bvec, const uint8_t* labels,
                             const float* class_weights, int n_classes, void* y, float* logits, float* mean, float* rstd,
                             float* loss_partials, int64_t tokens, int width, int children, int dtype, void* stream);
int hs_expand_ln_head_ce_step_fwd(const void* xn, const void* xn_lo, const void* wexp, const void* wfold, const float* bvec,
                                  const uint8_t* labels, const float* class_weights, int n_classes, void* y, float* logits, float* mean,
                                  float* rstd, float* loss_partials, uint8_t* preds, int64_t* confmat, int64_t* bad, int64_t tokens,
                                  int width, int children, int dtype, void* stream);
int hs_ln_head_ce_bwd(const void* y, const float* mean, const float* rstd, const uint8_t* labels, const float* class_weights,
                      const float* scale, int n_classes, const void* wfold, const float* bvec, const void* afold, void* dy, void* dprime,
                      float* partials, int64_t rows, int width, int dtype, void* stream);

int hs_expand_ln_head_depth_fwd(const void* xn, const void* xn_lo, const void* wexp, const void* wfold, const float* bvec, const float* target,
                                int kind, float huber_delta, int n_out, void* y, float* logits, float* mean, float* rstd, float* loss_partials,
                                int64_t tokens, int width, int children, int dtype, void* stream);
int hs_expand_ln_head_depth_step_fwd(const void* xn, const void* xn_lo, const void* wexp, const void* wfold, const float* bvec,
                                     const float* target, int kind, float huber_delta, int n_out, void* y, float* logits, float* mean,
                                     float* rstd, float* loss_partials, int flags, int transform, float shift, float scale, int use_logvar,
                                     double total_mean, const float* ranges, int n_ranges, double* metric_partials, double* metric_state,
                                     float* preds, float* logvar_out, int64_t tokens, int width, int children, int dtype, void* stream);
int hs_ln_head_depth_bwd(const void* y, const float* mean, const float* rstd, const float* target, int kind, float huber_delta,
                         const float* scale, int n_out, const void* wfold, const float* bvec, const void* afold, void* dy, void* dprime,
                         float* partials, int64_t rows, int width, int dtype, void* stream);

int hs_patch_merge_fwd(const void* x, const float* gamma, const float* beta, const void* w, void* normed, float* mean, float* rstd,
                       void* out, int64_t rows, int dim, int dim_out, int dtype, void* stream);
int64_t hs_patch_merge_bwd_workspace(int64_t rows, int dim, int dim_out);
int hs_patch_merge_bwd(const void* dout, const void* x, const void* normed, const float* gamma, const float* mean, const float* rstd,
                       const void* w_t, void* dnormed, void* dx, float* dw, float* dgamma, float* dbeta, float* workspace,
                       int accumulate, int64_t rows, int dim, int dim_out, int dtype, void* stream);
int hs_patch_expand_fwd(const void* x, const void* w, const float* gamma, const float* beta, void* expanded, float* mean, float* rstd,
                        void* out, int64_t rows, int dim, int dim_exp, int children, int dtype, void* stream);
int64_t hs_patch_expand_bwd_workspace(int64_t rows, int dim, int dim_exp, int children);
int hs_patch_expand_bwd(const void* dout, const void* x, const void* expanded, const float* gamma, const float* mean, const float* rstd,
                        const void* w_t, void* dexpanded, void* dx, float* dw, float* dgamma, float* dbeta, float* workspace,
                        int accumulate, int64_t rows, int dim, int dim_exp, int children, int dtype, void* stream);

int hs_flat_zorder(int Ht, int Wt, int T, int32_t* z_of_rm, int32_t* rm_of_z);
int hs_build_flat_shift(int Ht, int Wt, int T, int w, int s, int32_t* idx, int32_t* inv, uint8_t* labels);
int hs_flat_rel_pos_index(int w, int64_t* row_major, int64_t* zorder);
int hs_flat_attn_mask(int Ht, int Wt, int w, int s, float* out);

#define HS_U8 8
#define HS_I32 9
#define HS_I64 10
#define HS_FLAT_PATCH_ROWS 0
#define HS_FLAT_PIXEL_ROWS 1
int hs_flat_img_to_rows(const void* img, int in_dtype, void* rows, int out_dtype, int batch, int nch, int H, int W, int p, int T,
                        int mode, int64_t ld, void* stream);
int hs_flat_rows_to_img(const void* rows, int in_dtype, void* img, int out_dtype, int batch, int nch, int H, int W, int p, int T,
                        int mode, int64_t ld, void* stream);

#define HS_FLAT_IMAGE 2
int64_t hs_flat_resize_lds_bytes(int nch, int src_dtype, int tile_h, int tile_w, int span_h, int span_w);
int hs_flat_resize(const void* src, int src_dtype, int64_t src_stride_b, int batch, int nch, int H0, int W0, const int32_t* row_idx,
                   const float* row_wgt, const int32_t* col_idx, const float* col_wgt, void* out, int out_dtype, int H, int W, int layout,
                   int p, int T, int64_t ld, int tile_h, int tile_w, int span_h, int span_w, int flags, int transform, float shift,
                   float scale, void* stream);

#ifdef __cplusplus
}
#endif
#endif
```

Before: 57.32.

## Fuse qkv linear backward dgrad, wgrad and bias grad into one streaming kernel

Adds a HIP kernel that reads each 32-row tile of dy and x once into LDS through multi-buffered async buffer loads. From that one read it computes the weight-gradient partials, the bias sum and the input gradient dx, with a deferred epilogue. It is wired into the Python qkv LinearFn backward and into the C attention backward chain for bf16 with C=96 or 128. This replaces separate wgrad and dgrad GEMM launches that each re-read dy, at the cost of a per-block partial workspace reduction plus hand-tuned vmcnt and LDS-swizzle logic.

```diff
diff --git a/heal_swin_amd/_lib.py b/heal_swin_amd/_lib.py
--- a/heal_swin_amd/_lib.py
+++ b/heal_swin_amd/_lib.py
@@ -205,6 +205,9 @@
     "hs_window_attn_module_fwd_train": [c_ptr] * 17 + [c_i64] + [c_ptr] * 6 + [c_int, c_i64, c_int, c_int, c_int, c_uint, c_int, c_ptr],
     "hs_window_attn_module_bwd_chain": [c_ptr] * 14 + [c_i64] + [c_ptr] * 11 + [c_int, c_int, c_i64, c_int, c_int, c_int, c_uint, c_int, c_ptr],
     "hs_layernorm_bwd": [c_ptr, c_ptr, c_ptr, c_ptr, c_ptr, c_ptr, c_ptr, c_ptr, c_ptr, c_int, c_i64, c_int, c_int, c_ptr],
+    "hs_attn_half_bwd_supported": [c_int, c_int],
+    "hs_proj_bwd_fused": [c_ptr] * 7 + [c_i64, c_int, c_int, c_int, c_ptr],
+    "hs_qkv_bwd_fused": [c_ptr] * 7 + [c_i64, c_int, c_int, c_int, c_ptr],
     "hs_patch_merge_fwd": [c_ptr, c_ptr, c_ptr, c_ptr, c_ptr, c_ptr, c_ptr, c_ptr, c_i64, c_int, c_int, c_int, c_ptr],
     "hs_patch_merge_bwd": [c_ptr, c_ptr, c_ptr, c_ptr, c_ptr, c_ptr, c_ptr, c_ptr, c_ptr, c_ptr, c_ptr, c_ptr, c_ptr, c_int, c_i64,
                            c_int, c_int, c_int, c_ptr],
@@ -233,6 +236,7 @@
     "hs_ln_head_partials": ([c_i64], c_i64),
     "hs_expand_ln_head_blocks": ([c_i64], c_i64),
     "hs_linear_wgrad_workspace": ([c_i64, c_int, c_int], c_i64),
+    "hs_attn_half_bwd_workspace": ([c_i64, c_int, c_int], c_i64),
     "hs_linear_wgrad_group_workspace": ([c_ptr, c_int, c_i64, c_int], c_i64),
     "hs_window_attn_bwd_workspace": ([c_int, c_i64, c_int, c_int, c_int, c_int], c_i64),
     "hs_patch_merge_bwd_workspace": ([c_i64, c_int, c_int], c_i64),
diff --git a/heal_swin_amd/csrc/attn_half_bwd.hip b/heal_swin_amd/csrc/attn_half_bwd.hip
--- /dev/null
+++ b/heal_swin_amd/csrc/attn_half_bwd.hip
@@ -0,0 +1,278 @@
+#include <algorithm>
+
+#include "hs_lds.h"
+#include "hs_wgrad_device.h"
+
+namespace hs {
+namespace {
+
+typedef __attribute__((ext_vector_type(4))) short s16x4;
+typedef __attribute__((ext_vector_type(8))) short s16x8;
+
+constexpr int kT = 32;
+
+struct HalfBwdParams {
+    const uint16_t* dy;
+    const uint16_t* x;
+    const uint16_t* wt;
+    uint16_t* dx;
+    float* part;
+    int64_t tiles;
+    int want_bias;
+};
+
+__device__ __forceinline__ int swz(int row) { return ((row & 3) << 2) | ((row >> 2) & 3); }
+
+__device__ __forceinline__ s16x4 ld_tr(uint32_t addr) {
+    s16x4 v;
+    asm volatile("ds_read_b64_tr_b16 %0, %1" : "=v"(v) : "v"(addr));
+    return v;
+}
+
+template <int C, int NM>
+__global__ void __launch_bounds__(C * 4, 1) linear_bwd_fused_kernel(HalfBwdParams p) {
+#if defined(__HIP_DEVICE_COMPILE__)
+    constexpr int N = NM * C, NW = C / 16, KB = C / 32, NBLK = N / 32, NBW = (NBLK + 1) / 2, KS2 = N / 32;
+    constexpr int NCH = C / 8, NCHY = N / 8, YCH = NM == 1 ? 16 : 48;
+    constexpr int YPITCH = YCH * 16, XPITCH = 256, SPITCH = 512;
+    constexpr int YPIECES = kT * YCH / 64, YP = (YPIECES + NW - 1) / NW, XP = (8 + NW - 1) / NW;
+    constexpr int YB = kT * YPITCH, XB = kT * XPITCH, SB = kT * SPITCH;
+    constexpr int D = NM == 3 ? 2 : 4, NS = D + 1;
+    constexpr int Y_OFF = 0, X_OFF = NS * YB, S_OFF = X_OFF + NS * XB, SMEM = S_OFF + 2 * SB;
+    static_assert(NW == 2 * KB && NCHY <= YCH && SMEM >= NW * 512 * 4 && SMEM <= 160 * 1024, "wave roles / tile extents");
+    constexpr int L_LO = YPIECES / NW + 8 / NW, S_LO = 8 / NW, HI_WAVES = 8 % NW;
+    constexpr int L_HI = L_LO + 1 + (YPIECES % NW ? 1 : 0), S_HI = S_LO + 1;
+    constexpr int VM_LO = S_LO + (D - 1) * (L_LO + S_LO), VM_HI = S_HI + (D - 1) * (L_HI + S_HI);
+    static_assert(YPIECES % NW == 0 || YPIECES % NW == HI_WAVES, "the waves with an extra dy piece are those with an extra x piece");
+    static_assert(VM_HI < 64, "vmcnt is 6 bits");
+    __shared__ __attribute__((aligned(16))) unsigned char smem[SMEM];
+    const uint32_t lds0 = (uint32_t)(uintptr_t)(__attribute__((address_space(3))) unsigned char*)smem;
+
+    const int tid = threadIdx.x, lane = tid & 63, l15 = lane & 15, q4 = lane >> 4;
+    const int wave = __builtin_amdgcn_readfirstlane(tid >> 6);
+    const int kb = wave % KB, wn = wave / KB;
+    if ((int64_t)blockIdx.x >= p.tiles) return;
+
+    auto soff = [](int row, int c4) { return (uint32_t)(row * SPITCH + ((c4 ^ (row & 15)) << 4)); };
+
+    const int64_t y_bytes = p.tiles * kT * (int64_t)(N * 2), x_bytes = p.tiles * kT * (int64_t)(C * 2);
+    const __amdgpu_buffer_rsrc_t ry = __builtin_amdgcn_make_buffer_rsrc((void*)p.dy, 0, (int)std::min<int64_t>(y_bytes, 0x7FFFFE00ll), 0x00020000);
+    const __amdgpu_buffer_rsrc_t rx = __builtin_amdgcn_make_buffer_rsrc((void*)p.x, 0, (int)std::min<int64_t>(x_bytes, 0x7FFFFE00ll), 0x00020000);
+    int lane_o = lane;
+    auto issue = [&](int64_t ti, int buf) {
+#pragma unroll
+        for (int j = 0; j < YP; ++j) {
+            const int pc = wave + NW * j;
+            if (pc < YPIECES) {
+                const int slot = pc * 64 + lane_o, row = slot / YCH, lc = (slot % YCH) ^ swz(row);
+                const uint32_t voff = lc < NCHY ? (uint32_t)(((uint32_t)ti * kT + row) * (N * 2) + lc * 16) : kOob;
+                __builtin_amdgcn_raw_ptr_buffer_load_lds(ry, (lds_void*)(smem + Y_OFF + buf * YB + pc * 1024), 16, voff, 0, 0, 0);
+            }
+        }
+#pragma unroll
+        for (int j = 0; j < XP; ++j) {
+            const int pc = wave + NW * j;
+            if (pc < 8) {
+                const int row = 4 * pc + (lane_o >> 4), lc = (lane_o & 15) ^ swz(row);
+                const uint32_t voff = lc < NCH ? (uint32_t)(((uint32_t)ti * kT + row) * (C * 2) + lc * 16) : kOob;
+                __builtin_amdgcn_raw_ptr_buffer_load_lds(rx, (lds_void*)(smem + X_OFF + buf * XB + pc * 1024), 16, voff, 0, 0, 0);
+            }
+        }
+    };
+    int64_t ti = blockIdx.x;
+#pragma unroll
+    for (int d = 0; d < D; ++d)
+        if (ti + (int64_t)d * gridDim.x < p.tiles) issue(ti + (int64_t)d * gridDim.x, d);
+
+    bf16x8 wb[KS2];
+#pragma unroll
+    for (int ks = 0; ks < KS2; ++ks) wb[ks] = *(const bf16x8*)(p.wt + (int64_t)(16 * wave + l15) * N + 32 * ks + 8 * q4);
+    f32x16 acc[NBW][1];
+    zero(acc);
+    float bsum[8] = {0.f, 0.f, 0.f, 0.f, 0.f, 0.f, 0.f, 0.f};
+    const bool want_bias = p.want_bias != 0;
+
+    auto epilogue = [&](int64_t tp, uint32_t sb) {
+#pragma unroll
+        for (int j = 0; j < XP; ++j) {
+            const int pc = wave + NW * j;
+            if (pc < 8) {
+                const int row = 4 * pc + (lane_o >> 4), lc = lane_o & 15;
+                const int lcc = lc < NCH ? lc : 0;
+                u32x4 y0, y1;
+                ld128x2_now(sb + soff(row, 2 * lcc), sb + soff(row, 2 * lcc + 1), y0, y1);
+                const u32x4 o = {pack_bf16x2(__uint_as_float(y0[0]), __uint_as_float(y0[1])), pack_bf16x2(__uint_as_float(y0[2]), __uint_as_float(y0[3])),
+                                 pack_bf16x2(__uint_as_float(y1[0]), __uint_as_float(y1[1])), pack_bf16x2(__uint_as_float(y1[2]), __uint_as_float(y1[3]))};
+                if (lc < NCH) *(u32x4*)(p.dx + (tp * kT + row) * C + lc * 8) = o;
+            }
+        }
+    };
+
+    int64_t ti_prev = -1;
+    int buf = 0, sbuf = 0, it = 0;
+    for (; ti < p.tiles; ti += gridDim.x, ++it) {
+        asm volatile("" : "+v"(lane_o));
+        const uint32_t ybase = lds0 + Y_OFF + buf * YB, xbase = lds0 + X_OFF + buf * XB;
+        const uint32_t sbase = lds0 + S_OFF + sbuf * SB, sprev = lds0 + S_OFF + (sbuf ^ 1) * SB;
+        const int64_t ti_next = ti + (int64_t)D * gridDim.x;
+        const int nbuf = buf == 0 ? NS - 1 : buf - 1;
+        if (it > D && ti + (int64_t)(D - 1) * gridDim.x < p.tiles) {
+            if (HI_WAVES && wave < HI_WAVES) asm volatile("s_waitcnt vmcnt(%0)" ::"n"(VM_HI) : "memory");
+            else asm volatile("s_waitcnt vmcnt(%0)" ::"n"(VM_LO) : "memory");
+        } else {
+            asm volatile("s_waitcnt vmcnt(0)" ::: "memory");
+        }
+        asm volatile("s_waitcnt lgkmcnt(0)" ::: "memory");
+        __builtin_amdgcn_s_barrier();
+        if (ti_next < p.tiles) issue(ti_next, nbuf);
+        if (ti_prev >= 0) epilogue(ti_prev, sprev);
+
+        {
+            const int L = lane_o & 15, nblk = (lane_o >> 4) & 1, hf = lane_o >> 5;
+            const int cl = nblk * 2 + ((L & 3) >> 1);
+            s16x4 xf[2][2], yf[2][NBW][2];
+            auto reads = [&](int ks) {
+#pragma unroll
+                for (int h = 0; h < 2; ++h) {
+                    const int row = 16 * ks + 8 * hf + 4 * h + (L >> 2), sw = swz(row);
+                    const uint32_t in8 = (uint32_t)((L & 1) << 3);
+                    xf[ks][h] = ld_tr(xbase + row * XPITCH + (((4 * kb + cl) ^ sw) << 4) + in8);
+#pragma unroll
+                    for (int i = 0; i < NBW; ++i) yf[ks][i][h] = ld_tr(ybase + row * YPITCH + (((4 * (wn * NBW + i) + cl) ^ sw) << 4) + in8);
+                }
+            };
+            auto claim = [&](int ks) {
+                asm volatile("s_waitcnt lgkmcnt(0)" ::: "memory");
+#pragma unroll
+                for (int h = 0; h < 2; ++h) {
+                    asm volatile("" : "+v"(xf[ks][h]));
+#pragma unroll
+                    for (int i = 0; i < NBW; ++i) asm volatile("" : "+v"(yf[ks][i][h]));
+                }
+            };
+            auto mma = [&](int ks) {
+                const s16x8 b = {xf[ks][0][0], xf[ks][0][1], xf[ks][0][2], xf[ks][0][3], xf[ks][1][0], xf[ks][1][1], xf[ks][1][2], xf[ks][1][3]};
+#pragma unroll
+                for (int i = 0; i < NBW; ++i) {
+                    const s16x8 a = {yf[ks][i][0][0], yf[ks][i][0][1], yf[ks][i][0][2], yf[ks][i][0][3],
+                                     yf[ks][i][1][0], yf[ks][i][1][1], yf[ks][i][1][2], yf[ks][i][1][3]};
+                    acc[i][0] = __builtin_amdgcn_mfma_f32_32x32x16_bf16(__builtin_bit_cast(bf16x8, a), __builtin_bit_cast(bf16x8, b), acc[i][0], 0, 0, 0);
+                }
+            };
+            reads(0);
+            claim(0);
+            reads(1);
+            mma(0);
+            claim(1);
+            mma(1);
+        }
+        if (want_bias) {
+            constexpr int RJ = (kT + NW - 1) / NW;
+            const int yc = lane_o < NCHY ? lane_o : 0;
+            u32x4 v[RJ];
+#pragma unroll
+            for (int j = 0; j < RJ; ++j) {
+                const int row = wave + NW * j, rr = row < kT ? row : 0;
+                v[j] = ld128(ybase + rr * YPITCH + ((yc ^ swz(rr)) << 4));
+            }
+            asm volatile("s_waitcnt lgkmcnt(0)" ::: "memory");
+#pragma unroll
+            for (int j = 0; j < RJ; ++j) {
+                asm volatile("" : "+v"(v[j]));
+                if (wave + NW * j < kT && lane_o < NCHY) add_bf16x8(bsum, v[j][0], v[j][1], v[j][2], v[j][3]);
+            }
+        }
+        f32x4 y[2] = {f32x4{0.f, 0.f, 0.f, 0.f}, f32x4{0.f, 0.f, 0.f, 0.f}};
+        {
+            const int t15 = lane_o & 15, g4 = lane_o >> 4, sw = swz(t15);
+            const uint32_t ra0 = ybase + t15 * YPITCH, ra1 = ybase + (16 + t15) * YPITCH;
+            u32x4 fb[2][2];
+            auto reads = [&](int ks, int set) {
+                const uint32_t co = (uint32_t)(((4 * ks + g4) ^ sw) << 4);
+                fb[set][0] = ld128(ra0 + co);
+                fb[set][1] = ld128(ra1 + co);
+            };
+            reads(0, 0);
+#pragma unroll
+            for (int ks = 0; ks < KS2; ++ks) {
+                const int set = ks & 1;
+                if (ks + 1 < KS2) {
+                    reads(ks + 1, set ^ 1);
+                    asm volatile("s_waitcnt lgkmcnt(2)" : "+v"(fb[set][0]), "+v"(fb[set][1]));
+                } else {
+                    asm volatile("s_waitcnt lgkmcnt(0)" : "+v"(fb[set][0]), "+v"(fb[set][1]));
+                }
+                y[0] = __builtin_amdgcn_mfma_f32_16x16x32_bf16(wb[ks], as_frag(fb[set][0]), y[0], 0, 0, 0);
+                y[1] = __builtin_amdgcn_mfma_f32_16x16x32_bf16(wb[ks], as_frag(fb[set][1]), y[1], 0, 0, 0);
+            }
+            asm volatile("s_nop 7\n\ts_nop 7\n\ts_nop 7" : "+v"(y[0]), "+v"(y[1])::"memory");
+#pragma unroll
+            for (int t = 0; t < 2; ++t) st128(sbase + soff(16 * t + t15, 4 * wave + g4), __builtin_bit_cast(u32x4, y[t]));
+        }
+        ti_prev = ti;
+        buf = buf + 1 == NS ? 0 : buf + 1;
+        sbuf ^= 1;
+    }
+    asm volatile("s_waitcnt vmcnt(0)\n\ts_waitcnt lgkmcnt(0)" ::: "memory");
+    __builtin_amdgcn_s_barrier();
+    epilogue(ti_prev, lds0 + S_OFF + (sbuf ^ 1) * SB);
+
+    float* rec = p.part + (int64_t)blockIdx.x * record_floats(N, C);
+    store_partial(acc, rec, 32 * NBW * wn, 32 * kb, N, C, lane);
+    if (want_bias) {
+        __syncthreads();
+        fold_bias<512, NW>((float*)smem, bsum, tid, 0, N, rec + (int64_t)N * C);
+    }
+#endif
+}
+
+int64_t fused_grid(int64_t rows) { return std::max<int64_t>(1, std::min<int64_t>(rows / kT / 4, usable_cus())); }
+
+bool shape_ok(int n_out, int k_in, int dtype) { return dtype == HS_BF16 && (k_in == 96 || k_in == 128) && (n_out == k_in || n_out == 3 * k_in); }
+
+int linear_bwd_fused(const char* who, const void* dy, const void* x, const void* w_t, void* dx, float* dw, float* dbias, float* workspace,
+                     int64_t rows, int n_out, int k_in, int accumulate, int dtype, void* stream) {
+    HS_CHECK_ARG(dy && x && w_t && dx && dw && workspace, "%s: null pointer", who);
+    HS_CHECK_ARG(accumulate >= 0 && accumulate <= (1 | HS_ACC_DEFER), "%s: accumulate must be 0, 1 or either with HS_ACC_DEFER", who);
+    if (!shape_ok(n_out, k_in, dtype) || rows <= 0 || rows % kT || rows * n_out * 2 > 0x7FFFFE00ll)
+        return fail(HS_ERR_UNSUPPORTED, "%s: bf16, C = 96 or 128, rows a positive multiple of 32 below 2 GiB of dy only (got C = %d, rows %lld)", who,
+                    k_in, (long long)rows);
+    HS_CHECK_ALIGNED(who, 16, dy, x, w_t, dx, dw, dbias, workspace);
+    HalfBwdParams p{};
+    p.dy = (const uint16_t*)dy; p.x = (const uint16_t*)x; p.wt = (const uint16_t*)w_t; p.dx = (uint16_t*)dx;
+    p.part = workspace; p.tiles = rows / kT; p.want_bias = dbias != nullptr;
+    const int64_t grid = fused_grid(rows);
+    hipStream_t s = (hipStream_t)stream;
+    const dim3 g((unsigned)grid), b((unsigned)(k_in * 4));
+    if (k_in == 128 && n_out == 128) hipLaunchKernelGGL((linear_bwd_fused_kernel<128, 1>), g, b, 0, s, p);
+    else if (k_in == 128) hipLaunchKernelGGL((linear_bwd_fused_kernel<128, 3>), g, b, 0, s, p);
+    else if (n_out == 96) hipLaunchKernelGGL((linear_bwd_fused_kernel<96, 1>), g, b, 0, s, p);
+    else hipLaunchKernelGGL((linear_bwd_fused_kernel<96, 3>), g, b, 0, s, p);
+    HS_LAUNCH_CHECK("linear_bwd_fused");
+    return sum_slices(workspace, (int)grid, n_out, k_in, dw, dbias, accumulate, s);
+}
+
+}
+}
+
+extern "C" {
+
+int hs_attn_half_bwd_supported(int channels, int dtype) { return hs::shape_ok(channels, channels, dtype); }
+
+int64_t hs_attn_half_bwd_workspace(int64_t rows, int n_out, int channels) {
+    return rows > 0 ? hs::fused_grid(rows) * hs::record_floats(n_out, channels) : 0;
+}
+
+int hs_proj_bwd_fused(const void* dout, const void* o, const void* proj_w_t, void* d_o, float* dproj_w, float* dproj_b, float* workspace,
+                      int64_t rows, int channels, int accumulate, int dtype, void* stream) {
+    return hs::linear_bwd_fused("hs_proj_bwd_fused", dout, o, proj_w_t, d_o, dproj_w, dproj_b, workspace, rows, channels, channels, accumulate,
+                                dtype, stream);
+}
+
+int hs_qkv_bwd_fused(const void* dqkv, const void* qkv_in, const void* qkv_w_t, void* dx, float* dqkv_w, float* dqkv_b, float* workspace,
+                     int64_t rows, int channels, int accumulate, int dtype, void* stream) {
+    return hs::linear_bwd_fused("hs_qkv_bwd_fused", dqkv, qkv_in, qkv_w_t, dx, dqkv_w, dqkv_b, workspace, rows, 3 * channels, channels,
+                                accumulate, dtype, stream);
+}
+
+}
diff --git a/heal_swin_amd/csrc/hs_lds.h b/heal_swin_amd/csrc/hs_lds.h
--- /dev/null
+++ b/heal_swin_amd/csrc/hs_lds.h
@@ -0,0 +1,53 @@
+#pragma once
+#include "hs_device.h"
+
+namespace hs {
+
+typedef __attribute__((ext_vector_type(4))) float f32x4;
+typedef unsigned int u32x2v __attribute__((__vector_size__(8)));
+
+__device__ __forceinline__ u32x4 ld128(uint32_t addr) {
+    u32x4 v;
+    asm volatile("ds_read_b128 %0, %1" : "=v"(v) : "v"(addr));
+    return v;
+}
+__device__ __forceinline__ u32x2v ld64(uint32_t addr) {
+    u32x2v v;
+    asm volatile("ds_read_b64 %0, %1" : "=v"(v) : "v"(addr));
+    return v;
+}
+__device__ __forceinline__ u32x4 ld128_now(uint32_t addr) {
+    u32x4 v;
+    asm volatile("ds_read_b128 %0, %1\n\ts_waitcnt lgkmcnt(0)" : "=&v"(v) : "v"(addr) : "memory");
+    return v;
+}
+__device__ __forceinline__ void ld128x2_now(uint32_t a0, uint32_t a1, u32x4& v0, u32x4& v1) {
+    asm volatile("ds_read_b128 %0, %2\n\tds_read_b128 %1, %3\n\ts_waitcnt lgkmcnt(0)" : "=&v"(v0), "=&v"(v1) : "v"(a0), "v"(a1) : "memory");
+}
+__device__ __forceinline__ void ld128x4_now(uint32_t a0, uint32_t a1, uint32_t a2, uint32_t a3, u32x4& v0, u32x4& v1, u32x4& v2, u32x4& v3) {
+    asm volatile("ds_read_b128 %0, %4\n\tds_read_b128 %1, %5\n\tds_read_b128 %2, %6\n\tds_read_b128 %3, %7\n\ts_waitcnt lgkmcnt(0)"
+                 : "=&v"(v0), "=&v"(v1), "=&v"(v2), "=&v"(v3)
+                 : "v"(a0), "v"(a1), "v"(a2), "v"(a3)
+                 : "memory");
+}
+__device__ __forceinline__ void ld64x4_now(uint32_t a0, uint32_t a1, uint32_t a2, uint32_t a3, u32x2v& v0, u32x2v& v1, u32x2v& v2, u32x2v& v3) {
+    asm volatile("ds_read_b64 %0, %4\n\tds_read_b64 %1, %5\n\tds_read_b64 %2, %6\n\tds_read_b64 %3, %7\n\ts_waitcnt lgkmcnt(0)"
+                 : "=&v"(v0), "=&v"(v1), "=&v"(v2), "=&v"(v3)
+                 : "v"(a0), "v"(a1), "v"(a2), "v"(a3)
+                 : "memory");
+}
+__device__ __forceinline__ void st64(uint32_t addr, uint32_t a, uint32_t b) {
+    const u32x2v v = {a, b};
+    asm volatile("ds_write_b64 %0, %1" ::"v"(addr), "v"(v) : "memory");
+}
+__device__ __forceinline__ void st128(uint32_t addr, const u32x4& v) { asm volatile("ds_write_b128 %0, %1" ::"v"(addr), "v"(v) : "memory"); }
+__device__ __forceinline__ bf16x8 as_frag(const u32x4& v) { return __builtin_bit_cast(bf16x8, v); }
+__device__ __forceinline__ float row16_sum(float v) {
+    v += __builtin_bit_cast(float, __builtin_amdgcn_mov_dpp(__builtin_bit_cast(int, v), 0xB1, 0xF, 0xF, true));
+    v += __builtin_bit_cast(float, __builtin_amdgcn_mov_dpp(__builtin_bit_cast(int, v), 0x4E, 0xF, 0xF, true));
+    v += __builtin_bit_cast(float, __builtin_amdgcn_mov_dpp(__builtin_bit_cast(int, v), 0x141, 0xF, 0xF, true));
+    v += __builtin_bit_cast(float, __builtin_amdgcn_mov_dpp(__builtin_bit_cast(int, v), 0x140, 0xF, 0xF, true));
+    return v;
+}
+
+}
diff --git a/heal_swin_amd/csrc/hs_wgrad_device.h b/heal_swin_amd/csrc/hs_wgrad_device.h
--- /dev/null
+++ b/heal_swin_amd/csrc/hs_wgrad_device.h
@@ -0,0 +1,53 @@
+#pragma once
+#include "hs_device.h"
+
+namespace hs {
+
+__host__ __device__ constexpr int64_t record_floats(int n_out, int k_in) { return (int64_t)n_out * k_in + n_out; }
+
+template <int NB, int KB>
+__device__ __forceinline__ void store_partial(const f32x16 (&acc)[NB][KB], float* dst, int n_wave, int k_wave, int n_out, int k_in,
+                                              int lane) {
+#pragma unroll
+    for (int i = 0; i < NB; ++i)
+#pragma unroll
+        for (int j = 0; j < KB; ++j) {
+            const int kk = k_wave + j * 32 + (lane & 31);
+#pragma unroll
+            for (int r = 0; r < 16; ++r) {
+                const int nn = n_wave + i * 32 + (r & 3) + 8 * (r >> 2) + 4 * (lane >> 5);
+                if (nn < n_out && kk < k_in) dst[(int64_t)nn * k_in + kk] = acc[i][j][r];
+            }
+        }
+}
+
+template <int TN, int GROUPS, int PER_THREAD>
+__device__ __forceinline__ void fold_bias(float* bred, const float (&bsum)[PER_THREAD], int tid, int n0, int n_out, float* dst) {
+    constexpr int CH = TN / PER_THREAD;
+#pragma unroll
+    for (int i = 0; i < PER_THREAD; ++i) bred[(tid / CH) * TN + (tid % CH) * PER_THREAD + i] = bsum[i];
+    __syncthreads();
+    if (tid < TN) {
+        float t = 0.f;
+#pragma unroll
+        for (int rg = 0; rg < GROUPS; ++rg) t += bred[rg * TN + tid];
+        if (n0 + tid < n_out) dst[n0 + tid] = t;
+    }
+}
+
+__device__ __forceinline__ void add_bf16x8(float (&bsum)[8], uint32_t w0, uint32_t w1, uint32_t w2, uint32_t w3) {
+    const uint32_t w[4] = {w0, w1, w2, w3};
+#pragma unroll
+    for (int i = 0; i < 4; ++i) {
+        bsum[2 * i] += bf_lo(w[i]);
+        bsum[2 * i + 1] += bf_hi(w[i]);
+    }
+}
+
+inline int sum_slices(const float* part_w, int slices, int n_out, int k_in, float* dw, float* dbias, int accumulate, hipStream_t s) {
+    const int64_t n = (int64_t)n_out * k_in, rec = record_floats(n_out, k_in), count = dbias ? rec : n;
+    if (accumulate & HS_ACC_DEFER) return reduce_defer(part_w, rec, slices, n, count, dw, dbias, accumulate & 1, s);
+    return reduce_now(part_w, rec, slices, n, count, dw, dbias, accumulate & 1, s);
+}
+
+}
diff --git a/heal_swin_amd/csrc/linear_wgrad.hip b/heal_swin_amd/csrc/linear_wgrad.hip
--- a/heal_swin_amd/csrc/linear_wgrad.hip
+++ b/heal_swin_amd/csrc/linear_wgrad.hip
@@ -3,6 +3,7 @@
 #include <utility>
 
 #include "hs_gelu.h"
+#include "hs_wgrad_device.h"
 
 namespace hs {
 namespace {
@@ -31,8 +32,6 @@
     int tile_n, tile_k, tiles_n, tiles_k, tiles, slices, chunks, per_xcd, dma, reads_first;
     int64_t rows_per_slice;
 };
-
-__host__ __device__ constexpr int64_t record_floats(int n_out, int k_in) { return (int64_t)n_out * k_in + n_out; }
 
 inline void plan_slices(Geometry& g, int64_t rows, int wgs_per_cu) {
     int64_t want = ((int64_t)usable_cus() * wgs_per_cu) / g.tiles;
@@ -91,45 +90,6 @@
     int64_t m_end = m_begin + g.rows_per_slice;
     if (m_end > rows) m_end = rows;
     return {m_begin, m_end > m_begin ? (int)(m_end - m_begin) : 0};
-}
-
-template <int NB>
-__device__ __forceinline__ void store_partial(const f32x16 (&acc)[NB][2], float* dst, int n_wave, int k_wave, int n_out, int k_in,
-                                              int lane) {
-#pragma unroll
-    for (int i = 0; i < NB; ++i)
-#pragma unroll
-        for (int j = 0; j < 2; ++j) {
-            const int kk = k_wave + j * 32 + (lane & 31);
-#pragma unroll
-            for (int r = 0; r < 16; ++r) {
-                const int nn = n_wave + i * 32 + (r & 3) + 8 * (r >> 2) + 4 * (lane >> 5);
-                if (nn < n_out && kk < k_in) dst[(int64_t)nn * k_in + kk] = acc[i][j][r];
-            }
-        }
-}
-
-template <int TN, int GROUPS, int PER_THREAD>
-__device__ __forceinline__ void fold_bias(float* bred, const float (&bsum)[PER_THREAD], int tid, int n0, int n_out, float* dst) {
-    constexpr int CH = TN / PER_THREAD;
-#pragma unroll
-    for (int i = 0; i < PER_THREAD; ++i) bred[(tid / CH) * TN + (tid % CH) * PER_THREAD + i] = bsum[i];
-    __syncthreads();
-    if (tid < TN) {
-        float t = 0.f;
-#pragma unroll
-        for (int rg = 0; rg < GROUPS; ++rg) t += bred[rg * TN + tid];
-        if (n0 + tid < n_out) dst[n0 + tid] = t;
-    }
-}
-
-__device__ __forceinline__ void add_bf16x8(float (&bsum)[8], uint32_t w0, uint32_t w1, uint32_t w2, uint32_t w3) {
-    const uint32_t w[4] = {w0, w1, w2, w3};
-#pragma unroll
-    for (int i = 0; i < 4; ++i) {
-        bsum[2 * i] += bf_lo(w[i]);
-        bsum[2 * i + 1] += bf_hi(w[i]);
-    }
 }
 
 template <int NB>
@@ -600,12 +560,6 @@
         hipLaunchKernelGGL((wgrad_dma_kernel<2, 128>), grid, dim3(256), 0, s, tb, rows, g);
 }
 
-inline int sum_slices(const float* part_w, int slices, int n_out, int k_in, float* dw, float* dbias, int accumulate, hipStream_t s) {
-    const int64_t n = (int64_t)n_out * k_in, rec = record_floats(n_out, k_in), count = dbias ? rec : n;
-    if (accumulate & HS_ACC_DEFER) return reduce_defer(part_w, rec, slices, n, count, dw, dbias, accumulate & 1, s);
-    return reduce_now(part_w, rec, slices, n, count, dw, dbias, accumulate & 1, s);
-}
-
 struct GroupPlan {
     bool grouped;
     int variant, any_gelu;
diff --git a/heal_swin_amd/csrc/mlp_fused.hip b/heal_swin_amd/csrc/mlp_fused.hip
--- a/heal_swin_amd/csrc/mlp_fused.hip
+++ b/heal_swin_amd/csrc/mlp_fused.hip
@@ -1,13 +1,11 @@
 #include <algorithm>
 
 #include "hs_gelu.h"
+#include "hs_lds.h"
 
 namespace hs {
 HS_DEFINE_SEED_EPOCH_SETTER(set_seed_epoch_mlp_fused)
 namespace {
-
-typedef __attribute__((ext_vector_type(4))) float f32x4;
-typedef unsigned int u32x2v __attribute__((__vector_size__(8)));
 
 constexpr int kT = 32;
 constexpr float kLnEps = 1e-5f;
@@ -38,50 +36,6 @@
     int tiles_per_sample;
     int64_t row0;
 };
-
-__device__ __forceinline__ u32x4 ld128(uint32_t addr) {
-    u32x4 v;
-    asm volatile("ds_read_b128 %0, %1" : "=v"(v) : "v"(addr));
-    return v;
-}
-__device__ __forceinline__ u32x2v ld64(uint32_t addr) {
-    u32x2v v;
-    asm volatile("ds_read_b64 %0, %1" : "=v"(v) : "v"(addr));
-    return v;
-}
-__device__ __forceinline__ u32x4 ld128_now(uint32_t addr) {
-    u32x4 v;
-    asm volatile("ds_read_b128 %0, %1\n\ts_waitcnt lgkmcnt(0)" : "=&v"(v) : "v"(addr) : "memory");
-    return v;
-}
-__device__ __forceinline__ void ld128x2_now(uint32_t a0, uint32_t a1, u32x4& v0, u32x4& v1) {
-    asm volatile("ds_read_b128 %0, %2\n\tds_read_b128 %1, %3\n\ts_waitcnt lgkmcnt(0)" : "=&v"(v0), "=&v"(v1) : "v"(a0), "v"(a1) : "memory");
-}
-__device__ __forceinline__ void ld128x4_now(uint32_t a0, uint32_t a1, uint32_t a2, uint32_t a3, u32x4& v0, u32x4& v1, u32x4& v2, u32x4& v3) {
-    asm volatile("ds_read_b128 %0, %4\n\tds_read_b128 %1, %5\n\tds_read_b128 %2, %6\n\tds_read_b128 %3, %7\n\ts_waitcnt lgkmcnt(0)"
-                 : "=&v"(v0), "=&v"(v1), "=&v"(v2), "=&v"(v3)
-                 : "v"(a0), "v"(a1), "v"(a2), "v"(a3)
-                 : "memory");
-}
-__device__ __forceinline__ void ld64x4_now(uint32_t a0, uint32_t a1, uint32_t a2, uint32_t a3, u32x2v& v0, u32x2v& v1, u32x2v& v2, u32x2v& v3) {
-    asm volatile("ds_read_b64 %0, %4\n\tds_read_b64 %1, %5\n\tds_read_b64 %2, %6\n\tds_read_b64 %3, %7\n\ts_waitcnt lgkmcnt(0)"
-                 : "=&v"(v0), "=&v"(v1), "=&v"(v2), "=&v"(v3)
-                 : "v"(a0), "v"(a1), "v"(a2), "v"(a3)
-                 : "memory");
-}
-__device__ __forceinline__ void st64(uint32_t addr, uint32_t a, uint32_t b) {
-    const u32x2v v = {a, b};
-    asm volatile("ds_write_b64 %0, %1" ::"v"(addr), "v"(v) : "memory");
-}
-__device__ __forceinline__ void st128(uint32_t addr, const u32x4& v) { asm volatile("ds_write_b128 %0, %1" ::"v"(addr), "v"(v) : "memory"); }
-__device__ __forceinline__ bf16x8 as_frag(const u32x4& v) { return __builtin_bit_cast(bf16x8, v); }
-__device__ __forceinline__ float row16_sum(float v) {
-    v += __builtin_bit_cast(float, __builtin_amdgcn_mov_dpp(__builtin_bit_cast(int, v), 0xB1, 0xF, 0xF, true));
-    v += __builtin_bit_cast(float, __builtin_amdgcn_mov_dpp(__builtin_bit_cast(int, v), 0x4E, 0xF, 0xF, true));
-    v += __builtin_bit_cast(float, __builtin_amdgcn_mov_dpp(__builtin_bit_cast(int, v), 0x141, 0xF, 0xF, true));
-    v += __builtin_bit_cast(float, __builtin_amdgcn_mov_dpp(__builtin_bit_cast(int, v), 0x140, 0xF, 0xF, true));
-    return v;
-}
 
 template <int C, bool BWD, bool DROP>
 __global__ void __launch_bounds__(C * 4, 1) mlp_fused_kernel(MlpParams p) {
diff --git a/heal_swin_amd/csrc/module_ops.cpp b/heal_swin_amd/csrc/module_ops.cpp
--- a/heal_swin_amd/csrc/module_ops.cpp
+++ b/heal_swin_amd/csrc/module_ops.cpp
@@ -1,8 +1,15 @@
+#include <cstdlib>
+#include <cstring>
+
 #include "hs_common.h"
 
 namespace {
 inline int64_t max64(int64_t a, int64_t b) { return a > b ? a : b; }
 inline int64_t round4(int64_t v) { return (v + 3) & ~(int64_t)3; }
+inline bool qkv_fused(int64_t rows, int channels, int dtype) {
+    static const bool on = !(getenv("HS_FUSED_ATTN_HALF_BWD") && !strcmp(getenv("HS_FUSED_ATTN_HALF_BWD"), "0"));
+    return on && hs_attn_half_bwd_supported(channels, dtype) && rows % 32 == 0 && rows * 3 * channels * 2 <= 0x7FFFFE00ll;
+}
 }
 
 extern "C" {
@@ -13,6 +20,10 @@
     ws = max64(ws, hs_linear_wgrad_workspace(rows, 3 * channels, channels));
     ws = max64(ws, hs_linear_wgrad_workspace(rows, channels, channels));
     ws = max64(ws, hs_layernorm_bwd_workspace(rows, channels));
+    if (qkv_fused(rows, channels, HS_BF16)) {
+        const int64_t f = hs_attn_half_bwd_workspace(rows, 3 * channels, channels);
+        if (f > ws) ws += round4(f - ws);
+    }
     return round4(rows * channels * 5 / 2 + 4) + ws;
 }
 
@@ -62,13 +73,18 @@
                                     num_heads, window_size, cflags, 0.f, 0, dtype, stream))
         return st;
     const void* qkv_in = v1 ? xn : x;
-    if (int st = hs_linear_wgrad(dqkv, qkv_in, dqkv_w, dqkv_b, ws, rows, 3 * C, C, accumulate, dtype, stream)) return st;
-    if (!v1)
-        return hs_gemm_nt(dqkv, 3 * C, qkv_w_t, 3 * C, 3 * C, nullptr, 0, nullptr, 0, 0, nullptr, dx, nullptr, rows, C, HS_EPI_BIAS, 0.f, 0, dtype,
-                          stream);
-    if (int st = hs_gemm_nt(dqkv, 3 * C, qkv_w_t, 3 * C, 3 * C, nullptr, 0, nullptr, 0, 0, nullptr, dxn, nullptr, rows, C, HS_EPI_BIAS, 0.f, 0, dtype,
-                            stream))
-        return st;
+    if (qkv_fused(rows, C, dtype)) {
+        if (int st = hs_qkv_bwd_fused(dqkv, qkv_in, qkv_w_t, v1 ? (void*)dxn : dx, dqkv_w, dqkv_b, ws, rows, C, accumulate, dtype, stream)) return st;
+        if (!v1) return HS_OK;
+    } else {
+        if (int st = hs_linear_wgrad(dqkv, qkv_in, dqkv_w, dqkv_b, ws, rows, 3 * C, C, accumulate, dtype, stream)) return st;
+        if (!v1)
+            return hs_gemm_nt(dqkv, 3 * C, qkv_w_t, 3 * C, 3 * C, nullptr, 0, nullptr, 0, 0, nullptr, dx, nullptr, rows, C, HS_EPI_BIAS, 0.f, 0,
+                              dtype, stream);
+        if (int st = hs_gemm_nt(dqkv, 3 * C, qkv_w_t, 3 * C, 3 * C, nullptr, 0, nullptr, 0, 0, nullptr, dxn, nullptr, rows, C, HS_EPI_BIAS, 0.f, 0,
+                                dtype, stream))
+            return st;
+    }
     const void* dres = (flags & HS_ATTN_RESIDUAL) ? dout : nullptr;
     if (dres) return hs_add_layernorm_bwd(dxn, dres, x, ln_gamma, mean, rstd, dx, dln_gamma, dln_beta, ws, accumulate, rows, C, dtype, stream);
     return hs_layernorm_bwd(dxn, x, ln_gamma, mean, rstd, dx, dln_gamma, dln_beta, ws, accumulate, rows, C, dtype, stream);
diff --git a/heal_swin_amd/ops/attention.py b/heal_swin_amd/ops/attention.py
--- a/heal_swin_amd/ops/attention.py
+++ b/heal_swin_amd/ops/attention.py
@@ -338,13 +338,13 @@
         if residual_alias:
             qkv_t, x_res = LinearFn.apply(x, qkv_w, qkv_b, True, None, (qkv,))
         else:
-            qkv_t = LinearFn.apply(x, qkv_w, qkv_b, False, None, (qkv,))
+            qkv_t = LinearFn.apply(x, qkv_w, qkv_b, False, None, (qkv,), True)
         o_t = WindowAttnCoreFn.apply(qkv_t, bias, head_scale, idx, roll, labels, num_heads, window_size, cosine, 0.0, 0, (o, lse))
         y = LinearFn.apply(o_t, proj_w, proj_b, False, None, (out,))
         return (y, x_res) if residual_alias else y
     assert not residual_alias
     n1, xs = LayerNormFn.apply(x, ln_weight, ln_bias, None, None, True, None, False, (xn, mean, rstd))
-    qkv_t = LinearFn.apply(n1, qkv_w, qkv_b, False, None, (qkv,))
+    qkv_t = LinearFn.apply(n1, qkv_w, qkv_b, False, None, (qkv,), True)
     o_t = WindowAttnCoreFn.apply(qkv_t, bias, head_scale, idx, roll, labels, num_heads, window_size, cosine, 0.0, 0, (o, lse))
     x1 = LinearFn.apply(o_t, proj_w, proj_b, False, xs, (out,))
     if n2 is None:
diff --git a/heal_swin_amd/ops/gemm.py b/heal_swin_amd/ops/gemm.py
--- a/heal_swin_amd/ops/gemm.py
+++ b/heal_swin_amd/ops/gemm.py
@@ -351,10 +351,50 @@
     return dw, db
 
 
+FUSED_ATTN_HALF_BWD = os.environ.get("HS_FUSED_ATTN_HALF_BWD", "1") != "0"
+
+
+def _linear_bwd_fused(dy2, x2, weight, bias, want_b, cache):
+    rows, n_out = dy2.shape
+    k_in = x2.shape[1]
+    if not (FUSED_ATTN_HALF_BWD and dy2.dtype == torch.bfloat16 and x2.dtype == torch.bfloat16 and x2.is_contiguous() and
+            n_out in (k_in, 3 * k_in) and rows % 32 == 0 and rows * n_out * 2 <= 0x7FFFFE00 and
+            lib.hs_attn_half_bwd_supported(k_in, _lib.HS_BF16)):
+        return None
+    wbuf = _sink_buffer(weight)
+    bbuf = _sink_buffer(bias) if (wbuf is not None and want_b) else None
+    deposit = wbuf is not None and (not want_b or bbuf is not None)
+    w_t = _cast_param_t(weight, torch.bfloat16, cache)
+    if any(t.data_ptr() % 16 for t in (dy2, x2, w_t)):
+        return None
+    dev = dy2.device
+    if deposit:
+        acc = 1 | _defer_flag(dev)
+    else:
+        acc = 0
+        wbuf = torch.empty((n_out, k_in), dtype=torch.float32, device=dev)
+        bbuf = torch.empty(n_out, dtype=torch.float32, device=dev) if want_b else None
+    dx = torch.empty((rows, k_in), dtype=torch.bfloat16, device=dev)
+    ws = torch.empty(int(lib.hs_attn_half_bwd_workspace(rows, n_out, k_in)), dtype=torch.float32, device=dev)
+    fn, tag = (lib.hs_proj_bwd_fused, "proj_bwd_fused") if n_out == k_in else (lib.hs_qkv_bwd_fused, "qkv_bwd_fused")
+    with _timed(tag, dev, 2 * rows * (n_out + 2 * k_in), 4 * rows * n_out * k_in):
+        check(fn(ptr(dy2), ptr(x2), ptr(w_t), ptr(dx), ptr(wbuf.view(n_out, k_in)), ptr(bbuf), ptr(ws), rows, k_in, acc, _lib.HS_BF16,
+                 stream_ptr(dev)), tag)
+    if acc & _lib.HS_ACC_DEFER:
+        _defer_keep(dev, ws)
+    if not deposit:
+        return dx, wbuf.to(weight.dtype).view(weight.shape), (bbuf.to(bias.dtype) if want_b else None)
+    RT.grad_sink.deposited(weight)
+    if want_b:
+        RT.grad_sink.deposited(bias)
+    return dx, None, None
+
+
 class LinearFn(torch.autograd.Function):
 
     @staticmethod
-    def forward(ctx, x, weight, bias, passthrough=False, residual=None, pre=None):
+    def forward(ctx, x, weight, bias, passthrough=False, residual=None, pre=None, fuse_bwd=False):
+        ctx.fuse_bwd = bool(fuse_bwd)
         _require_gpu(x, weight, bias, residual)
         n_out = weight.shape[0]
         k_in = weight.numel() // n_out
@@ -430,18 +470,24 @@
         n_out = weight.shape[0]
         k_in = weight.numel() // n_out
         if dy is None:
-            return dx_res, None, None, None, None, None
+            return dx_res, None, None, None, None, None, None
         dy2 = dy.reshape(-1, n_out)
         x2 = None if x is None else x.reshape(-1, k_in)
         if not dy2.is_contiguous():
             dy2 = dy2.contiguous()
         dx = None
+        want_b = bias is not None and ctx.needs_input_grad[2]
+        if ctx.fuse_bwd and dx_res is None and x2 is not None and ctx.needs_input_grad[0] and ctx.needs_input_grad[1]:
+            fused = _linear_bwd_fused(dy2, x2, weight, bias, want_b, ctx.cast_cache)
+            if fused is not None:
+                ctx.w_cast = ctx.cast_cache = ctx.x3 = None
+                return fused[0].reshape(ctx.x_shape), fused[1], fused[2], None, (dy if ctx.has_residual else None), None, None
         if ctx.needs_input_grad[0]:
             dx = _input_grad(dy2, weight, ctx.w_cast, None if dx_res is None else dx_res.reshape(-1, k_in), ctx.cast_cache).reshape(ctx.x_shape)
         ctx.w_cast = ctx.cast_cache = None
         x3, ctx.x3 = ctx.x3, None
-        dw, db = _param_grads(dy2, x2, weight, bias, ctx.needs_input_grad[1], bias is not None and ctx.needs_input_grad[2], x3)
-        return dx, dw, db, None, (dy if ctx.has_residual else None), None
+        dw, db = _param_grads(dy2, x2, weight, bias, ctx.needs_input_grad[1], want_b, x3)
+        return dx, dw, db, None, (dy if ctx.has_residual else None), None, None
 
 
 def _input_grad(dy2, weight, w_cast, dx_res2=None, cache=None):
diff --git a/include/healswin.h b/include/healswin.h
--- a/include/healswin.h
+++ b/include/healswin.h
@@ -177,6 +177,12 @@
                      int channels, int hidden, unsigned flags, int dtype, void* stream);
 int hs_mlp_fused_bwd(const void* dy, const void* h, const void* w2_t, const void* w1_t, const void* dres, void* dh, void* dn, int64_t rows,
                      int channels, int hidden, int dtype, void* stream);
+int hs_attn_half_bwd_supported(int channels, int dtype);
+int64_t hs_attn_half_bwd_workspace(int64_t rows, int n_out, int channels);
+int hs_proj_bwd_fused(const void* dout, const void* o, const void* proj_w_t, void* d_o, float* dproj_w, float* dproj_b, float* workspace,
+                      int64_t rows, int channels, int accumulate, int dtype, void* stream);
+int hs_qkv_bwd_fused(const void* dqkv, const void* qkv_in, const void* qkv_w_t, void* dx, float* dqkv_w, float* dqkv_b, float* workspace,
+                     int64_t rows, int channels, int accumulate, int dtype, void* stream);
 int hs_mlp_fused_drop_fwd(const void* x, const float* ln_gamma, const float* ln_beta, const void* w1, const float* b1, const void* w2,
                           const float* b2, void* m_out, float* mean_out, float* rstd_out, void* h_out, void* act_out, void* out,
                           const float* row_scale, int64_t rows_per_sample, float drop_p, uint64_t seed_hidden, uint64_t seed_out,
```

New measurement: 57.45 (median of 6 runs). No clear change (+0.2%).
